# paninski-lab/lightning-pose

Measured on AMD Instinct MI355X. Metric: training frames/sec (whole node), ResNet-50 384x384 17-kp semi-sup, higher is better.
Workload: dtype bf16; 1 GPU; C2/C3: ResNet-50 SemiSupervisedHeatmapTracker 384x384, K=17, 64 labeled + 128 unlabeled frames per GPU, heatmap_mse + temporal + pca_singleview + unimodal_mse, Adam (backbone lr=0 as at step 0), bf16-mixed; global_batch=192, parallelism=dp1, sync_batchnorm=False, decode_prune=plain kernels (chosen from the maps)

## Files before the change

include/lp_hip.h:

```cpp
#ifndef LP_HIP_H
#define LP_HIP_H

#include <stddef.h>
#include <stdint.h>

#ifdef __cplusplus
extern "C" {
#endif

typedef void* lp_stream_t;

int lp_config_reload_env(void);

enum {
    LP_OK = 0,
    LP_ERR_ARGUMENT = -1,
    LP_ERR_UNSUPPORTED = -2,
};

enum { LP_TF_NONE = 0, LP_TF_SINGLE = 1, LP_TF_PER_FRAME = 2, LP_TF_PER_VIEW = 3 };

#define LP_HIP_ABI_VERSION 148
int lp_version(void);
const char* lp_strerror(int code);


typedef struct lp_decode_tables {
    const int* row_base;
    const float* row_taps;
    const int* col_start;
    const float* col_taps;
    const int* colT_start;
    const float* colT_taps;
    int ty, tx, tc;
} lp_decode_tables;

typedef struct lp_frame_map {
    const float* transforms;
    int tf_mode;
    const float* bbox;
    int bbox_stride;
    int kp_per_view;
    float model_h, model_w;
} lp_frame_map;

int lp_decode_window(int downsample_factor, int n);


int lp_decode_fwd(const float* heat, int B, int K, int h, int w, int downsample_factor, float temperature,
                  const lp_decode_tables* tables, const lp_frame_map* frame_map, float* kp_aug, float* kp_frame, float* conf,
                  float* stats, int prune, lp_stream_t stream);

int lp_decode_bwd(const float* heat, int B, int K, int h, int w, int downsample_factor, float temperature,
                  const lp_decode_tables* tables, const lp_frame_map* frame_map, const float* stats, const float* g_kp_aug,
                  const float* g_kp_frame, float* g_heat, int accumulate, int prune, lp_stream_t stream);

int lp_frame_map_apply(const float* kp_in, int B, int K, const lp_frame_map* frame_map, int backward, float* kp_out,
                       lp_stream_t stream);


int lp_heatmap_gen(const float* keypoints, const int* visibility, int B, int K, int img_h, int img_w, int h, int w, float sigma,
                   float* out, lp_stream_t stream);
int lp_heatmap_gen_bwd(const float* keypoints, const int* visibility, int B, int K, int img_h, int img_w, int h, int w, float sigma,
                       const float* grad_out, float* grad_keypoints, lp_stream_t stream);

size_t lp_temporal_heatmap_workspace_bytes(int S, int K);
int lp_temporal_heatmap_fwd(int kind, const float* pred, const float* conf, int S, int K, int h, int w, const float* epsilon,
                            float prob_threshold, float* loss, void* workspace, lp_stream_t stream);
int lp_temporal_heatmap_bwd(int kind, const float* pred, int S, int K, int h, int w, const void* workspace, const float* gout,
                            float* gpred, int accumulate, lp_stream_t stream);

int lp_heatmap_confidence(const float* heat, const float* locs, int B, int K, int h, int w, int radius, float* out, lp_stream_t stream);

size_t lp_heatmap_mse_workspace_bytes(int B, int K);
int lp_heatmap_mse_fwd(const float* targ, const float* pred, int B, int K, int h, int w, float* loss, void* workspace,
                       lp_stream_t stream);
int lp_heatmap_mse_bwd(const float* targ, const float* pred, int B, int K, int h, int w, const void* workspace, const float* gout,
                       float* gpred, int accumulate, lp_stream_t stream);
enum { LP_HM_MSE = 0, LP_HM_KL = 1, LP_HM_JS = 2 };
int lp_heatmap_loss_fwd(int kind, const float* targ, const float* pred, int B, int K, int h, int w, float* loss, void* workspace,
                        lp_stream_t stream);
int lp_heatmap_loss_bwd(int kind, const float* targ, const float* pred, int B, int K, int h, int w, const void* workspace,
                        const float* gout, float* gpred, int accumulate, lp_stream_t stream);

int lp_unimodal_mse_fwd(const float* kp_aug, const float* pred, const float* conf, int S, int K, int img_h, int img_w, int h, int w,
                        float sigma, float prob_threshold, float* loss, void* workspace, lp_stream_t stream);
int lp_unimodal_mse_bwd(const float* kp_aug, const float* pred, int S, int K, int img_h, int img_w, int h, int w, float sigma,
                        const void* workspace, const float* gout, float* gpred, int accumulate, lp_stream_t stream);

int lp_softmax2d_fwd(const float* in, long stride_b, long stride_i, long stride_k, int B, int K, int n, float* out,
                     lp_stream_t stream);
int lp_softmax2d_bwd(const float* prob, const float* gprob, int B, int K, int n, void* gin_bf16, long stride_b, long stride_i,
                     long stride_k, lp_stream_t stream);


int lp_temporal_fwd_bwd(const float* kp, const float* conf, int S, int K, const float* eps_per_kp, float prob_threshold,
                        float* loss, float* grad_unit, lp_stream_t stream);

int lp_pca_fwd_bwd(const float* kp, int S, int K, const int* index, int rows, int points, const float* mean,
                   const float* kept_eigenvectors, int ncomp, float epsilon, float* loss, float* grad_unit, lp_stream_t stream);

int lp_rmse_fwd(const float* kp_targ, const float* kp_pred, int n_points, float* loss, lp_stream_t stream);
int lp_loss_combine(const float* const* x, const float* w, const float* a, int n, float* weighted, float* total, lp_stream_t stream);
int lp_loss_combine_bwd(const float* w, const float* a, int n, const float* g_weighted, const float* g_total, float* gx, lp_stream_t stream);

typedef struct lp_conv_geom {
    int B, Hi, Wi, Ci;
    int Ho, Wo, Co;
    int R, S, stride, pad;
} lp_conv_geom;

#define LP_CONV_KERNEL_IGEMM 0
#define LP_CONV_KERNEL_PIPE 1
#define LP_CONV_KERNEL_WGRAD 2
#define LP_CONV_KERNEL_WGRAD_PIPE 3
#define LP_CONV_KERNEL_PIPE_HALO 4
#define LP_CONV_KERNEL_STEM_WGRAD_NB 8
#define LP_CONV_KERNEL_WGRAD_NB 9
#define LP_CONV_KERNEL_RES2D 5
int lp_conv_last_kernel(void);

int lp_conv_fwd(const void* x, const void* w, const lp_conv_geom* geom, const float* bias, void* out_bf16, float* out_f32, int ldo,
                int n_store, lp_stream_t stream);
int lp_conv_dgrad(const void* dy, const void* wd, const lp_conv_geom* geom, const float* bias, const void* addend,
                  const void* relu_mask, void* dx_bf16, float* dx_f32, int ldo, int n_store, int skip_empty_classes,
                  lp_stream_t stream);
typedef struct lp_gemm_batch {
    int nb, nh;
    long long a_b, a_h, b_b, b_h, c_b, c_h;
} lp_gemm_batch;
int lp_gemm_nt(const void* a, int lda, const void* b, int ldb, void* c_bf16, float* c_f32, int ldc, int M, int N, int K, int n_store,
               const float* bias, const lp_gemm_batch* batch, lp_stream_t stream);
int lp_gemm_tn(const void* x, int ldx, const void* y, int ldy, void* out_bf16, int ldo, int M, int J, int N, const lp_gemm_batch* batch,
               lp_stream_t stream);
int lp_attn_fwd(const void* qkv_bf16, int ld_qkv, int k_off, int v_off, int B, int nh, int T, float scale, void* p_bf16, int ldp,
                void* out_bf16, int ldo, lp_stream_t stream);
int lp_attn_bwd_kv(const void* qkv_bf16, int ld_qkv, int v_off, const void* d_out_bf16, int ld_do, const void* p_bf16, int ldp, const float* d_rows,
                   int B, int nh, int T, float scale, void* ds_bf16, void* dqkv_bf16, int ld_dqkv, int dk_off, int dv_off, lp_stream_t stream);
int lp_attn_rowdot(const void* a_bf16, const void* b_bf16, int rows, int nh, int ld, float* out, lp_stream_t stream);
int lp_attn_dscores(const void* d_out, int ld_do, const void* v, int ldv, const void* p_bf16, const float* d_rows, int d_row_stride,
                    long long d_b, long long d_h, float scale, void* ds_bf16, int ldc, int M, int N, int K, const lp_gemm_batch* batch,
                    lp_stream_t stream);
typedef struct lp_fxsum {
    long long hi, lo;
} lp_fxsum;
int lp_gemm_nt_gelu_bwd(const void* a, const void* b, const void* u_bf16, void* c_bf16, int M, int N, int K, lp_fxsum* colsum,
                        lp_stream_t stream);
int lp_gemm_nt_gelu_fwd(const void* a, const void* b, const float* bias, void* c_bf16, void* act_bf16, int M, int N, int K,
                        lp_stream_t stream);
typedef struct lp_bn_fuse {
    const void* z;
    const float* mean;
    const float* invstd;
    const float* gamma;
    const float* beta;
    int mask_from_z;
    const void* relu_bits;
    lp_fxsum* sums;
    int seg_images;
    int addend_half;
} lp_bn_fuse;
int lp_conv_dgrad_bits(const void* dy, const void* wd, const lp_conv_geom* geom, const void* addend, const void* relu_bits, void* dx_bf16,
                       int skip_empty_classes, lp_stream_t stream);
int lp_bn_fold(const float* w, const float* gamma, const float* beta, const float* running_mean, const float* running_var, float eps,
               int Co, int per_co, void* w_bf16, float* bias, lp_stream_t stream);
int lp_conv_fwd_act(const void* x, const void* w, const lp_conv_geom* geom, const float* bias, const void* residual_bf16, int relu,
                    void* out_bf16, lp_stream_t stream);
int lp_conv_fwd_bn(const void* x, const void* w, const lp_conv_geom* geom, void* out_bf16, const lp_bn_fuse* bn, lp_stream_t stream);
int lp_stem_fwd_bn(const void* x4, const void* w, const lp_conv_geom* geom, void* out_bf16, const lp_bn_fuse* bn, lp_stream_t stream);
int lp_conv_dgrad_bn(const void* dy, const void* wd, const lp_conv_geom* geom, const void* addend, const void* relu_mask,
                     void* dx_bf16, const lp_bn_fuse* bn, lp_stream_t stream);
size_t lp_conv_wgrad_workspace_bytes(const lp_conv_geom* geom, int split_hint);
int lp_conv_wgrad(const void* x, const void* dy, const lp_conv_geom* geom, float* dw, int split_hint, void* workspace,
                  size_t workspace_bytes, lp_stream_t stream);
int lp_conv_wgrad_bias(const void* x, const void* dy, const lp_conv_geom* geom, float* dw, float* dbias, int split_hint, void* workspace,
                       size_t workspace_bytes, lp_stream_t stream);
int lp_stem_fwd(const void* x4, const void* w, const lp_conv_geom* geom, void* out_bf16, lp_stream_t stream);
int lp_stem_wgrad(const void* x4, const void* dy, const lp_conv_geom* geom, float* dw, int split_hint, void* workspace,
                  size_t workspace_bytes, lp_stream_t stream);

int lp_f32_conv_fwd(const float* x, const float* w, const lp_conv_geom* geom, int KH, int KW, int CiS, const float* bias,
                    const float* addend, float* out, lp_stream_t stream);
int lp_f32_conv_dgrad(const float* dy, const float* w, const lp_conv_geom* geom, int KH, int KW, int CiS, const float* bias,
                      const float* addend, float* dx, lp_stream_t stream);
int lp_f32_conv_wgrad(const float* x, const float* dy, const lp_conv_geom* geom, int KH, int KW, int CiS, float* dw, lp_stream_t stream);
int lp_f32_bn_stats(const float* x, int M, int C, float* sums, lp_stream_t stream);
size_t lp_f32_bn_stats_workspace_bytes(int M, int C);
int lp_f32_bn_stats_ordered(const float* x, int M, int C, float* sums, void* workspace, size_t workspace_bytes, lp_stream_t stream);
int lp_f32_bn_apply(const float* x, const float* mean, const float* invstd, const float* gamma, const float* beta, const float* residual,
                    int relu, int M, int C, float* y, lp_stream_t stream);
int lp_f32_bn_bwd_reduce(const float* dy, const float* y_out, const float* x, const float* mean, const float* invstd, int M, int C,
                         float* sums, float* dbeta_acc, float* dgamma_acc, lp_stream_t stream);
int lp_f32_bn_bwd_apply(const float* dy, const float* y_out, const float* x, const float* mean, const float* invstd, const float* gamma,
                        const float* sums, float count, int M, int C, float* dx, float* dres, lp_stream_t stream);
int lp_f32_maxpool_fwd(const float* x, int B, int Hi, int Wi, int C, float* y, void* argmax_u8, lp_stream_t stream);
int lp_f32_maxpool_bwd(const void* argmax_u8, const float* dy, int B, int Hi, int Wi, int C, float* dx, lp_stream_t stream);
int lp_f32_images_to_nhwc4(const float* images, int B, int H, int W, float* out, lp_stream_t stream);
int lp_f32_pixel_shuffle(const float* in, int B, int h, int w, int c_out, int ld, int inverse, float* out, lp_stream_t stream);
int lp_f32_softmax2d_bwd(const float* prob, const float* gprob, int B, int K, int n, float* gin, long stride_b, long stride_i, long stride_k,
                         lp_stream_t stream);
int lp_f32_vit_patchify(const float* images, int B, int H, int W, int patch, float* out, lp_stream_t stream);
int lp_f32_vit_tokens_fwd(const float* patch, const float* cls, const float* pos, int B, int Np, int D, float* x, lp_stream_t stream);
int lp_f32_vit_tokens_bwd(const float* dx, int B, int Np, int D, float* dpatch, float* dpos, lp_stream_t stream);
int lp_f32_vit_mv_tokens_fwd(const float* patch, const float* pos, const float* view, int B, int V, int Np, int D, float* x, lp_stream_t stream);
int lp_f32_vit_mv_tokens_bwd(const float* dx, int B, int V, int Np, int D, float* dpatch, float* dpos, float* dview, void* workspace,
                             size_t workspace_bytes, lp_stream_t stream);
int lp_f32_layernorm_fwd(const float* x, const float* delta, float* x_out, const float* gamma, const float* beta, float eps, int M, int D,
                         int drop_T, float* y, float* mean, float* rstd, lp_stream_t stream);
int lp_f32_layernorm_bwd(const float* dy, const float* x, const float* mean, const float* rstd, const float* gamma, int M, int D, int drop_T,
                         float* dx_acc, float* dgamma_acc, float* dbeta_acc, lp_stream_t stream);
int lp_f32_layernorm_ls_fwd(const float* x, const float* delta, const float* ls, float* x_out, const float* gamma, const float* beta, float eps,
                            int M, int D, int drop_T, float* y, float* mean, float* rstd, lp_stream_t stream);
int lp_f32_layernorm_ls_bwd(const float* dy, const float* x, const float* mean, const float* rstd, const float* gamma, const float* ls,
                            const float* branch, int M, int D, int drop_T, float* dx_acc, float* dx_out, float* dgamma_acc, float* dbeta_acc,
                            float* colsum_acc, float* dls_acc, lp_stream_t stream);
int lp_f32_gelu_fwd(const float* x, size_t n, float* y, lp_stream_t stream);
int lp_f32_gelu_bwd(const float* x, const float* dy, size_t n, float* dx, lp_stream_t stream);
int lp_f32_attn_fwd(const float* qkv, int ld, int k_off, int v_off, int B, int nh, int T, float scale, float* p, float* o, int ldo,
                    lp_stream_t stream);
int lp_f32_attn_bwd(const float* qkv, int ld, int k_off, int v_off, const float* dout, int ldo, const float* p, int B, int nh, int T,
                    float scale, float* ds_workspace, float* dqkv, int ldd, lp_stream_t stream);

size_t lp_bn_reduce_workspace_bytes(int M, int C);
int lp_bn_stats(const void* x, int M, int C, lp_fxsum* sums, void* workspace, size_t workspace_bytes, lp_stream_t stream);
int lp_fxsum_accumulate(const lp_fxsum* sums, int n, float* dst, lp_stream_t stream);
int lp_bn_finalize(const lp_fxsum* sums, float count, int C, float eps, float momentum, float* mean, float* invstd,
                   float* running_mean, float* running_var, lp_stream_t stream);
int lp_bn_finalize_f32(const float* sums, float count, int C, float eps, float momentum, float* mean, float* invstd,
                       float* running_mean, float* running_var, lp_stream_t stream);
int lp_bn_finalize2(const lp_fxsum* sums, float count0, float count1, int C, float eps, float momentum, float* mean, float* invstd,
                    float* running_mean, float* running_var, lp_stream_t stream);
int lp_bn_apply(const void* x, const float* mean, const float* invstd, const float* gamma, const float* beta, const void* residual,
                int relu, int M, int C, void* y, void* relu_bits, lp_stream_t stream);
int lp_bn_apply_seg(const void* x, const float* mean, const float* invstd, const float* gamma, const float* beta, const void* residual,
                    int relu, int M, int C, int seg_rows, void* y, void* relu_bits, lp_stream_t stream);
int lp_bn_apply_seg_lo(const void* x, const float* mean, const float* invstd, const float* gamma, const float* beta, const void* residual,
                       const void* residual_lo, const void* zd, const float* mean_d, const float* invstd_d, const float* gamma_d,
                       const float* beta_d, int relu, int M, int C, int seg_rows, void* y, void* y_lo, void* relu_bits, lp_stream_t stream);
int lp_bn_apply_seg_rbn(const void* x, const float* mean, const float* invstd, const float* gamma, const float* beta, const void* zd,
                        const float* mean_d, const float* invstd_d, const float* gamma_d, const float* beta_d, int relu, int M, int C,
                        int seg_rows, void* y, void* relu_bits, lp_stream_t stream);
int lp_bn_bwd_reduce(const void* dy, const void* y_out, const void* x, const float* mean, const float* invstd, int M, int C,
                     lp_fxsum* sums, void* workspace, size_t workspace_bytes, lp_stream_t stream);
int lp_bn_bwd_apply(const void* dy, const void* y_out, const void* x, const float* mean, const float* invstd, const float* gamma,
                    const lp_fxsum* sums, float count, int M, int C, void* dx, void* dres, const lp_fxsum* sums_local, float* dbeta_acc,
                    float* dgamma_acc, float* terms_ws, lp_stream_t stream);
int lp_bn_bwd_apply_seg(const void* dy, const void* y_out, const void* x, const float* mean, const float* invstd, const float* gamma,
                        const lp_fxsum* sums, float count0, float count1, int M, int C, int seg_rows, void* dx, void* dres,
                        const lp_fxsum* sums_local, float* dbeta_acc, float* dgamma_acc, float* terms_ws, lp_stream_t stream);
size_t lp_bn_bwd_ds_workspace_bytes(int M, int C);
int lp_bn_bwd_apply_seg_ds(const void* dy, const void* y_out, const void* x, const float* mean, const float* invstd, const float* gamma,
                           const lp_fxsum* sums, float count0, float count1, int M, int C, int seg_rows, void* dx, void* dres,
                           const lp_fxsum* sums_local, float* dbeta_acc, float* dgamma_acc, float* terms_ws, const void* zd,
                           const float* mean_d, const float* invstd_d, lp_fxsum* sums_d, void* workspace, size_t workspace_bytes,
                           lp_stream_t stream);
int lp_maxpool_fwd(const void* x, int B, int Hi, int Wi, int C, void* y, void* argmax_u8, lp_stream_t stream);
int lp_maxpool_bwd(const void* argmax_u8, const void* dy, int B, int Hi, int Wi, int C, void* dx, lp_stream_t stream);
int lp_bn_relu_maxpool_fwd(const void* z, const float* mean, const float* invstd, const float* gamma, const float* beta, int B, int Hi, int Wi,
                           int C, void* y, void* argmax_u8, lp_stream_t stream);
int lp_bn_pool_bwd_reduce(const void* argmax_u8, const void* dy, const void* z, const float* mean, const float* invstd, const float* gamma,
                          const float* beta, int B, int Hi, int Wi, int C, lp_fxsum* sums, lp_stream_t stream);
int lp_bn_pool_bwd_apply(const void* argmax_u8, const void* dy, const void* z, const float* mean, const float* invstd, const float* gamma,
                         const float* beta, const lp_fxsum* sums, float count, int B, int Hi, int Wi, int C, void* dx,
                         const lp_fxsum* sums_local, float* dbeta_acc, float* dgamma_acc, lp_stream_t stream);
int lp_images_to_nhwc4(const float* images_nchw, int B, int H, int W, void* out_bf16, lp_stream_t stream);
int lp_pixel_shuffle(const void* in, int B, int h, int w, int c_out, int ld, int inverse, void* out, lp_stream_t stream);

int lp_vit_patchify(const float* images_nchw, int B, int H, int W, int patch, void* out_bf16, lp_stream_t stream);
int lp_vit_tokens_fwd(const void* patch_bf16, const float* cls, const float* pos, int B, int Np, int D, float* x, lp_stream_t stream);
int lp_vit_tokens_bwd(const float* dx, int B, int Np, int D, void* dpatch_bf16, float* dpos, lp_stream_t stream);
int lp_vit_mv_tokens_fwd(const void* patch_bf16, const float* pos, const float* view, int B, int V, int Np, int D, float* x,
                         lp_stream_t stream);
size_t lp_vit_mv_tokens_bwd_workspace_bytes(int B, int V, int Np, int D);
int lp_vit_mv_tokens_bwd(const float* dx, int B, int V, int Np, int D, void* dpatch_bf16, float* dpos, float* dview, void* workspace,
                         size_t workspace_bytes, lp_stream_t stream);
#define LP_CAM_MAX_VIEWS 32
size_t lp_cam_chain_workspace_bytes(int B, int V, int K);
int lp_cam_chain_fwd(const float* points, const float* intrinsics, const float* extrinsics, const float* dist12, const float* bbox, float model_h,
                     float model_w, int B, int V, int K, float* p3d, float* p2d, lp_stream_t stream);
int lp_cam_chain_bwd(const float* points, const float* intrinsics, const float* extrinsics, const float* dist12, const float* bbox, float model_h,
                     float model_w, int B, int V, int K, const float* p3d, const float* g3d, const float* g2d, void* workspace,
                     size_t workspace_bytes, float* gpoints, lp_stream_t stream);
int lp_cam_project_fwd(const float* points_3d, const float* intrinsics, const float* extrinsics, const float* dist12, const float* bbox,
                       float model_h, float model_w, int B, int V, int K, float* p2d, lp_stream_t stream);
int lp_cam_project_bwd(const float* points_3d, const float* intrinsics, const float* extrinsics, const float* dist12, const float* bbox,
                       float model_h, float model_w, int B, int V, int K, const float* g2d, float* g3d, lp_stream_t stream);
int lp_cam_pairwise_fwd_bwd(const float* targ_3d, const float* pred_3d, int B, int P, int K, float* loss, float* grad_unit, lp_stream_t stream);
int lp_small_matmul(const float* w, const float* x, int R, int Q, int D, int transpose_w, int accumulate, float* y, lp_stream_t stream);
int lp_layernorm_fwd(const float* x, const void* delta_bf16, float* x_out, const float* gamma, const float* beta, float eps, int M,
                     int D, int drop_T, void* y_bf16, float* mean, float* rstd, lp_stream_t stream);
int lp_layernorm_bwd(const void* dy_bf16, const float* x, const float* mean, const float* rstd, const float* gamma, int M, int D,
                     int drop_T, float* dx_acc, float* dgamma_acc, float* dbeta_acc, lp_stream_t stream);
int lp_layernorm_bwd_bf16(const void* dy_bf16, const float* x, const float* mean, const float* rstd, const float* gamma, int M, int D,
                          int drop_T, float* dx_acc, void* dx_bf16, float* dgamma_acc, float* dbeta_acc, lp_stream_t stream);
int lp_gelu_fwd(const void* x_bf16, size_t n, void* y_bf16, lp_stream_t stream);
int lp_gelu_bwd(const void* x_bf16, const void* dy_bf16, size_t n, void* dx_bf16, lp_stream_t stream);
int lp_gelu_bwd_colsum(const void* x_bf16, const void* dy_bf16, int rows, int cols, void* dx_bf16, float* colsum_acc, lp_stream_t stream);
int lp_layernorm_bwd_bf16_colsum(const void* dy_bf16, const float* x, const float* mean, const float* rstd, const float* gamma, int M, int D,
                                 int drop_T, float* dx_acc, void* dx_bf16, float* dgamma_acc, float* dbeta_acc, float* colsum_acc,
                                 lp_stream_t stream);
int lp_layernorm_ls_fwd(const float* x, const void* delta_bf16, const float* ls, float* x_out, const float* gamma, const float* beta, float eps,
                        int M, int D, int drop_T, void* y_bf16, float* mean, float* rstd, lp_stream_t stream);
int lp_layernorm_ls_bwd(const void* dy_bf16, const float* x, const float* mean, const float* rstd, const float* gamma, const float* ls,
                        const void* branch_bf16, int M, int D, int drop_T, float* dx_acc, void* dx_bf16, float* dgamma_acc, float* dbeta_acc,
                        float* colsum_acc, float* dls_acc, lp_stream_t stream);
int lp_softmax_rows_fwd(void* s_bf16, int rows, int n, int ld, float scale, lp_stream_t stream);
int lp_softmax_rows_bwd(const void* p_bf16, void* dp_bf16, int rows, int n, int ld, float scale, lp_stream_t stream);
int lp_transpose_batched(const void* in_bf16, int R, int Cc, int ldi, long long in_b, long long in_h, void* out_bf16, int ldo,
                         long long out_b, long long out_h, int nb, int nh, lp_stream_t stream);

enum { LP_BORDER_RENORM = 0,
       LP_BORDER_CLAMP = 1    };

typedef struct lp_frame_norm {
    float mean[3], std[3];
} lp_frame_norm;

typedef struct lp_frame_augment {
    int has_matrix;
    float matrix[6];
    float brightness, contrast, contrast_center;
    float shot_factor;
    unsigned long long seed;
} lp_frame_augment;

int lp_frames_resize(const void* src_u8, int S, int Hs, int Ws, long long frame_stride, int row_stride, int H, int W, int border,
                     const lp_frame_norm* finish_norm, float* dst, lp_stream_t stream);
int lp_frames_resize_cubic(const void* src_u8, int S, int Hs, int Ws, long long frame_stride, int row_stride, int H, int W, int round_u8,
                           const lp_frame_norm* finish_norm, float* dst, lp_stream_t stream);
int lp_frames_augment(const float* src_hwc, int S, int H, int W, const lp_frame_augment* aug, const lp_frame_norm* norm,
                      float* dst_nchw, lp_stream_t stream);
int lp_labeled_keypoints(const float* kp_src, const float* src_hw, const float* affine, const int* hflip, const int* swap,
                         const int* vis_in, int uniform_heatmaps, int B, int K, int H, int W, float* kp_out, int* vis_out,
                         lp_stream_t stream);

enum { LP_AUG_GEOM = 1, LP_AUG_BLUR = 2, LP_AUG_DROPOUT = 4, LP_AUG_DROP_PER_CHANNEL = 8, LP_AUG_SALT = 16, LP_AUG_PEPPER = 32,
       LP_AUG_ELASTIC = 64, LP_AUG_HISTEQ = 128, LP_AUG_CLAHE = 256, LP_AUG_EMBOSS = 512, LP_AUG_CROPPAD = 1024, LP_AUG_HFLIP = 2048 };
enum { LP_AUG_OP_DROPOUT = 0, LP_AUG_OP_SALT = 1, LP_AUG_OP_PEPPER = 2, LP_AUG_OP_ELASTIC = 3 };
enum { LP_AUG_LOCAL_BLUR_COARSE = 0, LP_AUG_LOCAL_EMBOSS = 1 };
#define LP_AUG_ELASTIC_MAX_RADIUS 20

typedef struct lp_labelaug_image {
    int flags;
    int image_id;
    float geom[6];
    float blur[25];
    float emboss[9];
    int coarse_gh[3], coarse_gw[3];
    unsigned coarse_thr[3];
    float elastic_alpha;
    int clahe_clip, clahe_tiles_y, clahe_tiles_x, clahe_slot;
    int pad[4];
} lp_labelaug_image;

int lp_labelaug_geom(const void* src_u8, int B, int H, int W, const lp_labelaug_image* params, void* dst_u8, lp_stream_t stream);
int lp_labelaug_local(const void* src_u8, int B, int H, int W, const lp_labelaug_image* params, int which, const void* salt_lut,
                      unsigned long long seed, void* dst_u8, lp_stream_t stream);
int lp_labelaug_elastic_field(int B, int H, int W, const lp_labelaug_image* params, float sigma, unsigned long long seed, float* tmp,
                              float* field, lp_stream_t stream);
int lp_labelaug_elastic_apply(const void* src_u8, int B, int H, int W, const lp_labelaug_image* params, const float* field, void* dst_u8,
                              lp_stream_t stream);
int lp_labelaug_histeq(const void* src_u8, int B, int H, int W, const lp_labelaug_image* params, unsigned* ws, void* lut_out, void* dst_u8,
                       lp_stream_t stream);
int lp_labelaug_clahe(const void* src_u8, int B, int H, int W, const lp_labelaug_image* params, const int* slot_image, int n_slots,
                      int max_ty, int max_tx, void* luts, void* dst_u8, lp_stream_t stream);
int lp_labelaug_finish(const void* src_u8, int B, int Hs, int Ws, const lp_labelaug_image* params, int H, int W, const lp_frame_norm* norm,
                       float* dst, lp_stream_t stream);
int lp_labelaug_keypoints(const float* kp, int B, int K, const float* affine, const lp_labelaug_image* params, const float* field, int H,
                          int W, float* kp_out, lp_stream_t stream);

int lp_patch_mask_f32(const float* images, int BV, int C, int H, int W, int patch, int count, unsigned long long key, const float* mask_in,
                      float* out, float* mask_out, lp_stream_t stream);

#define LP_MV3D_MAX_VIEWS 8
#define LP_MV3D_MAX_KEYPOINTS 128
int lp_mv3d_plan(const float* kp, const float* src_hw, const float* bbox, const float* intrinsics, const float* extrinsics,
                 const float* dist12, const float* draws, int augment, float shift_param, int H, int W, int B, int V, int K, float* kp3d,
                 float* kp2d, float* affine, int* status, lp_stream_t stream);
int lp_mv3d_fill(const void* src_u8, int B, int Hs, int Ws, const lp_frame_norm* norm, float* fill, lp_stream_t stream);
int lp_mv3d_finish(const void* src_u8, int B, int Hs, int Ws, const float* affine, const float* fill, const lp_frame_norm* norm, int V,
                   int v, int H, int W, float* dst, lp_stream_t stream);

int lp_adam_step(float* params, const float* grads, float* exp_avg, float* exp_avg_sq, size_t n, float lr, float beta1, float beta2,
                 float eps, float weight_decay, int decoupled, int step, float grad_scale, void* params_bf16, lp_stream_t stream);
int lp_cast_bf16(const float* src, size_t n, void* dst, lp_stream_t stream);
int lp_permute_cba(const void* src, int A, int B, int C, void* dst, lp_stream_t stream);

#ifdef __cplusplus
}
#endif
#endif
```

lightning-pose_amd/_lib.py:

```python

from __future__ import annotations

import ctypes as C
import os

_HERE = os.path.dirname(os.path.abspath(__file__))
LIB_PATH = os.environ.get("LP_HIP_LIB") or os.path.join(_HERE, "liblp_hip.so")


class LpHipUnavailable(RuntimeError):
    """liblp_hip.so could not be loaded, or an op was given a non-ROCm tensor.  There is no fallback path."""


class LpHipError(RuntimeError):
    pass


class DecodeTables(C.Structure):
    _fields_ = [("row_base", C.c_void_p), ("row_taps", C.c_void_p), ("col_start", C.c_void_p),
                ("col_taps", C.c_void_p), ("colT_start", C.c_void_p), ("colT_taps", C.c_void_p),
                ("ty", C.c_int), ("tx", C.c_int), ("tc", C.c_int)]


class FrameMap(C.Structure):
    _fields_ = [("transforms", C.c_void_p), ("tf_mode", C.c_int), ("bbox", C.c_void_p), ("bbox_stride", C.c_int),
                ("kp_per_view", C.c_int), ("model_h", C.c_float), ("model_w", C.c_float)]


class ConvGeom(C.Structure):
    _fields_ = [(n, C.c_int) for n in ("B", "Hi", "Wi", "Ci", "Ho", "Wo", "Co", "R", "S", "stride", "pad")]


class BnFuse(C.Structure):
    _fields_ = [("z", C.c_void_p), ("mean", C.c_void_p), ("invstd", C.c_void_p), ("gamma", C.c_void_p), ("beta", C.c_void_p),
                ("mask_from_z", C.c_int), ("relu_bits", C.c_void_p), ("sums", C.c_void_p), ("seg_images", C.c_int), ("addend_half", C.c_int)]


class FrameNorm(C.Structure):
    _fields_ = [("mean", C.c_float * 3), ("std", C.c_float * 3)]


class FrameAugment(C.Structure):
    _fields_ = [("has_matrix", C.c_int), ("matrix", C.c_float * 6), ("brightness", C.c_float), ("contrast", C.c_float),
                ("contrast_center", C.c_float), ("shot_factor", C.c_float), ("seed", C.c_ulonglong)]


class GemmBatch(C.Structure):
    _fields_ = [("nb", C.c_int), ("nh", C.c_int)] + [(n, C.c_longlong) for n in ("a_b", "a_h", "b_b", "b_h", "c_b", "c_h")]


HM_MSE, HM_KL, HM_JS = 0, 1, 2
(CONV_KERNEL_IGEMM, CONV_KERNEL_PIPE, CONV_KERNEL_WGRAD, CONV_KERNEL_WGRAD_PIPE, CONV_KERNEL_PIPE_HALO, CONV_KERNEL_RES2D, _CONV_KERNEL_6,
 _CONV_KERNEL_7, CONV_KERNEL_STEM_WGRAD_NB, CONV_KERNEL_WGRAD_NB) = range(10)
CONV_KERNEL_LABEL = {
    CONV_KERNEL_PIPE: (("conv_igemm_kernel", "conv_pipe_kernel"),),
    CONV_KERNEL_PIPE_HALO: (("conv_igemm_kernel", "conv_pipe_kernel"), (">", ",halo>")),
    CONV_KERNEL_RES2D: (("conv_igemm_kernel<64,", "conv_res2d_kernel<"), ("conv_igemm_kernel<64>", "conv_res2d_kernel<fwd>")),
    CONV_KERNEL_WGRAD_PIPE: (("conv_wgrad_kernel", "conv_wgrad_pipe_kernel"),),
    CONV_KERNEL_WGRAD_NB: (("conv_wgrad_kernel", "conv_wgrad_nb_kernel"),),
}
BORDER_RENORM, BORDER_CLAMP = 0, 1
AUG_GEOM, AUG_BLUR, AUG_DROPOUT, AUG_DROP_PER_CHANNEL, AUG_SALT, AUG_PEPPER = 1, 2, 4, 8, 16, 32
AUG_ELASTIC, AUG_HISTEQ, AUG_CLAHE, AUG_EMBOSS, AUG_CROPPAD, AUG_HFLIP = 64, 128, 256, 512, 1024, 2048
AUG_OP_DROPOUT, AUG_OP_SALT, AUG_OP_PEPPER, AUG_OP_ELASTIC = 0, 1, 2, 3
AUG_LOCAL_BLUR_COARSE, AUG_LOCAL_EMBOSS = 0, 1
AUG_ELASTIC_MAX_RADIUS = 20
TF_NONE, TF_SINGLE, TF_PER_FRAME, TF_PER_VIEW = 0, 1, 2, 3

ABI_VERSION = 148

_P, _I, _F, _L, _Z = C.c_void_p, C.c_int, C.c_float, C.c_long, C.c_size_t

PROTOTYPES = {
    "lp_version": (_I, []),
    "lp_strerror": (C.c_char_p, [_I]),
    "lp_config_reload_env": (_I, []),
    "lp_decode_window": (_I, [_I, _I]),
    "lp_decode_fwd": (_I, [_P, _I, _I, _I, _I, _I, _F, C.POINTER(DecodeTables), C.POINTER(FrameMap), _P, _P, _P, _P, _I, _P]),
    "lp_decode_bwd": (_I, [_P, _I, _I, _I, _I, _I, _F, C.POINTER(DecodeTables), C.POINTER(FrameMap), _P, _P, _P, _P, _I, _I, _P]),
    "lp_frame_map_apply": (_I, [_P, _I, _I, C.POINTER(FrameMap), _I, _P, _P]),
    "lp_heatmap_gen": (_I, [_P, _P, _I, _I, _I, _I, _I, _I, _F, _P, _P]),
    "lp_heatmap_gen_bwd": (_I, [_P, _P, _I, _I, _I, _I, _I, _I, _F, _P, _P, _P]),
    "lp_temporal_heatmap_workspace_bytes": (_Z, [_I, _I]),
    "lp_temporal_heatmap_fwd": (_I, [_I, _P, _P, _I, _I, _I, _I, _P, _F, _P, _P, _P]),
    "lp_temporal_heatmap_bwd": (_I, [_I, _P, _I, _I, _I, _I, _P, _P, _P, _I, _P]),
    "lp_heatmap_confidence": (_I, [_P, _P, _I, _I, _I, _I, _I, _P, _P]),
    "lp_heatmap_mse_workspace_bytes": (_Z, [_I, _I]),
    "lp_heatmap_mse_fwd": (_I, [_P, _P, _I, _I, _I, _I, _P, _P, _P]),
    "lp_heatmap_mse_bwd": (_I, [_P, _P, _I, _I, _I, _I, _P, _P, _P, _I, _P]),
    "lp_heatmap_loss_fwd": (_I, [_I, _P, _P, _I, _I, _I, _I, _P, _P, _P]),
    "lp_heatmap_loss_bwd": (_I, [_I, _P, _P, _I, _I, _I, _I, _P, _P, _P, _I, _P]),
    "lp_unimodal_mse_fwd": (_I, [_P, _P, _P, _I, _I, _I, _I, _I, _I, _F, _F, _P, _P, _P]),
    "lp_unimodal_mse_bwd": (_I, [_P, _P, _I, _I, _I, _I, _I, _I, _F, _P, _P, _P, _I, _P]),
    "lp_softmax2d_fwd": (_I, [_P, _L, _L, _L, _I, _I, _I, _P, _P]),
    "lp_softmax2d_bwd": (_I, [_P, _P, _I, _I, _I, _P, _L, _L, _L, _P]),
    "lp_temporal_fwd_bwd": (_I, [_P, _P, _I, _I, _P, _F, _P, _P, _P]),
    "lp_pca_fwd_bwd": (_I, [_P, _I, _I, _P, _I, _I, _P, _P, _I, _F, _P, _P, _P]),
    "lp_rmse_fwd": (_I, [_P, _P, _I, _P, _P]),
    "lp_loss_combine": (_I, [_P, _P, _P, _I, _P, _P, _P]),
    "lp_loss_combine_bwd": (_I, [_P, _P, _I, _P, _P, _P, _P]),
    "lp_conv_fwd": (_I, [_P, _P, C.POINTER(ConvGeom), _P, _P, _P, _I, _I, _P]),
    "lp_conv_dgrad": (_I, [_P, _P, C.POINTER(ConvGeom), _P, _P, _P, _P, _P, _I, _I, _I, _P]),
    "lp_conv_dgrad_bits": (_I, [_P, _P, C.POINTER(ConvGeom), _P, _P, _P, _I, _P]),
    "lp_gemm_nt": (_I, [_P, _I, _P, _I, _P, _P, _I, _I, _I, _I, _I, _P, C.POINTER(GemmBatch), _P]),
    "lp_gemm_nt_gelu_bwd": (_I, [_P, _P, _P, _P, _I, _I, _I, _P, _P]),
    "lp_gemm_nt_gelu_fwd": (_I, [_P, _P, _P, _P, _P, _I, _I, _I, _P]),
    "lp_gemm_tn": (_I, [_P, _I, _P, _I, _P, _I, _I, _I, _I, C.POINTER(GemmBatch), _P]),
    "lp_attn_fwd": (_I, [_P, _I, _I, _I, _I, _I, _I, C.c_float, _P, _I, _P, _I, _P]),
    "lp_attn_bwd_kv": (_I, [_P, _I, _I, _P, _I, _P, _I, _P, _I, _I, _I, C.c_float, _P, _P, _I, _I, _I, _P]),
    "lp_attn_rowdot": (_I, [_P, _P, _I, _I, _I, _P, _P]),
    "lp_attn_dscores": (_I, [_P, _I, _P, _I, _P, _P, _I, C.c_longlong, C.c_longlong, C.c_float, _P, _I, _I, _I, _I, C.POINTER(GemmBatch), _P]),
    "lp_conv_fwd_bn": (_I, [_P, _P, C.POINTER(ConvGeom), _P, C.POINTER(BnFuse), _P]),
    "lp_conv_last_kernel": (_I, []),
    "lp_stem_fwd_bn": (_I, [_P, _P, C.POINTER(ConvGeom), _P, C.POINTER(BnFuse), _P]),
    "lp_conv_dgrad_bn": (_I, [_P, _P, C.POINTER(ConvGeom), _P, _P, _P, C.POINTER(BnFuse), _P]),
    "lp_bn_fold": (_I, [_P, _P, _P, _P, _P, _F, _I, _I, _P, _P, _P]),
    "lp_conv_fwd_act": (_I, [_P, _P, C.POINTER(ConvGeom), _P, _P, _I, _P, _P]),
    "lp_conv_wgrad_workspace_bytes": (_Z, [C.POINTER(ConvGeom), _I]),
    "lp_conv_wgrad": (_I, [_P, _P, C.POINTER(ConvGeom), _P, _I, _P, _Z, _P]),
    "lp_conv_wgrad_bias": (_I, [_P, _P, C.POINTER(ConvGeom), _P, _P, _I, _P, C.c_size_t, _P]),
    "lp_stem_fwd": (_I, [_P, _P, C.POINTER(ConvGeom), _P, _P]),
    "lp_stem_wgrad": (_I, [_P, _P, C.POINTER(ConvGeom), _P, _I, _P, _Z, _P]),
    "lp_bn_reduce_workspace_bytes": (_Z, [_I, _I]),
    "lp_bn_stats": (_I, [_P, _I, _I, _P, _P, _Z, _P]),
    "lp_bn_finalize": (_I, [_P, _F, _I, _F, _F, _P, _P, _P, _P, _P]),
    "lp_fxsum_accumulate": (_I, [_P, _I, _P, _P]),
    "lp_bn_finalize_f32": (_I, [_P, _F, _I, _F, _F, _P, _P, _P, _P, _P]),
    "lp_bn_finalize2": (_I, [_P, _F, _F, _I, _F, _F, _P, _P, _P, _P, _P]),
    "lp_bn_apply": (_I, [_P, _P, _P, _P, _P, _P, _I, _I, _I, _P, _P, _P]),
    "lp_bn_apply_seg": (_I, [_P, _P, _P, _P, _P, _P, _I, _I, _I, _I, _P, _P, _P]),
    "lp_bn_apply_seg_lo": (_I, [_P, _P, _P, _P, _P, _P, _P, _P, _P, _P, _P, _P, _I, _I, _I, _I, _P, _P, _P, _P]),
    "lp_bn_apply_seg_rbn": (_I, [_P, _P, _P, _P, _P, _P, _P, _P, _P, _P, _I, _I, _I, _I, _P, _P, _P]),
    "lp_bn_bwd_apply_seg": (_I, [_P, _P, _P, _P, _P, _P, _P, _F, _F, _I, _I, _I, _P, _P, _P, _P, _P, _P, _P]),
    "lp_bn_bwd_ds_workspace_bytes": (_Z, [_I, _I]),
    "lp_bn_bwd_apply_seg_ds": (_I, [_P, _P, _P, _P, _P, _P, _P, _F, _F, _I, _I, _I, _P, _P, _P, _P, _P, _P, _P, _P, _P, _P, _P, _Z, _P]),
    "lp_bn_bwd_reduce": (_I, [_P, _P, _P, _P, _P, _I, _I, _P, _P, _Z, _P]),
    "lp_bn_bwd_apply": (_I, [_P, _P, _P, _P, _P, _P, _P, _F, _I, _I, _P, _P, _P, _P, _P, _P, _P]),
    "lp_maxpool_fwd": (_I, [_P, _I, _I, _I, _I, _P, _P, _P]),
    "lp_maxpool_bwd": (_I, [_P, _P, _I, _I, _I, _I, _P, _P]),
    "lp_bn_relu_maxpool_fwd": (_I, [_P, _P, _P, _P, _P, _I, _I, _I, _I, _P, _P, _P]),
    "lp_bn_pool_bwd_reduce": (_I, [_P, _P, _P, _P, _P, _P, _P, _I, _I, _I, _I, _P, _P]),
    "lp_bn_pool_bwd_apply": (_I, [_P, _P, _P, _P, _P, _P, _P, _P, C.c_float, _I, _I, _I, _I, _P, _P, _P, _P, _P]),
    "lp_images_to_nhwc4": (_I, [_P, _I, _I, _I, _P, _P]),
    "lp_pixel_shuffle": (_I, [_P, _I, _I, _I, _I, _I, _I, _P, _P]),
    "lp_vit_patchify": (_I, [_P, _I, _I, _I, _I, _P, _P]),
    "lp_vit_tokens_fwd": (_I, [_P, _P, _P, _I, _I, _I, _P, _P]),
    "lp_vit_tokens_bwd": (_I, [_P, _I, _I, _I, _P, _P, _P]),
    "lp_vit_mv_tokens_fwd": (_I, [_P, _P, _P, _I, _I, _I, _I, _P, _P]),
    "lp_vit_mv_tokens_bwd_workspace_bytes": (_Z, [_I, _I, _I, _I]),
    "lp_vit_mv_tokens_bwd": (_I, [_P, _I, _I, _I, _I, _P, _P, _P, _P, _Z, _P]),
    "lp_cam_chain_workspace_bytes": (_Z, [_I, _I, _I]),
    "lp_cam_chain_fwd": (_I, [_P, _P, _P, _P, _P, _F, _F, _I, _I, _I, _P, _P, _P]),
    "lp_cam_chain_bwd": (_I, [_P, _P, _P, _P, _P, _F, _F, _I, _I, _I, _P, _P, _P, _P, _Z, _P, _P]),
    "lp_cam_project_fwd": (_I, [_P, _P, _P, _P, _P, _F, _F, _I, _I, _I, _P, _P]),
    "lp_cam_project_bwd": (_I, [_P, _P, _P, _P, _P, _F, _F, _I, _I, _I, _P, _P, _P]),
    "lp_cam_pairwise_fwd_bwd": (_I, [_P, _P, _I, _I, _I, _P, _P, _P]),
    "lp_small_matmul": (_I, [_P, _P, _I, _I, _I, _I, _I, _P, _P]),
    "lp_layernorm_fwd": (_I, [_P, _P, _P, _P, _P, _F, _I, _I, _I, _P, _P, _P, _P]),
    "lp_layernorm_bwd": (_I, [_P, _P, _P, _P, _P, _I, _I, _I, _P, _P, _P, _P]),
    "lp_layernorm_bwd_bf16": (_I, [_P, _P, _P, _P, _P, _I, _I, _I, _P, _P, _P, _P, _P]),
    "lp_gelu_fwd": (_I, [_P, _Z, _P, _P]),
    "lp_gelu_bwd": (_I, [_P, _P, _Z, _P, _P]),
    "lp_gelu_bwd_colsum": (_I, [_P, _P, _I, _I, _P, _P, _P]),
    "lp_layernorm_bwd_bf16_colsum": (_I, [_P, _P, _P, _P, _P, _I, _I, _I, _P, _P, _P, _P, _P, _P]),
    "lp_layernorm_ls_fwd": (_I, [_P, _P, _P, _P, _P, _P, _F, _I, _I, _I, _P, _P, _P, _P]),
    "lp_layernorm_ls_bwd": (_I, [_P, _P, _P, _P, _P, _P, _P, _I, _I, _I, _P, _P, _P, _P, _P, _P, _P]),
    "lp_softmax_rows_fwd": (_I, [_P, _I, _I, _I, _F, _P]),
    "lp_softmax_rows_bwd": (_I, [_P, _P, _I, _I, _I, _F, _P]),
    "lp_transpose_batched": (_I, [_P, _I, _I, _I, C.c_longlong, C.c_longlong, _P, _I, C.c_longlong, C.c_longlong, _I, _I, _P]),
    "lp_frames_resize": (_I, [_P, _I, _I, _I, C.c_longlong, _I, _I, _I, _I, C.POINTER(FrameNorm), _P, _P]),
    "lp_frames_resize_cubic": (_I, [_P, _I, _I, _I, C.c_longlong, _I, _I, _I, _I, C.POINTER(FrameNorm), _P, _P]),
    "lp_frames_augment": (_I, [_P, _I, _I, _I, C.POINTER(FrameAugment), C.POINTER(FrameNorm), _P, _P]),
    "lp_labeled_keypoints": (_I, [_P, _P, _P, _P, _P, _P, _I, _I, _I, _I, _I, _P, _P, _P]),
    "lp_labelaug_geom": (_I, [_P, _I, _I, _I, _P, _P, _P]),
    "lp_labelaug_local": (_I, [_P, _I, _I, _I, _P, _I, _P, C.c_ulonglong, _P, _P]),
    "lp_labelaug_elastic_field": (_I, [_I, _I, _I, _P, _F, C.c_ulonglong, _P, _P, _P]),
    "lp_labelaug_elastic_apply": (_I, [_P, _I, _I, _I, _P, _P, _P, _P]),
    "lp_labelaug_histeq": (_I, [_P, _I, _I, _I, _P, _P, _P, _P, _P]),
    "lp_labelaug_clahe": (_I, [_P, _I, _I, _I, _P, _P, _I, _I, _I, _P, _P, _P]),
    "lp_labelaug_finish": (_I, [_P, _I, _I, _I, _P, _I, _I, C.POINTER(FrameNorm), _P, _P]),
    "lp_labelaug_keypoints": (_I, [_P, _I, _I, _P, _P, _P, _I, _I, _P, _P]),
    "lp_patch_mask_f32": (_I, [_P, _I, _I, _I, _I, _I, _I, C.c_ulonglong, _P, _P, _P, _P]),
    "lp_mv3d_plan": (_I, [_P, _P, _P, _P, _P, _P, _P, _I, _F, _I, _I, _I, _I, _I, _P, _P, _P, _P, _P]),
    "lp_mv3d_fill": (_I, [_P, _I, _I, _I, C.POINTER(FrameNorm), _P, _P]),
    "lp_mv3d_finish": (_I, [_P, _I, _I, _I, _P, _P, C.POINTER(FrameNorm), _I, _I, _I, _I, _P, _P]),
    "lp_f32_conv_fwd": (_I, [_P, _P, C.POINTER(ConvGeom), _I, _I, _I, _P, _P, _P, _P]),
    "lp_f32_conv_dgrad": (_I, [_P, _P, C.POINTER(ConvGeom), _I, _I, _I, _P, _P, _P, _P]),
    "lp_f32_conv_wgrad": (_I, [_P, _P, C.POINTER(ConvGeom), _I, _I, _I, _P, _P]),
    "lp_f32_bn_stats": (_I, [_P, _I, _I, _P, _P]),
    "lp_f32_bn_stats_workspace_bytes": (C.c_size_t, [_I, _I]),
    "lp_f32_bn_stats_ordered": (_I, [_P, _I, _I, _P, _P, C.c_size_t, _P]),
    "lp_f32_bn_apply": (_I, [_P, _P, _P, _P, _P, _P, _I, _I, _I, _P, _P]),
    "lp_f32_bn_bwd_reduce": (_I, [_P, _P, _P, _P, _P, _I, _I, _P, _P, _P, _P]),
    "lp_f32_bn_bwd_apply": (_I, [_P, _P, _P, _P, _P, _P, _P, _F, _I, _I, _P, _P, _P]),
    "lp_f32_maxpool_fwd": (_I, [_P, _I, _I, _I, _I, _P, _P, _P]),
    "lp_f32_maxpool_bwd": (_I, [_P, _P, _I, _I, _I, _I, _P, _P]),
    "lp_f32_images_to_nhwc4": (_I, [_P, _I, _I, _I, _P, _P]),
    "lp_f32_pixel_shuffle": (_I, [_P, _I, _I, _I, _I, _I, _I, _P, _P]),
    "lp_f32_softmax2d_bwd": (_I, [_P, _P, _I, _I, _I, _P, _L, _L, _L, _P]),
    "lp_f32_vit_patchify": (_I, [_P, _I, _I, _I, _I, _P, _P]),
    "lp_f32_vit_tokens_fwd": (_I, [_P, _P, _P, _I, _I, _I, _P, _P]),
    "lp_f32_vit_tokens_bwd": (_I, [_P, _I, _I, _I, _P, _P, _P]),
    "lp_f32_vit_mv_tokens_fwd": (_I, [_P, _P, _P, _I, _I, _I, _I, _P, _P]),
    "lp_f32_vit_mv_tokens_bwd": (_I, [_P, _I, _I, _I, _I, _P, _P, _P, _P, _Z, _P]),
    "lp_f32_layernorm_fwd": (_I, [_P, _P, _P, _P, _P, _F, _I, _I, _I, _P, _P, _P, _P]),
    "lp_f32_layernorm_bwd": (_I, [_P, _P, _P, _P, _P, _I, _I, _I, _P, _P, _P, _P]),
    "lp_f32_layernorm_ls_fwd": (_I, [_P, _P, _P, _P, _P, _P, _F, _I, _I, _I, _P, _P, _P, _P]),
    "lp_f32_layernorm_ls_bwd": (_I, [_P, _P, _P, _P, _P, _P, _P, _I, _I, _I, _P, _P, _P, _P, _P, _P, _P]),
    "lp_f32_gelu_fwd": (_I, [_P, _Z, _P, _P]),
    "lp_f32_gelu_bwd": (_I, [_P, _P, _Z, _P, _P]),
    "lp_f32_attn_fwd": (_I, [_P, _I, _I, _I, _I, _I, _I, _F, _P, _P, _I, _P]),
    "lp_f32_attn_bwd": (_I, [_P, _I, _I, _I, _P, _I, _P, _I, _I, _I, _F, _P, _P, _I, _P]),
    "lp_adam_step": (_I, [_P, _P, _P, _P, _Z, _F, _F, _F, _F, _F, _I, _I, _F, _P, _P]),
    "lp_cast_bf16": (_I, [_P, _Z, _P, _P]),
    "lp_permute_cba": (_I, [_P, _I, _I, _I, _P, _P]),
}


def declare(lib: C.CDLL) -> C.CDLL:
    for name, (res, args) in PROTOTYPES.items():
        fn = getattr(lib, name)
        fn.restype = res
        fn.argtypes = args
    have = int(lib.lp_version())
    if have != ABI_VERSION:
        raise LpHipUnavailable(f"{getattr(lib, '_name', 'liblp_hip.so')} was built for ABI {have}, this package binds ABI {ABI_VERSION} "
                               "(include/lp_hip.h: LP_HIP_ABI_VERSION) - rebuild it: python -c 'import __graft_entry__ as g; g.build()'")
    return lib


_lib = None


def lib() -> C.CDLL:
    global _lib
    if _lib is None:
        if not os.path.exists(LIB_PATH):
            raise LpHipUnavailable(
                f"{LIB_PATH} not found - build it with `python -c 'import __graft_entry__ as g; g.build()'` "
                "(lightning-pose_amd/csrc/build.sh).  lightning_pose_amd has no CPU fallback.")
        try:
            _lib = declare(C.CDLL(LIB_PATH))
        except OSError as e:
            raise LpHipUnavailable(f"cannot load {LIB_PATH}: {e}") from e
    return _lib


def check(code: int, what: str) -> None:
    if code == 0:
        return
    msg = lib().lp_strerror(code).decode()
    if code == -1:
        raise ValueError(f"{what}: {msg}")
    if code == -2:
        raise NotImplementedError(f"{what}: {msg}")
    raise LpHipError(f"{what}: HIP error {code}: {msg}")
```

lightning-pose_amd/csrc/api.hip:

```cpp
#include "lp_common.h"

#include <stdlib.h>

#include <atomic>

extern "C" int lp_version(void) { return LP_HIP_ABI_VERSION; }

namespace lp {
static int env_int(const char* name, int dflt) {
    const char* e = getenv(name);
    return (e == nullptr || *e == 0) ? dflt : atoi(e);
}
static LpSwitches read_switches() {
    LpSwitches s;
    s.conv_pipe = env_int("LP_CONV_PIPE", 1);
    s.conv_halo = env_int("LP_CONV_HALO", 1);
    s.conv_res2d = env_int("LP_CONV_RES2D", 1);
    s.infer_pipe = env_int("LP_INFER_PIPE", 1);
    s.gemm_pipe = env_int("LP_GEMM_PIPE", 1);
    s.wgrad_pipe = env_int("LP_WGRAD_PIPE", 1);
    s.wgrad_nb = env_int("LP_WGRAD_NB", 1);
    s.stem_2d = env_int("LP_STEM_2D", 1);
    s.stem_wgrad_nb = env_int("LP_STEM_WGRAD_NB", 1);
    s.pool_v2 = env_int("LP_POOL_V2", 1);
    s.bn_bwd_wgs_per_cu = env_int("LP_BN_BWD_WGS_PER_CU", 5);
    if (s.bn_bwd_wgs_per_cu < 1 || s.bn_bwd_wgs_per_cu > 5) s.bn_bwd_wgs_per_cu = 5;
    s.conv_max_wgs = env_int("LP_CONV_MAX_WGS", 0);
    return s;
}
static std::atomic<const LpSwitches*> g_switches{new LpSwitches(read_switches())};
const LpSwitches& lp_switches() { return *g_switches.load(std::memory_order_acquire); }
}

extern "C" int lp_config_reload_env(void) {
    lp::g_switches.store(new lp::LpSwitches(lp::read_switches()), std::memory_order_release);
    return LP_OK;
}

extern "C" const char* lp_strerror(int code) {
    if (code == LP_OK) return "ok";
    if (code == LP_ERR_ARGUMENT) return "invalid argument (null pointer or non-positive dimension)";
    if (code == LP_ERR_UNSUPPORTED) return "shape not covered by the instantiated kernels";
    if (code > 0) return hipGetErrorString((hipError_t)code);
    return "unknown lp_hip error";
}
```

lightning-pose_amd/csrc/bn.hip:

```cpp
#include <stdlib.h>

#include "lp_common.h"

namespace lp {

__device__ __forceinline__ void unpack8(const u16x8& v, float (&f)[8]) {
#pragma unroll
    for (int i = 0; i < 8; ++i) f[i] = bf16_to_f32(v[i]);
}

__device__ __forceinline__ u16x8 pack8(const float (&f)[8]) { return pack_bf16x8(f); }

__device__ __forceinline__ u16x8 load_stream8(const unsigned short* p) {
#if defined(__HIP_DEVICE_COMPILE__)
    return __builtin_nontemporal_load(reinterpret_cast<const u16x8*>(p));
#else
    return *reinterpret_cast<const u16x8*>(p);
#endif
}

template <int MODE>
__global__ __launch_bounds__(256) void colreduce_kernel(const unsigned short* __restrict__ A, const unsigned short* __restrict__ Yout,
                                                        const unsigned short* __restrict__ X, const float* __restrict__ mean,
                                                        const float* __restrict__ invstd, int M, int C,
// ... 839 lines not shown
}

__global__ __launch_bounds__(256) void bn_fold_kernel(const float* __restrict__ w, const float* __restrict__ gamma,
                                                      const float* __restrict__ beta, const float* __restrict__ rmean,
                                                      const float* __restrict__ rvar, float eps, int per_co,
                                                      unsigned short* __restrict__ w_out, float* __restrict__ bias_out) {
    const int co = blockIdx.x;
    const float a = gamma[co] / sqrtf(rvar[co] + eps);
    const float* src = w + (size_t)co * per_co;
    unsigned short* dst = w_out + (size_t)co * per_co;
    for (int j = threadIdx.x; j < per_co; j += 256) dst[j] = f32_to_bf16(src[j] * a);
    if (threadIdx.x == 0) bias_out[co] = beta[co] - rmean[co] * a;
}

}

extern "C" size_t lp_bn_reduce_workspace_bytes(int M, int C) {
    if (M <= 0 || C <= 0) return 0;
    return (size_t)lp::colreduce_blocks(M, C) * 2 * C * sizeof(float);
}

extern "C" int lp_bn_stats(const void* x, int M, int C, lp_fxsum* sums, void* workspace, size_t workspace_bytes, lp_stream_t stream) {
    using namespace lp;
    LP_REQUIRE(x && sums && workspace && M > 0 && C > 0);
    if (C % 8 != 0) return LP_ERR_UNSUPPORTED;
    dim3 grid(colreduce_blocks(M, C), 1);
    LP_REQUIRE(workspace_bytes >= (size_t)grid.x * 2 * C * sizeof(float));
    hipLaunchKernelGGL((colreduce_kernel<0>), grid, dim3(256), 0, (hipStream_t)stream, (const unsigned short*)x,
                       (const unsigned short*)nullptr, (const unsigned short*)nullptr, (const float*)nullptr, (const float*)nullptr, M,
                       C, (float*)workspace);
    hipLaunchKernelGGL(rows_reduce_kernel, dim3((C + 15) / 16), dim3(256), 0, (hipStream_t)stream, (const float*)workspace, (int)grid.x, C, sums);
    return launch_status();
}

__global__ void fx_accumulate_kernel(const lp_fxsum* __restrict__ sums, int n, float* __restrict__ dst) {
    const int i = blockIdx.x * blockDim.x + threadIdx.x;
    if (i < n) dst[i] += lp::fx_value(&sums[i]);
}

extern "C" int lp_fxsum_accumulate(const lp_fxsum* sums, int n, float* dst, lp_stream_t stream) {
    LP_REQUIRE(sums && dst && n > 0);
    hipLaunchKernelGGL(fx_accumulate_kernel, dim3((n + 255) / 256), dim3(256), 0, (hipStream_t)stream, sums, n, dst);
    return lp::launch_status();
}

extern "C" int lp_bn_fold(const float* w, const float* gamma, const float* beta, const float* running_mean, const float* running_var,
                          float eps, int Co, int per_co, void* w_bf16, float* bias, lp_stream_t stream) {
    using namespace lp;
    LP_REQUIRE(w && gamma && beta && running_mean && running_var && w_bf16 && bias && Co > 0 && per_co > 0 && eps > 0.f);
    hipLaunchKernelGGL(bn_fold_kernel, dim3(Co), dim3(256), 0, (hipStream_t)stream, w, gamma, beta, running_mean, running_var, eps, per_co,
                       (unsigned short*)w_bf16, bias);
    return launch_status();
}

extern "C" int lp_bn_finalize(const lp_fxsum* sums, float count, int C, float eps, float momentum, float* mean, float* invstd,
                              float* running_mean, float* running_var, lp_stream_t stream) {
    using namespace lp;
    LP_REQUIRE(sums && mean && invstd && C > 0 && count > 0.f);
    hipLaunchKernelGGL(bn_finalize_kernel<lp_fxsum>, dim3((C + 255) / 256), dim3(256), 0, (hipStream_t)stream, sums, count, count, 1, C, eps,
                       momentum, mean, invstd, running_mean, running_var);
    return launch_status();
}

extern "C" int lp_bn_finalize2(const lp_fxsum* sums, float count0, float count1, int C, float eps, float momentum, float* mean, float* invstd,
                               float* running_mean, float* running_var, lp_stream_t stream) {
    using namespace lp;
    LP_REQUIRE(sums && mean && invstd && C > 0 && count0 > 0.f && count1 > 0.f);
    hipLaunchKernelGGL(bn_finalize_kernel<lp_fxsum>, dim3((C + 255) / 256), dim3(256), 0, (hipStream_t)stream, sums, count0, count1, 2, C, eps,
                       momentum, mean, invstd, running_mean, running_var);
    return launch_status();
}

extern "C" int lp_bn_finalize_f32(const float* sums, float count, int C, float eps, float momentum, float* mean, float* invstd,
                                  float* running_mean, float* running_var, lp_stream_t stream) {
    using namespace lp;
    LP_REQUIRE(sums && mean && invstd && C > 0 && count > 0.f);
    hipLaunchKernelGGL(bn_finalize_kernel<float>, dim3((C + 255) / 256), dim3(256), 0, (hipStream_t)stream, sums, count, count, 1, C, eps,
                       momentum, mean, invstd, running_mean, running_var);
    return launch_status();
}


static int bn_apply_impl(const void* x, const float* mean, const float* invstd, const float* gamma, const float* beta, const void* residual,
                         int relu, int M, int C, int seg_rows, void* y, void* relu_bits, lp_stream_t stream) {
    using namespace lp;
    LP_REQUIRE(x && mean && invstd && gamma && beta && y && M > 0 && C > 0 && seg_rows >= 0 && seg_rows < M);
    if (C % 8 != 0) return LP_ERR_UNSUPPORTED;
    const size_t n_chunks = (size_t)M * (C / 8);
    hipLaunchKernelGGL(bn_apply_kernel<false>, dim3(bn_grid(n_chunks, C / 8)), dim3(256), 0, (hipStream_t)stream, (const unsigned short*)x, mean, invstd,
                       gamma, beta, (const unsigned short*)residual, relu, n_chunks, C, (unsigned short*)y, (unsigned char*)relu_bits,
                       (size_t)seg_rows * (C / 8), BnResidualBn{});
    return launch_status();
}

extern "C" int lp_bn_apply_seg_rbn(const void* x, const float* mean, const float* invstd, const float* gamma, const float* beta, const void* zd,
                                   const float* mean_d, const float* invstd_d, const float* gamma_d, const float* beta_d, int relu, int M, int C,
                                   int seg_rows, void* y, void* relu_bits, lp_stream_t stream) {
    using namespace lp;
    LP_REQUIRE(x && mean && invstd && gamma && beta && zd && mean_d && invstd_d && gamma_d && beta_d && y && M > 0 && C > 0 && seg_rows >= 0 &&
               seg_rows < M);
    if (C % 8 != 0) return LP_ERR_UNSUPPORTED;
    const size_t n_chunks = (size_t)M * (C / 8);
    hipLaunchKernelGGL(bn_apply_kernel<true>, dim3(bn_grid(n_chunks, C / 8)), dim3(256), 0, (hipStream_t)stream, (const unsigned short*)x, mean, invstd,
                       gamma, beta, (const unsigned short*)zd, relu, n_chunks, C, (unsigned short*)y, (unsigned char*)relu_bits,
                       (size_t)seg_rows * (C / 8), BnResidualBn{mean_d, invstd_d, gamma_d, beta_d});
    return launch_status();
}

extern "C" int lp_bn_apply_seg_lo(const void* x, const float* mean, const float* invstd, const float* gamma, const float* beta, const void* residual,
                                  const void* residual_lo, const void* zd, const float* mean_d, const float* invstd_d, const float* gamma_d,
                                  const float* beta_d, int relu, int M, int C, int seg_rows, void* y, void* y_lo, void* relu_bits,
                                  lp_stream_t stream) {
    using namespace lp;
    LP_REQUIRE(x && mean && invstd && gamma && beta && y && M > 0 && C > 0 && seg_rows >= 0 && seg_rows < M);
    LP_REQUIRE((zd == nullptr) || (mean_d && invstd_d && gamma_d && beta_d && residual == nullptr && residual_lo == nullptr));
    LP_REQUIRE(residual_lo == nullptr || residual != nullptr);
    if (C % 8 != 0) return LP_ERR_UNSUPPORTED;
    const size_t n_chunks = (size_t)M * (C / 8);
    const BnResidualLo rl{(const unsigned short*)residual_lo, (unsigned short*)y_lo};
    if (zd != nullptr)
        hipLaunchKernelGGL((bn_apply_kernel<true, true>), dim3(bn_grid(n_chunks, C / 8)), dim3(256), 0, (hipStream_t)stream, (const unsigned short*)x, mean,
                           invstd, gamma, beta, (const unsigned short*)zd, relu, n_chunks, C, (unsigned short*)y, (unsigned char*)relu_bits,
                           (size_t)seg_rows * (C / 8), BnResidualBn{mean_d, invstd_d, gamma_d, beta_d}, rl);
    else
        hipLaunchKernelGGL((bn_apply_kernel<false, true>), dim3(bn_grid(n_chunks, C / 8)), dim3(256), 0, (hipStream_t)stream, (const unsigned short*)x, mean,
                           invstd, gamma, beta, (const unsigned short*)residual, relu, n_chunks, C, (unsigned short*)y, (unsigned char*)relu_bits,
                           (size_t)seg_rows * (C / 8), BnResidualBn{}, rl);
    return launch_status();
}

extern "C" int lp_bn_apply(const void* x, const float* mean, const float* invstd, const float* gamma, const float* beta,
                           const void* residual, int relu, int M, int C, void* y, void* relu_bits, lp_stream_t stream) {
    return bn_apply_impl(x, mean, invstd, gamma, beta, residual, relu, M, C, 0, y, relu_bits, stream);
}

extern "C" int lp_bn_apply_seg(const void* x, const float* mean, const float* invstd, const float* gamma, const float* beta,
                               const void* residual, int relu, int M, int C, int seg_rows, void* y, void* relu_bits, lp_stream_t stream) {
    return bn_apply_impl(x, mean, invstd, gamma, beta, residual, relu, M, C, seg_rows, y, relu_bits, stream);
}

extern "C" int lp_bn_bwd_reduce(const void* dy, const void* y_out, const void* x, const float* mean, const float* invstd, int M, int C,
                                lp_fxsum* sums, void* workspace, size_t workspace_bytes, lp_stream_t stream) {
    using namespace lp;
    LP_REQUIRE(dy && x && mean && invstd && sums && workspace && M > 0 && C > 0);
    if (C % 8 != 0) return LP_ERR_UNSUPPORTED;
    dim3 grid(colreduce_blocks(M, C), 1);
    LP_REQUIRE(workspace_bytes >= (size_t)grid.x * 2 * C * sizeof(float));
    hipLaunchKernelGGL((colreduce_kernel<1>), grid, dim3(256), 0, (hipStream_t)stream, (const unsigned short*)dy,
                       (const unsigned short*)y_out, (const unsigned short*)x, mean, invstd, M, C, (float*)workspace);
    hipLaunchKernelGGL(rows_reduce_kernel, dim3((C + 15) / 16), dim3(256), 0, (hipStream_t)stream, (const float*)workspace, (int)grid.x, C, sums);
    return launch_status();
}

static int bn_bwd_apply_impl(const void* dy, const void* y_out, const void* x, const float* mean, const float* invstd, const float* gamma,
                             const lp_fxsum* sums, float count0, float count1, int M, int C, int seg_rows, void* dx, void* dres,
                             const lp_fxsum* sums_local, float* dbeta_acc, float* dgamma_acc, float* terms_ws, lp_stream_t stream) {
    using namespace lp;
    LP_REQUIRE(dy && x && mean && invstd && gamma && dx && M > 0 && C > 0 && count0 > 0.f && count1 > 0.f && seg_rows >= 0 && seg_rows < M);
    LP_REQUIRE(sums_local != nullptr || (dbeta_acc == nullptr && dgamma_acc == nullptr));
    if (C % 8 != 0 || (terms_ws == nullptr && C > kBnBwdMaxC)) return LP_ERR_UNSUPPORTED;
    const size_t n_chunks = (size_t)M * (C / 8);
    if (terms_ws != nullptr) {
        const int nseg = seg_rows > 0 ? 2 : 1;
        hipLaunchKernelGGL(bn_bwd_terms_kernel, dim3((nseg * 2 * C + 255) / 256), dim3(256), 0, (hipStream_t)stream, sums, 1.f / count0, 1.f / count1, C,
                           nseg, terms_ws, sums_local, dbeta_acc, dgamma_acc);
        hipLaunchKernelGGL(bn_bwd_apply_kernel<true>, dim3(bn_grid(n_chunks, C / 8, lp_switches().bn_bwd_wgs_per_cu)), dim3(256), 0, (hipStream_t)stream, (const unsigned short*)dy,
                           (const unsigned short*)y_out, (const unsigned short*)x, mean, invstd, gamma, sums, 1.f / count0, n_chunks, C,
                           (unsigned short*)dx, (unsigned short*)dres, (size_t)seg_rows * (C / 8), 1.f / count1, sums_local, dbeta_acc, dgamma_acc,
                           (const float*)terms_ws);
        return launch_status();
    }
    hipLaunchKernelGGL(bn_bwd_apply_kernel<false>, dim3(bn_grid(n_chunks, C / 8)), dim3(256), 0, (hipStream_t)stream, (const unsigned short*)dy,
                       (const unsigned short*)y_out, (const unsigned short*)x, mean, invstd, gamma, sums, 1.f / count0, n_chunks, C,
                       (unsigned short*)dx, (unsigned short*)dres, (size_t)seg_rows * (C / 8), 1.f / count1, sums_local, dbeta_acc, dgamma_acc,
                       (const float*)nullptr);
    return launch_status();
}

extern "C" int lp_bn_bwd_apply(const void* dy, const void* y_out, const void* x, const float* mean, const float* invstd,
                               const float* gamma, const lp_fxsum* sums, float count, int M, int C, void* dx, void* dres,
                               const lp_fxsum* sums_local, float* dbeta_acc, float* dgamma_acc, float* terms_ws, lp_stream_t stream) {
    return bn_bwd_apply_impl(dy, y_out, x, mean, invstd, gamma, sums, count, count, M, C, 0, dx, dres, sums_local, dbeta_acc, dgamma_acc, terms_ws,
                             stream);
}

extern "C" int lp_bn_bwd_apply_seg(const void* dy, const void* y_out, const void* x, const float* mean, const float* invstd,
                                   const float* gamma, const lp_fxsum* sums, float count0, float count1, int M, int C, int seg_rows, void* dx,
                                   void* dres, const lp_fxsum* sums_local, float* dbeta_acc, float* dgamma_acc, float* terms_ws,
                                   lp_stream_t stream) {
    return bn_bwd_apply_impl(dy, y_out, x, mean, invstd, gamma, sums, count0, count1, M, C, seg_rows, dx, dres, sums_local, dbeta_acc,
                             dgamma_acc, terms_ws, stream);
}

extern "C" size_t lp_bn_bwd_ds_workspace_bytes(int M, int C) {
    if (M <= 0 || C <= 0 || C % 8 != 0) return 0;
    return (size_t)2 * lp::bn_grid((size_t)M * (C / 8), C / 8, lp::lp_switches().bn_bwd_wgs_per_cu) * 2 * C * sizeof(float);
}

extern "C" int lp_bn_bwd_apply_seg_ds(const void* dy, const void* y_out, const void* x, const float* mean, const float* invstd,
                                      const float* gamma, const lp_fxsum* sums, float count0, float count1, int M, int C, int seg_rows,
                                      void* dx, void* dres, const lp_fxsum* sums_local, float* dbeta_acc, float* dgamma_acc, float* terms_ws,
                                      const void* zd, const float* mean_d, const float* invstd_d, lp_fxsum* sums_d, void* workspace,
                                      size_t workspace_bytes, lp_stream_t stream) {
    using namespace lp;
    LP_REQUIRE(dy && x && mean && invstd && gamma && dx && M > 0 && C > 0 && count0 > 0.f && count1 > 0.f && seg_rows >= 0 && seg_rows < M);
    LP_REQUIRE(sums_local != nullptr || (dbeta_acc == nullptr && dgamma_acc == nullptr));
    LP_REQUIRE(terms_ws && zd && mean_d && invstd_d && sums_d && workspace);
    if (C % 8 != 0 || 256 % (C / 8) != 0) return LP_ERR_UNSUPPORTED;
    const size_t n_chunks = (size_t)M * (C / 8);
    const int nseg = seg_rows > 0 ? 2 : 1;
    const int grid = bn_grid(n_chunks, C / 8, lp_switches().bn_bwd_wgs_per_cu);
    LP_REQUIRE(workspace_bytes >= (size_t)nseg * grid * 2 * C * sizeof(float));
    hipStream_t st = (hipStream_t)stream;
    hipLaunchKernelGGL(bn_bwd_terms_kernel, dim3((nseg * 2 * C + 255) / 256), dim3(256), 0, st, sums, 1.f / count0, 1.f / count1, C, nseg, terms_ws,
                       sums_local, dbeta_acc, dgamma_acc);
    hipLaunchKernelGGL((bn_bwd_apply_kernel<true, true>), dim3(grid), dim3(256), 0, st, (const unsigned short*)dy, (const unsigned short*)y_out,
                       (const unsigned short*)x, mean, invstd, gamma, sums, 1.f / count0, n_chunks, C, (unsigned short*)dx, (unsigned short*)dres,
                       (size_t)seg_rows * (C / 8), 1.f / count1, sums_local, dbeta_acc, dgamma_acc, (const float*)terms_ws,
                       BnBwdDs{(const unsigned short*)zd, mean_d, invstd_d, (float*)workspace});
    for (int sg = 0; sg < nseg; ++sg)
        hipLaunchKernelGGL(rows_reduce_kernel, dim3((C + 15) / 16), dim3(256), 0, st, (const float*)workspace + (size_t)sg * grid * 2 * C, grid, C,
                           sums_d + (size_t)sg * 2 * C);
    return launch_status();
}

extern "C" int lp_maxpool_fwd(const void* x, int B, int Hi, int Wi, int C, void* y, void* argmax_u8, lp_stream_t stream) {
    using namespace lp;
    LP_REQUIRE(x && y && argmax_u8 && B > 0 && Hi > 0 && Wi > 0 && C > 0);
    if (C % 8 != 0) return LP_ERR_UNSUPPORTED;
    const int Ho = (Hi - 1) / 2 + 1, Wo = (Wi - 1) / 2 + 1;
    hipLaunchKernelGGL(maxpool_fwd_kernel, dim3(grid_for((size_t)B * Ho * Wo * (C / 8))), dim3(256), 0, (hipStream_t)stream,
                       (const unsigned short*)x, B, Hi, Wi, C, Ho, Wo, (unsigned short*)y, (unsigned char*)argmax_u8);
    return launch_status();
}

extern "C" int lp_maxpool_bwd(const void* argmax_u8, const void* dy, int B, int Hi, int Wi, int C, void* dx, lp_stream_t stream) {
    using namespace lp;
    LP_REQUIRE(argmax_u8 && dy && dx && B > 0 && Hi > 0 && Wi > 0 && C > 0);
    if (C % 8 != 0) return LP_ERR_UNSUPPORTED;
    const int Ho = (Hi - 1) / 2 + 1, Wo = (Wi - 1) / 2 + 1;
    hipLaunchKernelGGL(maxpool_bwd_kernel, dim3(grid_for((size_t)B * Hi * Wi * (C / 8))), dim3(256), 0, (hipStream_t)stream,
                       (const unsigned char*)argmax_u8, (const unsigned short*)dy, B, Hi, Wi, C, Ho, Wo, (unsigned short*)dx);
    return launch_status();
}

extern "C" int lp_bn_relu_maxpool_fwd(const void* z, const float* mean, const float* invstd, const float* gamma, const float* beta, int B,
                                      int Hi, int Wi, int C, void* y, void* argmax_u8, lp_stream_t stream) {
    using namespace lp;
    LP_REQUIRE(z && mean && invstd && gamma && beta && y && argmax_u8 && B > 0 && Hi > 0 && Wi > 0 && C > 0);
    if (C % 8 != 0 || 256 % (C / 8) != 0 || (long long)B * Hi >= (1LL << 31)) return LP_ERR_UNSUPPORTED;
    const int Ho = (Hi - 1) / 2 + 1, Wo = (Wi - 1) / 2 + 1;
    hipLaunchKernelGGL(bn_relu_maxpool_fwd_kernel, dim3(pool_row_blocks(B * Ho)), dim3(256), 0, (hipStream_t)stream,
                       (const unsigned short*)z, mean, invstd, gamma, beta, B, Hi, Wi, C, Ho, Wo, (unsigned short*)y,
                       (unsigned char*)argmax_u8);
    return launch_status();
}

extern "C" int lp_bn_pool_bwd_reduce(const void* argmax_u8, const void* dy, const void* z, const float* mean, const float* invstd,
                                     const float* gamma, const float* beta, int B, int Hi, int Wi, int C, lp_fxsum* sums, lp_stream_t stream) {
    using namespace lp;
    LP_REQUIRE(argmax_u8 && dy && z && mean && invstd && gamma && beta && sums && B > 0 && Hi > 0 && Wi > 0 && C > 0);
    if (C % 8 != 0 || 256 % (C / 8) != 0) return LP_ERR_UNSUPPORTED;
    const int Ho = (Hi - 1) / 2 + 1, Wo = (Wi - 1) / 2 + 1;
    const long long pixels = (long long)B * Hi * Wi;
    if (pixels >= (1LL << 31)) return LP_ERR_UNSUPPORTED;
    if (pool_v2_ok(C, Hi, Wi, Ho, Wo)) {
        const int band = pool_v2_band(), wgs = B * ((Ho + band - 1) / band);
        hipLaunchKernelGGL(bn_pool_bwd_v2_kernel<false>, dim3(wgs), dim3(256), 0, (hipStream_t)stream,
                           (const unsigned char*)argmax_u8, (const unsigned short*)dy, (const unsigned short*)z, mean, invstd, gamma, beta, nullptr,
                           0.f, B, Hi, Wi, Ho, Wo, band, sums, nullptr, nullptr, nullptr, nullptr);
        return launch_status();
    }
    hipLaunchKernelGGL(bn_pool_bwd_reduce_kernel, dim3(pool_row_blocks(B * Hi, 4)), dim3(256), 0, (hipStream_t)stream,
                       (const unsigned char*)argmax_u8, (const unsigned short*)dy, (const unsigned short*)z, mean, invstd, gamma, beta, B, Hi,
                       Wi, C, Ho, Wo, sums);
    return launch_status();
}

extern "C" int lp_bn_pool_bwd_apply(const void* argmax_u8, const void* dy, const void* z, const float* mean, const float* invstd,
                                    const float* gamma, const float* beta, const lp_fxsum* sums, float count, int B, int Hi, int Wi, int C,
                                    void* dx, const lp_fxsum* sums_local, float* dbeta_acc, float* dgamma_acc, lp_stream_t stream) {
    using namespace lp;
    LP_REQUIRE(argmax_u8 && dy && z && mean && invstd && gamma && beta && dx && B > 0 && Hi > 0 && Wi > 0 && C > 0 && count > 0.f);
    LP_REQUIRE(sums_local != nullptr || (dbeta_acc == nullptr && dgamma_acc == nullptr));
    if (C % 8 != 0 || 256 % (C / 8) != 0 || (long long)B * Hi >= (1LL << 31)) return LP_ERR_UNSUPPORTED;
    const int Ho = (Hi - 1) / 2 + 1, Wo = (Wi - 1) / 2 + 1;
    if (pool_v2_ok(C, Hi, Wi, Ho, Wo)) {
        const int band = pool_v2_band(), wgs = B * ((Ho + band - 1) / band);
        hipLaunchKernelGGL(bn_pool_bwd_v2_kernel<true>, dim3(wgs), dim3(256), 0, (hipStream_t)stream,
                           (const unsigned char*)argmax_u8, (const unsigned short*)dy, (const unsigned short*)z, mean, invstd, gamma, beta, sums,
                           1.f / count, B, Hi, Wi, Ho, Wo, band, nullptr, (unsigned short*)dx, sums_local, dbeta_acc, dgamma_acc);
        return launch_status();
    }
    hipLaunchKernelGGL(bn_pool_bwd_apply_kernel, dim3(pool_row_blocks(B * Hi)), dim3(256), 0, (hipStream_t)stream,
                       (const unsigned char*)argmax_u8, (const unsigned short*)dy, (const unsigned short*)z, mean, invstd, gamma, beta, sums,
                       1.f / count, B, Hi, Wi, C, Ho, Wo, (unsigned short*)dx, sums_local, dbeta_acc, dgamma_acc);
    return launch_status();
}

extern "C" int lp_images_to_nhwc4(const float* images, int B, int H, int W, void* out, lp_stream_t stream) {
    using namespace lp;
    LP_REQUIRE(images && out && B > 0 && H > 0 && W > 0);
    hipLaunchKernelGGL(nchw3_to_nhwc4_kernel, dim3(grid_for((size_t)B * H * W)), dim3(256), 0, (hipStream_t)stream, images, B, H * W,
                       (unsigned short*)out);
    return launch_status();
}
// ... 15 lines not shown
```

lightning-pose_amd/csrc/conv.hip:

```cpp
#include <stdlib.h>

#include "lp_common.h"

namespace lp {

constexpr int kBM = 128;
constexpr int kBK = 64;
constexpr int kLD = kBK + 8;

struct ConvGeom {
    int B, Hi, Wi, Ci;
    int Ho, Wo, Co;
    int R, S, stride, pad;
};

struct ConvEpilogue {
    unsigned short* out_bf16;
    float* out_f32;
    int ldo;
    int n_store;
    const float* bias;
    const unsigned short* addend;
    const unsigned short* relu_mask;
    const unsigned char* relu_bits;
// ... 1008 lines not shown
    return (p.ek == kEkNone || p.ek == kEkInfer || p.ek == kEkZ) && halo_shape_ok(p.g, p.M, conv_ck(p), p.N > 64 ? 384 : 512);
}

static bool admits_res2d(const ConvProblem& p) {
    if (!res2d_shape_ok(p.g, conv_ck(p), p.N)) return false;
    if (p.mode == kModeInfer) return p.ep.addend == nullptr;
    return (p.ek == kEkNone || p.ek == kEkZ) && p.ep.bias == nullptr && admits_pipe(p);
}

static ConvRoute route_conv(const ConvProblem& p, const LpSwitches& sw) {
    const bool pipe = sw.conv_pipe != 0 && (p.gate == nullptr || sw.*p.gate != 0);
    if (p.mode == kModeStem) return ConvRoute{pipe && stem2d_shape_ok(p.g) ? LP_CONV_KERNEL_RES2D : LP_CONV_KERNEL_IGEMM, 64, p.mode, p.ek};
    if (pipe && sw.conv_res2d != 0 && admits_res2d(p)) return ConvRoute{LP_CONV_KERNEL_RES2D, 64, p.mode, p.ek};
    if (pipe && admits_pipe(p))
        return ConvRoute{sw.conv_halo != 0 && admits_halo(p) ? LP_CONV_KERNEL_PIPE_HALO : LP_CONV_KERNEL_PIPE, p.N > 64 ? 128 : 64, p.mode, p.ek};
    return ConvRoute{p.igemm_form ? LP_CONV_KERNEL_IGEMM : kNoKernel, p.igemm_cols > 64 ? 128 : 64, p.mode, p.ek};
}

static int conv_max_wgs(int per_cu) {
    if (lp_switches().conv_max_wgs > 0) return lp_switches().conv_max_wgs;
    static int cus = [] {
        int dev = 0, c = 0;
        if (hipGetDevice(&dev) != hipSuccess || hipDeviceGetAttribute(&c, hipDeviceAttributeMultiprocessorCount, dev) != hipSuccess || c <= 0) c = 256;
        return c;
    }();
    return per_cu * cus;
}

template <int BN, int MODE>
static void launch_igemm(const ConvProblem& p, hipStream_t st) {
    const ConvGeom& g = p.g;
    const int tm = (p.M + kBM - 1) / kBM, tn = (p.N + BN - 1) / BN, per_z = tm * tn, ntiles = per_z * p.nz;
    const int grid = ntiles < conv_max_wgs(2) ? ntiles : conv_max_wgs(2);
    const int ck = MODE == kModeDgrad ? g.Co : g.Ci;
    unsigned x_bytes = (unsigned)(2ull * (MODE == kModeDgrad ? (size_t)g.B * g.Ho * g.Wo * g.Co : (size_t)g.B * g.Hi * g.Wi * g.Ci));
    unsigned w_bytes = (unsigned)(2ull * (size_t)p.N * (MODE == kModeStem ? (size_t)p.K : (size_t)g.R * g.S * ck));
    GemmExt gx{ck, MODE == kModeStem ? p.K : g.R * g.S * ck, 1, per_z, 0u, 0u, 0u, 0u, 0u, 0u};
    if (p.gemm) {
        gx = p.gx;
        gx.tiles_per_z = per_z;
        x_bytes = p.x_bytes;
        w_bytes = p.w_bytes;
    }
    hipLaunchKernelGGL((conv_igemm_kernel<BN, MODE>), dim3(grid), dim3(256), 0, st, (const unsigned short*)p.x, (const unsigned short*)p.w,
                       x_bytes, w_bytes, g, p.lat, gx, make_fastdiv(p.lat.nh * p.lat.nw), make_fastdiv(p.lat.nw), p.M, p.N, p.K, tn, ntiles, p.ep);
}

template <int MODE, bool INFER = false>
static void launch_res2d(const ConvProblem& p, hipStream_t st) {
    const ConvGeom& g = p.g;
    const int ntiles = g.B * (g.Hi / 16) * (g.Wi / 16);
    const int grid = ntiles < conv_max_wgs(1) ? ntiles : conv_max_wgs(1);
    const unsigned x_bytes = (unsigned)(2ull * g.B * g.Hi * g.Wi * 64), w_bytes = (unsigned)(2ull * 64 * 9 * 64);
    hipLaunchKernelGGL((conv_res2d_kernel<MODE, INFER>), dim3(grid), dim3(512), 0, st, (const unsigned short*)p.x, (const unsigned short*)p.w, x_bytes,
                       w_bytes, g.B, g.Hi, g.Wi, ntiles, p.ep);
}

static void launch_stem2d(const ConvProblem& p, hipStream_t st) {
    const ConvGeom& g = p.g;
    const int ntiles = g.B * (g.Ho / 16) * (g.Wo / 16);
    const int grid = ntiles < 2 * conv_max_wgs(1) ? ntiles : 2 * conv_max_wgs(1);
    hipLaunchKernelGGL(conv_stem2d_kernel, dim3(grid), dim3(512), 0, st, (const unsigned short*)p.x, (const unsigned short*)p.w,
                       (unsigned)(2ull * g.B * g.Hi * g.Wi * 4), g.B, g.Ho, g.Wo, ntiles, p.ep);
}

template <int BN, int MODE, int EK, bool HALO = false>
static void launch_pipe(const ConvProblem& p, hipStream_t st) {
    const ConvGeom& g = p.g;
    const int tm = (p.M + kPM - 1) / kPM, tn = p.N / BN, ntiles = tm * tn;
    const int grid = ntiles < conv_max_wgs(1) ? ntiles : conv_max_wgs(1);
    const int ck = MODE == kModeDgrad ? g.Co : g.Ci;
    const unsigned x_bytes = (unsigned)(2ull * (MODE == kModeDgrad ? (size_t)g.B * g.Ho * g.Wo * g.Co : (size_t)g.B * g.Hi * g.Wi * g.Ci));
    const unsigned w_bytes = (unsigned)(2ull * (size_t)p.N * g.R * g.S * ck);
    const HaloDivs hd{make_fastdiv(g.Hi), make_fastdiv(g.Wi + 2), make_fastdiv(g.Hi + 2)};
    hipLaunchKernelGGL((conv_pipe_kernel<BN, MODE, EK, HALO>), dim3(grid), dim3(512), 0, st, (const unsigned short*)p.x, (const unsigned short*)p.w,
                       x_bytes, w_bytes, g, p.lat, make_fastdiv(p.lat.nh * p.lat.nw), make_fastdiv(p.lat.nw), p.M, p.N, p.K, tn, ntiles, p.ep, hd);
}

template <int BN>
static void launch_conv_bn(const ConvRoute& r, const ConvProblem& p, hipStream_t st) {
    if (r.kernel == LP_CONV_KERNEL_IGEMM) {
        switch (r.mode) {
            case kModeFwd: return launch_igemm<BN, kModeFwd>(p, st);
            case kModeDgrad: return launch_igemm<BN, kModeDgrad>(p, st);
            case kModeInfer: return launch_igemm<BN, kModeInfer>(p, st);
            default: return launch_igemm<BN, kModeAttn>(p, st);
        }
    }
    const bool halo = r.kernel == LP_CONV_KERNEL_PIPE_HALO;
    switch (r.ek) {
        case kEkNone: return halo ? launch_pipe<BN, kModeFwd, kEkNone, true>(p, st) : launch_pipe<BN, kModeFwd, kEkNone>(p, st);
        case kEkInfer: return halo ? launch_pipe<BN, kModeFwd, kEkInfer, true>(p, st) : launch_pipe<BN, kModeFwd, kEkInfer>(p, st);
        case kEkZ: return halo ? launch_pipe<BN, kModeDgrad, kEkZ, true>(p, st) : launch_pipe<BN, kModeDgrad, kEkZ>(p, st);
        case kEkAZB: return launch_pipe<BN, kModeDgrad, kEkAZB>(p, st);
        case kEkPB: return launch_pipe<BN, kModeDgrad, kEkPB>(p, st);
        default: return launch_pipe<BN, kModeDgrad, kEkPlain>(p, st);
    }
}

static void launch_conv(const ConvRoute& r, const ConvProblem& p, hipStream_t st) {
    g_last_conv_kernel = r.kernel;
    if (r.kernel == LP_CONV_KERNEL_RES2D) {
        switch (r.mode) {
            case kModeStem: return launch_stem2d(p, st);
            case kModeInfer: return launch_res2d<kModeFwd, true>(p, st);
            case kModeDgrad: return launch_res2d<kModeDgrad>(p, st);
            default: return launch_res2d<kModeFwd>(p, st);
        }
    }
    if (r.mode == kModeStem) return launch_igemm<64, kModeStem>(p, st);
    if (r.ek == kEkGeluFwd) return launch_pipe<128, kModeFwd, kEkGeluFwd>(p, st);
    if (r.ek == kEkGeluBwd) return launch_pipe<128, kModeFwd, kEkGeluBwd>(p, st);
    if (r.bn == 128) launch_conv_bn<128>(r, p, st);
    else launch_conv_bn<64>(r, p, st);
}

static int run_conv(const ConvProblem& p, lp_stream_t stream) {
    const ConvRoute r = route_conv(p, lp_switches());
    if (r.kernel == kNoKernel) return LP_ERR_UNSUPPORTED;
    launch_conv(r, p, (hipStream_t)stream);
    return launch_status();
}

static ConvProblem conv_problem(int mode, const void* x, const void* w, const ConvGeom& g, int rows_h, int rows_w, int N, int K) {
    ConvProblem p{};
    p.mode = mode, p.ek = -1, p.x = x, p.w = w, p.g = g;
    p.lat = Lattice{0, 1, rows_h, 0, 1, rows_w, 0, 1, g.R, 0, 1, g.S};
    p.M = g.B * rows_h * rows_w, p.N = N, p.K = K, p.seg_rows = p.M;
    p.dense = true, p.igemm_form = true, p.igemm_cols = N, p.nz = 1;
    return p;
}

static int gemm_problem(ConvProblem& p, int mode, const void* a, int lda, const void* b, int ldb, int ldc, int c_align, int M, int N, int K,
                        const lp_gemm_batch* batch) {
    if (K % kBK != 0 || lda % 8 != 0 || ldb % 8 != 0 || ldc % c_align != 0) return LP_ERR_UNSUPPORTED;
    const lp_gemm_batch z = batch ? *batch : lp_gemm_batch{1, 1, 0, 0, 0, 0, 0, 0};
    LP_REQUIRE(z.nb > 0 && z.nh > 0 && z.a_b >= 0 && z.a_h >= 0 && z.b_b >= 0 && z.b_h >= 0 && z.c_b >= 0 && z.c_h >= 0);
    const long long a_elems = (z.nb - 1) * z.a_b + (z.nh - 1) * z.a_h + (long long)(M - 1) * lda + K;
    const long long b_elems = (z.nb - 1) * z.b_b + (z.nh - 1) * z.b_h + (long long)(N - 1) * ldb + K;
    const long long c_elems = (z.nb - 1) * z.c_b + (z.nh - 1) * z.c_h + (long long)M * ldc;
    if (a_elems >= (1LL << 31) || b_elems >= (1LL << 31) || c_elems >= (1LL << 32)) return LP_ERR_UNSUPPORTED;
    if ((z.a_b | z.a_h | z.b_b | z.b_h) % 8 != 0 || (z.c_b | z.c_h) % c_align != 0) return LP_ERR_UNSUPPORTED;
    p = conv_problem(mode, a, b, ConvGeom{1, 1, M, K, 1, M, N, 1, 1, 1, 0}, 1, M, N, K);
    p.dense = z.nb * z.nh == 1 && lda == K && ldb == K && ldc == N;
    p.gemm = true, p.nz = z.nb * z.nh, p.x_bytes = (unsigned)(2 * a_elems), p.w_bytes = (unsigned)(2 * b_elems);
    p.gx = GemmExt{lda, ldb, z.nh, 0, (unsigned)(2 * z.a_b), (unsigned)(2 * z.a_h), (unsigned)(2 * z.b_b), (unsigned)(2 * z.b_h), (unsigned)z.c_b,
                   (unsigned)z.c_h};
    return LP_OK;
}

}
#include "conv_stem_wgrad.h"
#include "conv_wgrad_nb.h"
namespace lp {

constexpr int kWgradWgs = 512;

struct WgradRoute {
    bool ok;
    int kernel;
    int split, per;
    size_t ws_floats;
    int bn, tiles_a, tiles_b;
    bool swap, tuned;
    int Ka, Cb;
    int kh, PT, lead;
};

static void slice_pixels(WgradRoute& p, int units, int ksteps, int split, int cap) {
    if (split > cap) split = cap;
    if (split < 1) split = 1;
    p.per = ((ksteps + split - 1) / split) * kBK;
    p.split = (units + p.per - 1) / p.per;
}

static WgradRoute plan_wgrad(int M, int Kw, int Co, int split_hint) {
    WgradRoute p{};
    p.kernel = LP_CONV_KERNEL_WGRAD;
    p.bn = Co > 64 ? 128 : 64;
    p.tiles_a = (Kw + kBM - 1) / kBM;
    p.tiles_b = p.bn == 128 ? (Co + 127) / 128 : 1;
    const int tiles = p.tiles_a * p.tiles_b, ksteps = (M + kBK - 1) / kBK;
    slice_pixels(p, M, ksteps, split_hint > 0 ? split_hint : kWgradWgs / tiles, ksteps < 65535 ? ksteps : 65535);
    p.ws_floats = (size_t)p.split * tiles * 4 * 2 * (p.bn / 64) * 16 * 64;
    p.ok = true;
    return p;
}

static WgradRoute plan_stem_wgrad_nb(const ConvGeom& g, int split_hint) {
    WgradRoute p{};
    if (g.Wo % 64 != 0 || g.Hi != 2 * g.Ho || g.Wi != 2 * g.Wo || 128ull * g.B * g.Ho * g.Wo >= (1ull << 31) ||
        8ull * g.B * g.Hi * g.Wi >= (1ull << 31))
        return p;
    p.kernel = LP_CONV_KERNEL_STEM_WGRAD_NB;
    p.bn = 64, p.tiles_a = 2, p.tiles_b = 1;
    const int M = g.B * g.Ho * g.Wo, ksteps = M / kBK;
    slice_pixels(p, M, ksteps, split_hint > 0 ? split_hint : 768, ksteps);
    p.ws_floats = (size_t)p.split * 2 * 4 * 2 * 16 * 64;
    p.ok = true;
    return p;
}

static WgradRoute plan_wgrad_pipe(const ConvGeom& g, int split_hint) {
    WgradRoute p{};
    const int M = g.B * g.Ho * g.Wo, Kw = g.R * g.S * g.Ci;
    const bool one = g.R == 1 && g.S == 1 && g.stride == 1 && g.pad == 0 && g.Hi == g.Ho && g.Wi == g.Wo;
    if (g.Ci % 8 != 0 || g.Co % 64 != 0 || M < 4 * kBK) return p;
    p.kernel = LP_CONV_KERNEL_WGRAD_PIPE;
    p.swap = one && Kw % 256 != 0 && g.Co % 256 == 0 && Kw % 64 == 0;
    p.Ka = p.swap ? g.Co : Kw;
    p.Cb = p.swap ? Kw : g.Co;
    p.bn = p.Cb % 128 == 0 ? 128 : 64;
    if (p.Cb % p.bn != 0) return p;
    p.tiles_a = (p.Ka + 255) / 256;
    p.tiles_b = p.Cb / p.bn;
    p.tuned = (long long)p.tiles_a * 256 * 8 <= (long long)p.Ka * 9 && (long long)p.Ka * p.Cb >= 120LL * (p.Ka + p.Cb);
    const int tiles = p.tiles_a * p.tiles_b;
    const int cus = conv_max_wgs(1);
    const int ksteps = (M + kBK - 1) / kBK;
    int split = split_hint;
    if (split <= 0) {
        double best = 1e30;
        for (int s = 1; s <= 2 * cus && s <= ksteps / 2; ++s) {
            if (s != 1 && (tiles * s) % cus > 0 && (tiles * (s + 1) + cus - 1) / cus == (tiles * s + cus - 1) / cus) continue;
            const double rounds = (double)((tiles * s + cus - 1) / cus), per = (double)((ksteps + s - 1) / s);
            const double cost = rounds * per + 0.04 * (p.bn / 128.0) * s * tiles + 2.0 * rounds;
            if (cost < best) best = cost, split = s;
        }
    }
    slice_pixels(p, M, ksteps, split, ksteps / 2);
    p.ws_floats = (size_t)p.split * tiles * 256 * p.bn;
    p.ok = true;
    return p;
}

static WgradRoute plan_wgrad_nb(const ConvGeom& g, int split_hint) {
    WgradRoute p{};
    if (g.R != 3 || g.S != 3 || g.stride != 1 || g.pad != 1 || g.Hi != g.Ho || g.Wi != g.Wo || g.Ci % 64 != 0 || g.Co % 64 != 0) return p;
    if (g.Wi > 126) return p;
    const long long pt = (long long)g.B * (g.Hi + 1) * (g.Wi + 1);
    if (pt + 64 * 8 >= (1LL << 31)) return p;
    p.kernel = LP_CONV_KERNEL_WGRAD_NB;
    p.PT = (int)pt;
    p.lead = 1 + (g.Wi + 1) / 64;
    p.bn = g.Co % 128 == 0 ? 128 : 64;
    p.kh = p.bn == 64 ? 2 : 1;
    p.tiles_a = g.Ci / 64;
    p.tiles_b = g.Co / p.bn;
    const int tiles = p.tiles_a * p.tiles_b;
    const int ksteps = (p.PT + kBK - 1) / kBK;
    int split = split_hint;
    if (split <= 0) {
        const int cus = conv_max_wgs(1);
        const double step_us = 0.96 * p.bn / 128.0;
        double best = 1e30;
        for (int s = 1; s <= ksteps && s * tiles <= 2 * cus; ++s) {
            const double rounds = (double)((tiles * s + cus - 1) / cus), per = (double)((ksteps + s - 1) / s);
            const double cost = rounds * (per * step_us + 15.0) + 0.06 * s * tiles;
            if (cost < best) best = cost, split = s;
        }
    }
    slice_pixels(p, p.PT, ksteps, split, ksteps < 65535 ? ksteps : 65535);
    p.ws_floats = (size_t)p.split * p.kh * tiles * 9 * 64 * p.bn;
    p.ok = true;
    return p;
}

static bool is_stem(const ConvGeom& g) { return g.R == 7 && g.S == 7 && g.stride == 2 && g.pad == 3 && g.Ci == 4 && g.Co == 64; }

struct WgradCandidates {
    int n;
    WgradRoute r[3];
};

static WgradCandidates wgrad_candidates(const ConvGeom& g, bool stem, int split_hint) {
    WgradCandidates c{};
    const int M = g.B * g.Ho * g.Wo;
    auto add = [&c](const WgradRoute& p) {
        if (p.ok) c.r[c.n++] = p;
    };
    if (stem) {
        if (lp_switches().stem_wgrad_nb != 0) add(plan_stem_wgrad_nb(g, split_hint));
        add(plan_wgrad(M, 256, 64, split_hint));
    } else {
        add(plan_wgrad_nb(g, split_hint));
        add(plan_wgrad_pipe(g, split_hint));
        add(plan_wgrad(M, g.R * g.S * g.Ci, g.Co, split_hint));
    }
    return c;
}

static const WgradRoute& route_wgrad(const WgradCandidates& c, const LpSwitches& sw, bool dbias) {
    const bool pipe = !dbias && sw.conv_pipe != 0;
    for (int i = 0; i < c.n - 1; ++i) {
        const WgradRoute& r = c.r[i];
        if (r.kernel == LP_CONV_KERNEL_WGRAD_NB && !(pipe && sw.wgrad_pipe == 1 && sw.wgrad_nb != 0)) continue;
        if (r.kernel == LP_CONV_KERNEL_WGRAD_PIPE && !(pipe && sw.wgrad_pipe != 0 && (sw.wgrad_pipe == 2 || r.tuned))) continue;
        return r;
    }
    return c.r[c.n - 1];
}

template <int BN>
static void launch_wgrad(const WgradRoute& p, const void* x, const void* dy, const ConvGeom& g, float* dw, float* dbias, float* ws, hipStream_t st) {
    const int M = g.B * g.Ho * g.Wo, Kw = g.R * g.S * g.Ci, tiles = p.tiles_a * p.tiles_b;
    const unsigned x_bytes = (unsigned)(2ull * g.B * g.Hi * g.Wi * g.Ci), dy_bytes = (unsigned)(2ull * M * g.Co);
    TnExt ext{};
    ext.col_sums = dbias;
    const auto kernel = dbias ? conv_wgrad_kernel<BN, false, true> : conv_wgrad_kernel<BN, false, false>;
    hipLaunchKernelGGL(kernel, dim3(tiles * p.split), dim3(256), 0, st, (const unsigned short*)x, (const unsigned short*)dy, x_bytes, dy_bytes, g,
                       M, Kw, tiles, p.tiles_b, p.per, make_fastdiv(g.Ho * g.Wo), make_fastdiv(g.Wo), ws, ext);
    launch_wgrad_reduce<BN>(ws, p.split, tiles, p.tiles_b, Kw, g.Co, dw, st);
}

template <int BN>
static void launch_wgrad_pipe(const WgradRoute& p, const void* x, const void* dy, const ConvGeom& g, float* dw, float* ws, hipStream_t st) {
    const int M = g.B * g.Ho * g.Wo, Kw = g.R * g.S * g.Ci;
    const unsigned x_bytes = (unsigned)(2ull * g.B * g.Hi * g.Wi * g.Ci), dy_bytes = (unsigned)(2ull * M * g.Co);
    WgradPipeGeom wg{};
    const void *pa = x, *qb = dy;
    unsigned pa_bytes = x_bytes, qb_bytes = dy_bytes;
    if (p.swap) {
        wg = WgradPipeGeom{g.B, g.Ho, g.Wo, g.Ho, g.Wo, g.Co, 1, 1, 1, 0, p.Ka, p.Cb, 1};
        pa = dy, qb = x, pa_bytes = dy_bytes, qb_bytes = x_bytes;
    } else {
        const int plain = g.R == 1 && g.S == 1 && g.stride == 1 && g.pad == 0 && g.Hi == g.Ho && g.Wi == g.Wo;
        wg = WgradPipeGeom{g.B, g.Hi, g.Wi, g.Ho, g.Wo, g.Ci, g.R, g.S, g.stride, g.pad, p.Ka, p.Cb, plain};
    }
    const int tiles = p.tiles_a * p.tiles_b;
    const int sa = p.swap ? Kw : 1, sb = p.swap ? 1 : Kw;
    hipLaunchKernelGGL((conv_wgrad_pipe_kernel<BN>), dim3(tiles * p.split), dim3(512), 0, st, (const unsigned short*)pa, (const unsigned short*)qb,
                       pa_bytes, qb_bytes, wg, M, tiles, p.tiles_b, p.per, make_fastdiv(g.Ho * g.Wo), make_fastdiv(g.Wo), ws);
    hipLaunchKernelGGL((wgrad_pipe_reduce_kernel<BN>), dim3(tiles * 256 * BN / 64), dim3(256), 0, st, ws, p.split, tiles, p.tiles_b, p.Ka, p.Cb,
                       sa, sb, dw);
}

template <int BN>
static void launch_wgrad_nb(const WgradRoute& p, const void* x, const void* dy, const ConvGeom& g, float* dw, float* ws, hipStream_t st) {
    const unsigned x_bytes = (unsigned)(2ull * g.B * g.Hi * g.Wi * g.Ci), dy_bytes = (unsigned)(2ull * g.B * g.Ho * g.Wo * g.Co);
    const WgradNbGeom ng{g.B, g.Hi, g.Wi, g.Ci, g.Co, p.PT, p.lead};
    const int tiles = p.tiles_a * p.tiles_b;
    hipLaunchKernelGGL((conv_wgrad_nb_kernel<BN>), dim3(tiles * p.split), dim3(512), 0, st, (const unsigned short*)x, (const unsigned short*)dy,
                       x_bytes, dy_bytes, ng, tiles, p.tiles_b, p.per, make_fastdiv(g.Wi + 1), make_fastdiv(g.Hi + 1), ws);
    hipLaunchKernelGGL((wgrad_nb_reduce_kernel<BN>), dim3(tiles * 9 * BN), dim3(256), 0, st, ws, p.split * p.kh, tiles, p.tiles_b, g.Ci, dw);
}

static bool geom_ok(const lp_conv_geom* c) {
    return c && c->B > 0 && c->Hi > 0 && c->Wi > 0 && c->Ci > 0 && c->Ho > 0 && c->Wo > 0 && c->Co > 0 && c->R > 0 && c->S > 0 &&
           c->stride > 0 && c->pad >= 0;
}

static ConvGeom to_geom(const lp_conv_geom* c) {
    ConvGeom g{c->B, c->Hi, c->Wi, c->Ci, c->Ho, c->Wo, c->Co, c->R, c->S, c->stride, c->pad};
    return g;
}

}

static int conv_fwd_impl(const void* x, const void* w, const lp_conv_geom* geom, const float* bias, void* out_bf16, float* out_f32, int ldo,
                         int n_store, const lp_bn_fuse* bn, lp_stream_t stream) {
    using namespace lp;
    LP_REQUIRE(x && w && geom_ok(geom) && (out_bf16 || out_f32) && ldo > 0);
    ConvGeom g = to_geom(geom);
    if (g.Ci % kBK != 0 || g.R * g.S > 32 || (long long)g.B * g.Hi * g.Wi * g.Ci >= (1LL << 31) ||
        (long long)g.B * g.Ho * g.Wo * ldo >= (1LL << 32))
        return LP_ERR_UNSUPPORTED;
    ConvProblem p = conv_problem(kModeFwd, x, w, g, g.Ho, g.Wo, g.Co, g.R * g.S * g.Ci);
    p.ek = kEkNone;
    p.ep = ConvEpilogue{(unsigned short*)out_bf16, out_f32, ldo, n_store > 0 ? n_store : p.N, bias};
    if (bn) {
        LP_REQUIRE(bn->sums && bn->seg_images >= 0);
        if (p.N % 8 != 0) return LP_ERR_UNSUPPORTED;
        p.seg_rows = seg_split_rows(bn->seg_images, g.B, (long long)g.Ho * g.Wo, p.M);
        if (p.seg_rows < 0) return LP_ERR_UNSUPPORTED;
        bn_fuse_begin(p.ep, bn);
    }
    return run_conv(p, stream);
}

extern "C" int lp_conv_last_kernel(void) { return lp::g_last_conv_kernel; }

extern "C" int lp_conv_fwd(const void* x, const void* w, const lp_conv_geom* geom, const float* bias, void* out_bf16, float* out_f32,
                           int ldo, int n_store, lp_stream_t stream) {
    return conv_fwd_impl(x, w, geom, bias, out_bf16, out_f32, ldo, n_store, nullptr, stream);
}

extern "C" int lp_conv_fwd_act(const void* x, const void* w, const lp_conv_geom* geom, const float* bias, const void* residual_bf16, int relu,
                               void* out_bf16, lp_stream_t stream) {
    using namespace lp;
    LP_REQUIRE(x && w && geom_ok(geom) && out_bf16);
    ConvGeom g = to_geom(geom);
    if (g.Ci % kBK != 0 || g.Co % 8 != 0 || g.R * g.S > 32 || (long long)g.B * g.Hi * g.Wi * g.Ci >= (1LL << 31) ||
        (long long)g.B * g.Ho * g.Wo * g.Co >= (1LL << 32))
        return LP_ERR_UNSUPPORTED;
    ConvProblem p = conv_problem(kModeInfer, x, w, g, g.Ho, g.Wo, g.Co, g.R * g.S * g.Ci);
    p.ek = kEkInfer, p.gate = &LpSwitches::infer_pipe;
    p.ep.out_bf16 = (unsigned short*)out_bf16, p.ep.ldo = p.N, p.ep.n_store = p.N, p.ep.bias = bias;
    p.ep.addend = (const unsigned short*)residual_bf16, p.ep.relu_fwd = relu != 0;
    return run_conv(p, stream);
}

extern "C" int lp_conv_fwd_bn(const void* x, const void* w, const lp_conv_geom* geom, void* out_bf16, const lp_bn_fuse* bn,
                              lp_stream_t stream) {
    LP_REQUIRE(bn && geom && out_bf16);
    return conv_fwd_impl(x, w, geom, nullptr, out_bf16, nullptr, geom->Co, 0, bn, stream);
}

extern "C" int lp_gemm_nt(const void* a, int lda, const void* b, int ldb, void* c_bf16, float* c_f32, int ldc, int M, int N, int K,
                          int n_store, const float* bias, const lp_gemm_batch* batch, lp_stream_t stream) {
    using namespace lp;
    LP_REQUIRE(a && b && (c_bf16 || c_f32) && M > 0 && N > 0 && K > 0 && lda >= K && ldb >= K && ldc > 0);
    ConvProblem p;
    if (const int rc = gemm_problem(p, kModeFwd, a, lda, b, ldb, ldc, 1, M, N, K, batch)) return rc;
    p.ek = kEkNone, p.gate = &LpSwitches::gemm_pipe;
    p.ep = ConvEpilogue{(unsigned short*)c_bf16, c_f32, ldc, n_store > 0 ? n_store : N, bias};
    p.igemm_cols = p.ep.n_store;
    return run_conv(p, stream);
}

extern "C" int lp_gemm_nt_gelu_fwd(const void* a, const void* b, const float* bias, void* c_bf16, void* act_bf16, int M, int N, int K,
                                   lp_stream_t stream) {
    using namespace lp;
    LP_REQUIRE(a && b && c_bf16 && act_bf16 && M > 0 && N > 0 && K > 0);
    ConvProblem p;
    if (const int rc = gemm_problem(p, kModeFwd, a, K, b, K, N, 1, M, N, K, nullptr)) return rc;
    p.ek = kEkGeluFwd, p.igemm_form = false;
    p.ep = ConvEpilogue{(unsigned short*)c_bf16, nullptr, N, N, bias};
    p.ep.out2_bf16 = (unsigned short*)act_bf16;
    return run_conv(p, stream);
}

extern "C" int lp_gemm_nt_gelu_bwd(const void* a, const void* b, const void* u_bf16, void* c_bf16, int M, int N, int K, lp_fxsum* colsum,
                                   lp_stream_t stream) {
    using namespace lp;
    LP_REQUIRE(a && b && u_bf16 && c_bf16 && M > 0 && N > 0 && K > 0);
    ConvProblem p;
    if (const int rc = gemm_problem(p, kModeFwd, a, K, b, K, N, 1, M, N, K, nullptr)) return rc;
    p.ek = kEkGeluBwd, p.igemm_form = false;
    p.ep = ConvEpilogue{(unsigned short*)c_bf16, nullptr, N, N, nullptr};
    p.ep.addend = (const unsigned short*)u_bf16;
    p.ep.stats_sums = colsum;
    return run_conv(p, stream);
}

extern "C" int lp_attn_dscores(const void* d_out, int ld_do, const void* v, int ldv, const void* p_bf16, const float* d_rows, int d_row_stride,
                               long long d_b, long long d_h, float scale, void* ds_bf16, int ldc, int M, int N, int K,
                               const lp_gemm_batch* batch, lp_stream_t stream) {
    using namespace lp;
    LP_REQUIRE(d_out && v && p_bf16 && d_rows && ds_bf16 && batch && M > 0 && N > 0 && K > 0 && ld_do >= K && ldv >= K && ldc >= N &&
               d_row_stride > 0 && d_b >= 0 && d_h >= 0);
    ConvProblem p;
    if (const int rc = gemm_problem(p, kModeAttn, d_out, ld_do, v, ldv, ldc, 8, M, N, K, batch)) return rc;
    const long long d_elems = (batch->nb - 1) * d_b + (batch->nh - 1) * d_h + (long long)(M - 1) * d_row_stride + 1;
// ... 65 lines not shown
            for (int pw = 0; pw < 2; ++pw) {
                const int h0 = ((ph - g.pad) % 2 + 2) % 2, w0 = ((pw - g.pad) % 2 + 2) % 2;
                const int nh = h0 < g.Hi ? (g.Hi - h0 + 1) / 2 : 0, nw = w0 < g.Wi ? (g.Wi - w0 + 1) / 2 : 0;
                const int nr = ph < g.R ? (g.R - ph + 1) / 2 : 0, ns = pw < g.S ? (g.S - pw + 1) / 2 : 0;
                if (skip_empty_classes && nr * ns == 0) continue;
                add(Lattice{h0, 2, nh, w0, 2, nw, ph, 2, nr, pw, 2, ns});
            }
    }
    auto problem_of = [&p](const DgradLaunch& e) {
        p.lat = e.lat, p.M = e.M, p.K = e.K, p.seg_rows = e.seg_rows;
    };
    for (int i = 0; i < n; ++i) {
        if (plan[i].seg_rows < 0) return LP_ERR_UNSUPPORTED;
        problem_of(plan[i]);
        plan[i].route = route_conv(p, lp_switches());
    }
    for (int i = 0; i < n; ++i) {
        problem_of(plan[i]);
        launch_conv(plan[i].route, p, (hipStream_t)stream);
    }
    return launch_status();
}

extern "C" int lp_conv_dgrad(const void* dy, const void* wd, const lp_conv_geom* geom, const float* bias, const void* addend,
                             const void* relu_mask, void* dx_bf16, float* dx_f32, int ldo, int n_store, int skip_empty_classes,
                             lp_stream_t stream) {
    return conv_dgrad_impl(dy, wd, geom, bias, addend, relu_mask, dx_bf16, dx_f32, ldo, n_store, skip_empty_classes, nullptr, stream);
}

extern "C" int lp_conv_dgrad_bits(const void* dy, const void* wd, const lp_conv_geom* geom, const void* addend, const void* relu_bits,
                                  void* dx_bf16, int skip_empty_classes, lp_stream_t stream) {
    LP_REQUIRE(relu_bits && geom);
    return conv_dgrad_impl(dy, wd, geom, nullptr, addend, nullptr, dx_bf16, nullptr, geom->Ci, 0, skip_empty_classes, nullptr, stream, relu_bits);
}

extern "C" int lp_conv_dgrad_bn(const void* dy, const void* wd, const lp_conv_geom* geom, const void* addend, const void* relu_mask,
                                void* dx_bf16, const lp_bn_fuse* bn, lp_stream_t stream) {
    LP_REQUIRE(bn && geom);
    return conv_dgrad_impl(dy, wd, geom, nullptr, addend, relu_mask, dx_bf16, nullptr, geom->Ci, 0, 0, bn, stream);
}

extern "C" size_t lp_conv_wgrad_workspace_bytes(const lp_conv_geom* geom, int split_hint) {
    using namespace lp;
    if (!geom_ok(geom)) return 0;
    const ConvGeom g = to_geom(geom);
    const WgradCandidates c = wgrad_candidates(g, is_stem(g), split_hint);
    size_t fl = 0;
    for (int i = 0; i < c.n; ++i)
        if (c.r[i].ws_floats > fl) fl = c.r[i].ws_floats;
    return fl * sizeof(float);
}

static int conv_wgrad_impl(const void* x, const void* dy, const lp_conv_geom* geom, float* dw, float* dbias, int split_hint, void* workspace,
                           size_t workspace_bytes, lp_stream_t stream) {
    using namespace lp;
    LP_REQUIRE(x && dy && geom_ok(geom) && dw && workspace);
    ConvGeom g = to_geom(geom);
    if (g.Ci % 8 != 0 || g.Co % 8 != 0 || (long long)g.B * g.Hi * g.Wi * g.Ci >= (1LL << 31) ||
        (long long)g.B * g.Ho * g.Wo * g.Co >= (1LL << 31))
        return LP_ERR_UNSUPPORTED;
    const WgradCandidates c = wgrad_candidates(g, false, split_hint);
    const WgradRoute& p = route_wgrad(c, lp_switches(), dbias != nullptr);
    LP_REQUIRE(workspace_bytes >= p.ws_floats * sizeof(float));
    hipStream_t st = (hipStream_t)stream;
    float* ws = (float*)workspace;
    g_last_conv_kernel = p.kernel;
    if (p.kernel == LP_CONV_KERNEL_WGRAD_NB) {
        if (p.bn == 128) launch_wgrad_nb<128>(p, x, dy, g, dw, ws, st);
        else launch_wgrad_nb<64>(p, x, dy, g, dw, ws, st);
    } else if (p.kernel == LP_CONV_KERNEL_WGRAD_PIPE) {
        if (p.bn == 128) launch_wgrad_pipe<128>(p, x, dy, g, dw, ws, st);
        else launch_wgrad_pipe<64>(p, x, dy, g, dw, ws, st);
    } else {
        if (p.bn == 128) launch_wgrad<128>(p, x, dy, g, dw, dbias, ws, st);
        else launch_wgrad<64>(p, x, dy, g, dw, dbias, ws, st);
    }
    return launch_status();
}

extern "C" int lp_conv_wgrad(const void* x, const void* dy, const lp_conv_geom* geom, float* dw, int split_hint, void* workspace,
                             size_t workspace_bytes, lp_stream_t stream) {
    return conv_wgrad_impl(x, dy, geom, dw, nullptr, split_hint, workspace, workspace_bytes, stream);
}

extern "C" int lp_conv_wgrad_bias(const void* x, const void* dy, const lp_conv_geom* geom, float* dw, float* dbias, int split_hint,
                                  void* workspace, size_t workspace_bytes, lp_stream_t stream) {
    LP_REQUIRE(dbias);
    return conv_wgrad_impl(x, dy, geom, dw, dbias, split_hint, workspace, workspace_bytes, stream);
}

extern "C" int lp_gemm_tn(const void* x, int ldx, const void* y, int ldy, void* out_bf16, int ldo, int M, int J, int N,
                          const lp_gemm_batch* batch, lp_stream_t stream) {
    using namespace lp;
    LP_REQUIRE(x && y && out_bf16 && M > 0 && J > 0 && N > 0 && ldx >= J && ldy >= N && ldo >= N);
    if (ldx % 8 != 0 || ldy % 8 != 0 || N % 8 != 0) return LP_ERR_UNSUPPORTED;
    const int nb = batch ? batch->nb : 1, nh = batch ? batch->nh : 1;
    LP_REQUIRE(nb > 0 && nh > 0);
    const long long a_b = batch ? batch->a_b : 0, a_h = batch ? batch->a_h : 0, b_b = batch ? batch->b_b : 0, b_h = batch ? batch->b_h : 0;
    const long long c_b = batch ? batch->c_b : 0, c_h = batch ? batch->c_h : 0;
    LP_REQUIRE(a_b >= 0 && a_h >= 0 && b_b >= 0 && b_h >= 0 && c_b >= 0 && c_h >= 0);
    if ((a_b | a_h | b_b | b_h) % 8 != 0) return LP_ERR_UNSUPPORTED;
    const int Jr = (J + 7) / 8 * 8;
    LP_REQUIRE(Jr <= ldx);
    const long long x_elems = (nb - 1) * a_b + (nh - 1) * a_h + (long long)(M - 1) * ldx + Jr;
    const long long y_elems = (nb - 1) * b_b + (nh - 1) * b_h + (long long)(M - 1) * ldy + N;
    const long long o_elems = (nb - 1) * c_b + (nh - 1) * c_h + (long long)J * ldo;
    if (x_elems >= (1LL << 31) || y_elems >= (1LL << 31) || o_elems >= (1LL << 32)) return LP_ERR_UNSUPPORTED;
    ConvGeom g{1, 1, M, Jr, 1, M, N, 1, 1, 1, 0};
    const int tj = (Jr + kBM - 1) / kBM;
    TnExt tn{(unsigned short*)out_bf16, ldx, ldy, ldo, nh, (unsigned)(2 * a_b), (unsigned)(2 * a_h), (unsigned)(2 * b_b), (unsigned)(2 * b_h),
             (unsigned)c_b, (unsigned)c_h};
    hipStream_t st = (hipStream_t)stream;
    const int nz = nb * nh;
    if (N > 64) {
        const int tn_ = (N + 127) / 128;
        hipLaunchKernelGGL((conv_wgrad_kernel<128, false>), dim3(tj * tn_ * nz), dim3(256), 0, st, (const unsigned short*)x,
                           (const unsigned short*)y, (unsigned)(2 * x_elems), (unsigned)(2 * y_elems), g, M, J, tj * tn_, tn_, M,
                           make_fastdiv(M), make_fastdiv(M), (float*)nullptr, tn);
    } else {
        hipLaunchKernelGGL((conv_wgrad_kernel<64, false>), dim3(tj * nz), dim3(256), 0, st, (const unsigned short*)x,
                           (const unsigned short*)y, (unsigned)(2 * x_elems), (unsigned)(2 * y_elems), g, M, J, tj, 1, M, make_fastdiv(M),
                           make_fastdiv(M), (float*)nullptr, tn);
    }
    return launch_status();
}

static int stem_fwd_impl(const void* x4, const void* w, const lp_conv_geom* geom, void* out_bf16, const lp_bn_fuse* bn,
                         lp_stream_t stream) {
    using namespace lp;
    LP_REQUIRE(x4 && w && geom_ok(geom) && out_bf16);
    ConvGeom g = to_geom(geom);
    if (!is_stem(g)) return LP_ERR_UNSUPPORTED;
    ConvProblem p = conv_problem(kModeStem, x4, w, g, g.Ho, g.Wo, 64, 256);
    p.gate = &LpSwitches::stem_2d;
    p.ep = ConvEpilogue{(unsigned short*)out_bf16, nullptr, 64, 64};
    if (bn) {
        LP_REQUIRE(bn->sums && bn->seg_images >= 0);
        if (seg_split_rows(bn->seg_images, g.B, (long long)g.Ho * g.Wo, p.M) < 0) return LP_ERR_UNSUPPORTED;
        bn_fuse_begin(p.ep, bn);
    }
    return run_conv(p, stream);
}

extern "C" int lp_stem_fwd(const void* x4, const void* w, const lp_conv_geom* geom, void* out_bf16, lp_stream_t stream) {
    return stem_fwd_impl(x4, w, geom, out_bf16, nullptr, stream);
}

extern "C" int lp_stem_fwd_bn(const void* x4, const void* w, const lp_conv_geom* geom, void* out_bf16, const lp_bn_fuse* bn,
                              lp_stream_t stream) {
    LP_REQUIRE(bn);
    return stem_fwd_impl(x4, w, geom, out_bf16, bn, stream);
}

extern "C" int lp_stem_wgrad(const void* x4, const void* dy, const lp_conv_geom* geom, float* dw, int split_hint, void* workspace,
                             size_t workspace_bytes, lp_stream_t stream) {
    using namespace lp;
    LP_REQUIRE(x4 && dy && geom_ok(geom) && dw && workspace);
    ConvGeom g = to_geom(geom);
    if (!is_stem(g)) return LP_ERR_UNSUPPORTED;
    const WgradCandidates c = wgrad_candidates(g, true, split_hint);
    const WgradRoute& p = route_wgrad(c, lp_switches(), false);
    LP_REQUIRE(workspace_bytes >= p.ws_floats * sizeof(float));
    const int M = g.B * g.Ho * g.Wo, Kw = 256;
    const unsigned short *xs = (const unsigned short*)x4, *dys = (const unsigned short*)dy;
    const FastDiv dhw = make_fastdiv(g.Ho * g.Wo), dwo = make_fastdiv(g.Wo);
    hipStream_t st = (hipStream_t)stream;
    float* ws = (float*)workspace;
    g_last_conv_kernel = p.kernel;
    if (p.kernel == LP_CONV_KERNEL_STEM_WGRAD_NB)
        hipLaunchKernelGGL(stem_wgrad_nb_kernel, dim3(p.split), dim3(256), 0, st, xs, dys, (unsigned)(8ull * g.B * g.Hi * g.Wi),
                           (unsigned)(128ull * M), g, M, p.per, dhw, dwo, ws);
    else
        hipLaunchKernelGGL((conv_wgrad_kernel<64, true>), dim3(p.tiles_a * p.split), dim3(256), 0, st, xs, dys, 0u, 0u, g, M, Kw, p.tiles_a, 1,
                           p.per, dhw, dwo, ws, TnExt{});
    launch_wgrad_reduce<64>(ws, p.split, p.tiles_a, 1, Kw, 64, dw, st);
    return launch_status();
}
```

lightning-pose_amd/csrc/lp_common.h:

```cpp
#pragma once

#include <hip/hip_runtime.h>
#include <stdint.h>

#include "../../include/lp_hip.h"

namespace lp {

constexpr int kWave = 64;

typedef __attribute__((ext_vector_type(8))) __bf16 bf16x8;
typedef __attribute__((ext_vector_type(8))) unsigned short u16x8;
typedef __attribute__((ext_vector_type(4))) unsigned short u16x4;
typedef __attribute__((ext_vector_type(4))) float f32x4;
typedef __attribute__((ext_vector_type(16))) float f32x16;

__device__ __forceinline__ float bf16_to_f32(unsigned short b) { return __uint_as_float(((unsigned)b) << 16); }

#if defined(__HIP_DEVICE_COMPILE__)
typedef __attribute__((ext_vector_type(2))) __bf16 bf16x2_t;
typedef __attribute__((ext_vector_type(2))) float f32x2_t;
__device__ __forceinline__ unsigned short f32_to_bf16(float f) { return __builtin_bit_cast(unsigned short, (__bf16)f); }
__device__ __forceinline__ unsigned pack_bf16x2(float lo, float hi) {
    const f32x2_t v = {lo, hi};
// ... 94 lines not shown
__device__ __forceinline__ u16x8 buf_load16_nt(buf_rsrc r, unsigned voff, unsigned soff) {
    typedef __attribute__((ext_vector_type(4))) unsigned u32x4_t;
    const u32x4_t v = __builtin_amdgcn_raw_buffer_load_b128(r, voff, soff, 2);
    return __builtin_bit_cast(u16x8, v);
}
__device__ __forceinline__ void buf_load16_lds(buf_rsrc r, void* lds_wave_base, unsigned voff, unsigned soff) {
    __builtin_amdgcn_raw_ptr_buffer_load_lds(r, (__attribute__((address_space(3))) void*)lds_wave_base, 16, voff, soff, 0, 0);
}
#else
struct buf_rsrc {
    const char* p;
    unsigned bytes;
};
__device__ __forceinline__ buf_rsrc make_buf_rsrc(const void* p, unsigned bytes) { return buf_rsrc{(const char*)p, bytes}; }
__device__ __forceinline__ u16x8 buf_load16(buf_rsrc r, unsigned voff, unsigned soff) {
    u16x8 v = {0, 0, 0, 0, 0, 0, 0, 0};
    if (voff < r.bytes && (unsigned long long)voff + 16 <= r.bytes) v = *reinterpret_cast<const u16x8*>(r.p + voff + soff);
    return v;
}
__device__ __forceinline__ u16x8 buf_load16_nt(buf_rsrc r, unsigned voff, unsigned soff) { return buf_load16(r, voff, soff); }
#if !defined(__HIP__)
__device__ __forceinline__ void buf_load16_lds(buf_rsrc r, void* lds_wave_base, unsigned voff, unsigned soff) {
    *reinterpret_cast<u16x8*>(static_cast<char*>(lds_wave_base) + (threadIdx.x & 63) * 16) = buf_load16(r, voff, soff);
}
#else
__device__ __forceinline__ void buf_load16_lds(buf_rsrc, void*, unsigned, unsigned) {}
#endif
#endif

typedef __attribute__((ext_vector_type(4))) short s16x4_t;
#if defined(__HIP_DEVICE_COMPILE__)
__device__ __forceinline__ s16x4_t lds_read_tr16(const unsigned short* p) {
    return __builtin_amdgcn_ds_read_tr16_b64_v4i16((__attribute__((address_space(3))) s16x4_t*)p);
}
__device__ __forceinline__ s16x4_t lds_read_tr16_async(const unsigned short* p) {
    s16x4_t v;
    const unsigned a = (unsigned)(size_t)(__attribute__((address_space(3))) const unsigned short*)p;
    asm volatile("ds_read_b64_tr_b16 %0, %1" : "=v"(v) : "v"(a) : "memory");
    return v;
}
template <int OFF>
__device__ __forceinline__ s16x4_t lds_read_tr16_async_off(const unsigned char* p) {
    static_assert(OFF >= 0 && OFF < 65536, "16-bit offset field");
    s16x4_t v;
    const unsigned a = (unsigned)(size_t)(__attribute__((address_space(3))) const unsigned char*)p;
    asm volatile("ds_read_b64_tr_b16 %0, %1 offset:%2" : "=v"(v) : "v"(a), "n"(OFF) : "memory");
    return v;
}
#elif defined(__HIP__)
__device__ __forceinline__ s16x4_t lds_read_tr16(const unsigned short*) { return s16x4_t{0, 0, 0, 0}; }
__device__ __forceinline__ s16x4_t lds_read_tr16_async(const unsigned short*) { return s16x4_t{0, 0, 0, 0}; }
template <int OFF>
__device__ __forceinline__ s16x4_t lds_read_tr16_async_off(const unsigned char*) { return s16x4_t{0, 0, 0, 0}; }
#else
__device__ __forceinline__ s16x4_t lds_read_tr16(const unsigned short* p) {
    const int lane = threadIdx.x & 63, base = lane & ~15, c = lane & 15;
    s16x4_t r;
    for (int e = 0; e < 4; ++e) {
        const unsigned short* q = __shfl(p, base + 4 * e + (c >> 2), 64);
        r[e] = (short)q[c & 3];
    }
    return r;
}
__device__ __forceinline__ s16x4_t lds_read_tr16_async(const unsigned short* p) { return lds_read_tr16(p); }
template <int OFF>
__device__ __forceinline__ s16x4_t lds_read_tr16_async_off(const unsigned char* p) { return lds_read_tr16(reinterpret_cast<const unsigned short*>(p + OFF)); }
#endif

#if defined(__HIP_DEVICE_COMPILE__)
#define LP_OPAQUE(x) asm volatile("" : "+v"(x))
#else
#define LP_OPAQUE(x) asm volatile("" : "+r"(x))
#endif

#ifndef LP_UNIFORM_LOADS
#define LP_UNIFORM_LOADS 1
#endif
#if defined(__HIP_DEVICE_COMPILE__) && LP_UNIFORM_LOADS
template <typename T>
using uniform_ptr = const __attribute__((address_space(4))) T*;
template <typename T>
__device__ __forceinline__ uniform_ptr<T> as_uniform(const T* p) {
    return (uniform_ptr<T>)(unsigned long long)p;
}
#else
template <typename T>
using uniform_ptr = const T*;
template <typename T>
__host__ __device__ inline uniform_ptr<T> as_uniform(const T* p) {
    return p;
}
#endif

__device__ __forceinline__ float wave_sum(float v) {
#pragma unroll
    for (int m = 32; m >= 1; m >>= 1) v += __shfl_xor(v, m, 64);
    return v;
}

__device__ __forceinline__ float wave_max(float v) {
#pragma unroll
    for (int m = 32; m >= 1; m >>= 1) v = fmaxf(v, __shfl_xor(v, m, 64));
    return v;
}

template <int NW>
__device__ __forceinline__ float block_sum(float v, float* scratch) {
    v = wave_sum(v);
    const int lane = threadIdx.x & 63, wave = threadIdx.x >> 6;
    if (lane == 0) scratch[wave] = v;
    __syncthreads();
    float t = 0.f;
#pragma unroll
    for (int i = 0; i < NW; ++i) t += scratch[i];
    __syncthreads();
    return t;
}

template <int NW>
__device__ __forceinline__ float block_max(float v, float* scratch) {
    v = wave_max(v);
    const int lane = threadIdx.x & 63, wave = threadIdx.x >> 6;
    if (lane == 0) scratch[wave] = v;
    __syncthreads();
    float t = scratch[0];
#pragma unroll
    for (int i = 1; i < NW; ++i) t = fmaxf(t, scratch[i]);
    __syncthreads();
    return t;
}

constexpr long long kFxPoison = 5LL << 60;
constexpr long long kFxPoisonSeen = 1LL << 59;
__device__ __forceinline__ void fx_add(lp_fxsum* p, float t) {
    double td = (double)t;
    if (!(fabs(td) <= 0x1p127 * 2.0)) {
        atomicMax(&p->lo, kFxPoison);
        return;
    }
    td = fmin(fmax(td, -0x1p49), 0x1p49);
    const double h = rint(td * 0x1p12);
    const long long hi = (long long)h;
    const long long lo = (long long)rint((td - h * 0x1p-12) * 0x1p60);
    atomicAdd(reinterpret_cast<unsigned long long*>(&p->hi), (unsigned long long)hi);
    atomicAdd(reinterpret_cast<unsigned long long*>(&p->lo), (unsigned long long)lo);
}
__device__ __forceinline__ float fx_value(const lp_fxsum* p) {
    const long long lo = p->lo;
    if (lo >= kFxPoisonSeen || lo <= -kFxPoisonSeen) return __int_as_float(0x7fc00000);
    return (float)((double)p->hi * 0x1p-12 + (double)lo * 0x1p-60);
}

struct LpSwitches {
    int conv_pipe, conv_halo, conv_res2d, infer_pipe, gemm_pipe, wgrad_pipe, wgrad_nb, stem_2d, stem_wgrad_nb, pool_v2, conv_max_wgs, bn_bwd_wgs_per_cu;
};
const LpSwitches& lp_switches();

inline int launch_status() {
    hipError_t e = hipGetLastError();
    return e == hipSuccess ? LP_OK : (int)e;
}

}

#define LP_REQUIRE(cond)                    \
    do {                                    \
        if (!(cond)) return LP_ERR_ARGUMENT; \
    } while (0)
```

lightning-pose_amd/engine.py:

```python

from __future__ import annotations

import ctypes as C
import math
import os
from dataclasses import dataclass, field

import torch
import torch.distributed as dist

from . import _lib
from ._lib import check
from . import ops
from .ops import _p

BN_EPS = 1e-5
BN_MOMENTUM = 0.1
CPAD = 64


@dataclass
class ConvP:
    name: str
    kind: str
# ... 33 lines not shown
    bn3: BNP
    down: ConvP | None = None
    dbn: BNP | None = None


@dataclass
class Plan:
    stem: ConvP
    stem_bn: BNP
    blocks: list[Block]
    head: list[ConvP]
    n_backbone: int = 0
    n_total: int = 0
    n_wd: int = 0
    n_running: int = 0
    convs: list[ConvP] = field(default_factory=list)
    bns: list[BNP] = field(default_factory=list)

    def group_ranges(self) -> dict[str, tuple[int, int]]:
        return {"backbone": (0, self.n_backbone), "head": (self.n_backbone, self.n_total)}


def build_head(feat_channels: int, stride: int, num_keypoints: int, downsample_factor: int, int_channels: int | None = None) -> list[ConvP]:
    n_layers = int(math.log2(stride)) - downsample_factor - 1
    if n_layers < 1:
        raise NotImplementedError(f"downsample_factor={downsample_factor} leaves no upsampling layer for a stride-{stride} backbone")
    head: list[ConvP] = []
    cin = feat_channels // 4
    for i in range(n_layers):
        cout = num_keypoints if i == n_layers - 1 else (int_channels or num_keypoints)
        co_store, ci_store = -(-cin // 64) * 64, -(-cout // 64) * 64
        head.append(ConvP(f"head.upsampling_layers.{i + 1}", "convT", cin, cout, 3, 2, 1, co_store, ci_store))
        cin = cout
    return head


def build_plan(num_keypoints: int, downsample_factor: int) -> Plan:
    if num_keypoints > CPAD:
        raise NotImplementedError(f"at most {CPAD} heat-map channels (keypoints x views) are supported, got {num_keypoints}")
    stem = ConvP("backbone.0", "stem", 3, 64, 7, 2, 3, 64, 4)
    stem_bn = BNP("backbone.1", 64)
    blocks: list[Block] = []
    inplanes = 64
    for li, (planes, nblk, stride) in enumerate(((64, 3, 1), (128, 4, 2), (256, 6, 2), (512, 3, 2))):
        for bi in range(nblk):
            pre = f"backbone.{4 + li}.{bi}"
            st = stride if bi == 0 else 1
            blk = Block(
                ConvP(f"{pre}.conv1", "conv", inplanes, planes, 1, 1, 0, planes, inplanes), BNP(f"{pre}.bn1", planes),
                ConvP(f"{pre}.conv2", "conv", planes, planes, 3, st, 1, planes, planes), BNP(f"{pre}.bn2", planes),
                ConvP(f"{pre}.conv3", "conv", planes, planes * 4, 1, 1, 0, planes * 4, planes), BNP(f"{pre}.bn3", planes * 4))
            if bi == 0 and (st != 1 or inplanes != planes * 4):
                blk.down = ConvP(f"{pre}.downsample.0", "conv", inplanes, planes * 4, 1, st, 0, planes * 4, inplanes)
                blk.dbn = BNP(f"{pre}.downsample.1", planes * 4)
            blocks.append(blk)
            inplanes = planes * 4
    head = build_head(2048, 32, num_keypoints, downsample_factor)

    plan = Plan(stem, stem_bn, blocks, head)
    off = 0
    wd = 0
    run = 0

    def add_conv(c: ConvP):
        nonlocal off, wd
        c.w_off = off
        off += c.numel
        if c.kind != "stem":
            c.wd_off = wd
            wd += c.numel
        if c.kind == "convT":
            c.bias_off = off
            off += c.Ci
        plan.convs.append(c)

    def add_bn(b: BNP):
        nonlocal off, run
        b.g_off = off
        b.b_off = off + b.C
        off += 2 * b.C
        b.r_off = run
        run += 2 * b.C
        plan.bns.append(b)

    add_conv(stem)
    add_bn(stem_bn)
    for blk in blocks:
        add_conv(blk.conv1); add_bn(blk.bn1)
        add_conv(blk.conv2); add_bn(blk.bn2)
        add_conv(blk.conv3); add_bn(blk.bn3)
        if blk.down is not None:
            add_conv(blk.down); add_bn(blk.dbn)
    plan.n_backbone = off
    for c in head:
        add_conv(c)
    plan.n_total = off
    plan.n_wd = wd
    plan.n_running = run
    return plan


class Tape:

    def __init__(self):
        self.t: dict[str, torch.Tensor] = {}
        self.meta: dict[str, object] = {}


class Engine:
    wgrad_side_stream = True
    dgrad_mask_bits = True
    bn_bwd_ds = True
    bn_apply_rbn = True
    residual_fp32 = False
    dgrad_half_addend = True

    final_softmax = True

    def __init__(self, num_keypoints: int, downsample_factor: int = 2, device: torch.device | str = "cuda:0", plan: Plan | None = None):
        self.device = torch.device(device)
        ops.require_device_type(self.device)
        _lib.lib()
        self.K = num_keypoints
        self.ds = downsample_factor
        self.plan = build_plan(num_keypoints, downsample_factor) if plan is None else plan
        n = self.plan.n_total
        dev = self.device
        self.P = torch.zeros(n, device=dev, dtype=torch.float32)
        self.G = torch.zeros(n, device=dev, dtype=torch.float32)
        self.Wb = torch.zeros(n, device=dev, dtype=torch.bfloat16)
        self.Wd = torch.zeros(self.plan.n_wd, device=dev, dtype=torch.bfloat16)
        self.R = torch.zeros(self.plan.n_running, device=dev, dtype=torch.float32)
        for b in self.plan.bns:
            self.P[b.g_off:b.g_off + b.C] = 1.0
            self.R[b.r_off + b.C:b.r_off + 2 * b.C] = 1.0
        self.nbt = torch.zeros((), dtype=torch.long)
        self.sync_bn = False
        self.grad_progress = None
        self.single_backward = False
        self._bwd_training = True
        self.sync_bn_messages = 0
        self.process_group = None
        self.sync_bn_gather = os.environ.get("LP_SYNCBN_GATHER", "0") == "1"
        self.bn_bwd_terms = os.environ.get("LP_BN_BWD_TERMS", "1") != "0"
        self.dgrad_half_addend = os.environ.get("LP_DGRAD_HALF_ADDEND", "1") != "0"
        self.bn_apply_rbn = os.environ.get("LP_BN_APPLY_RBN", "1") != "0"
        self.bn_bwd_ds = os.environ.get("LP_BN_BWD_DS", "1") != "0"
        self.residual_fp32 = os.environ.get("LP_RESIDUAL_FP32", "0") == "1"
        self.dgrad_mask_bits = os.environ.get("LP_DGRAD_MASK_BITS", "1") != "0"
        self._gather_buf: torch.Tensor | None = None
        self._lib = _lib.lib()
        self.profile: list | None = None
        self._wgrad_ws: torch.Tensor | None = None
        self._red_ws: torch.Tensor | None = None
        self._side = None
        self._side_busy = False
        self._side_keep: list = []
        self._fold: tuple[torch.Tensor, torch.Tensor] | None = None

    def _zeros_f32(self, n: int) -> torch.Tensor:
        ar = getattr(self, "_zero_arena", None)
        if ar is not None and self._zero_off + n <= ar.numel():
            t = ar[self._zero_off:self._zero_off + n]
            self._zero_off += (n + 3) // 4 * 4
            return t
        return torch.zeros(n, device=self.device, dtype=torch.float32)

    def _zeros_fx(self, n: int) -> torch.Tensor:
        return self._zeros_f32(4 * n).view(torch.int64)

    def _timed(self, tag: str, flops: float, fn, nbytes: float = 0.0, layer: str = ""):
        if self.profile is None:
            return fn()
        e0, e1 = torch.cuda.Event(enable_timing=True), torch.cuda.Event(enable_timing=True)
        e0.record()
        out = fn()
        e1.record()
        if tag.startswith("conv_") and hasattr(self._lib, "lp_conv_last_kernel"):
            for old, new in _lib.CONV_KERNEL_LABEL.get(self._lib.lp_conv_last_kernel(), ()):
                tag = tag.replace(old, new)
        self.profile.append((tag, flops, e0, e1, nbytes, layer))
        return out

    def _wgrad(self, x, dy, g, dw: torch.Tensor, stem: bool = False, dbias: torch.Tensor | None = None) -> None:
        need = self._lib.lp_conv_wgrad_workspace_bytes(C.byref(g), 0)
        if self._wgrad_ws is None or self._wgrad_ws.numel() < need:
            self._join_side_stream()
            self._wgrad_ws = torch.empty(max(need, 96 << 20), device=self.device, dtype=torch.uint8)
        fn = self._lib.lp_stem_wgrad if stem else self._lib.lp_conv_wgrad
        what = "lp_stem_wgrad" if stem else "lp_conv_wgrad"
        if dbias is not None:
            what = "lp_conv_wgrad_bias"
            fn = lambda x_, dy_, g_, dw_, split, ws, nws, st: self._lib.lp_conv_wgrad_bias(x_, dy_, g_, dw_, _p(dbias), split, ws, nws, st)
        if (self.device.type != "cuda" or not self.wgrad_side_stream or self.profile is not None
                or os.environ.get("LP_WGRAD_SIDE_STREAM", "1") == "0"):
            check(fn(_p(x), _p(dy), C.byref(g), _p(dw), 0, _p(self._wgrad_ws), self._wgrad_ws.numel(), ops._stream()), what)
            return
        if self._side is None:
            self._side = torch.cuda.Stream(device=self.device)
        main = torch.cuda.current_stream(self.device)
        self._side.wait_stream(main)
        self._side_keep.append((x, dy))
        with torch.cuda.stream(self._side):
            check(fn(_p(x), _p(dy), C.byref(g), _p(dw), 0, _p(self._wgrad_ws), self._wgrad_ws.numel(), ops._stream()), what)
        self._side_busy = True

    def _join_side_stream(self) -> None:
        if getattr(self, "_side_busy", False):
            torch.cuda.current_stream(self.device).wait_stream(self._side)
            self._side_busy = False
            self._side_keep.clear()

    @staticmethod
    def _bytes(c: "ConvP", g, wgrad: bool = False) -> float:
        kk = 8 * 8 if c.kind == "stem" else c.k * c.k
        acts = 2.0 * g.B * (g.Hi * g.Wi * g.Ci + g.Ho * g.Wo * g.Co)
        return acts + (4.0 if wgrad else 2.0) * c.Co * kk * c.Ci

    @staticmethod
    def _flops(c: "ConvP", g) -> float:
        kk = c.k * c.k
        if c.kind == "convT":
            return 2.0 * g.B * g.Ho * g.Wo * c.cin * kk * c.cout
        return 2.0 * g.B * g.Ho * g.Wo * c.cout * kk * c.cin

    def param_view(self, c: ConvP | BNP, which: str = "weight", buf: torch.Tensor | None = None) -> torch.Tensor:
        buf = self.P if buf is None else buf
        if isinstance(c, BNP):
            off = c.g_off if which == "weight" else c.b_off
            return buf[off:off + c.C]
        if which == "bias":
            return buf[c.bias_off:c.bias_off + c.cout]
        flat = buf[c.w_off:c.w_off + c.numel]
        if c.kind == "stem":
            return flat.view(64, 8, 8, 4)[:, :7, :7, :3].permute(0, 3, 1, 2)
        if c.kind == "convT":
            return flat.view(c.Co, 3, 3, c.Ci)[:c.cin, :, :, :c.cout].permute(0, 3, 1, 2)
        return flat.view(c.Co, c.k, c.k, c.Ci).permute(0, 3, 1, 2)

    def running_view(self, b: BNP, which: str) -> torch.Tensor:
        off = b.r_off if which == "running_mean" else b.r_off + b.C
        return self.R[off:off + b.C]

    def state_dict(self) -> dict[str, torch.Tensor]:
        sd: dict[str, torch.Tensor] = {}
        plan = self.plan

        def put_bn(b: BNP):
            sd[f"{b.name}.weight"] = self.param_view(b, "weight")
            sd[f"{b.name}.bias"] = self.param_view(b, "bias")
            sd[f"{b.name}.running_mean"] = self.running_view(b, "running_mean")
            sd[f"{b.name}.running_var"] = self.running_view(b, "running_var")
            sd[f"{b.name}.num_batches_tracked"] = self.nbt

        sd[f"{plan.stem.name}.weight"] = self.param_view(plan.stem)
        put_bn(plan.stem_bn)
        for blk in plan.blocks:
            for c, b in ((blk.conv1, blk.bn1), (blk.conv2, blk.bn2), (blk.conv3, blk.bn3)):
                sd[f"{c.name}.weight"] = self.param_view(c)
                put_bn(b)
            if blk.down is not None:
                sd[f"{blk.down.name}.weight"] = self.param_view(blk.down)
                put_bn(blk.dbn)
        for c in plan.head:
            sd[f"{c.name}.weight"] = self.param_view(c)
            sd[f"{c.name}.bias"] = self.param_view(c, "bias")
        return sd

    @torch.no_grad()
    def load_state_dict(self, sd: dict[str, torch.Tensor], strict: bool = True) -> None:
        own = self.state_dict()
        missing = [k for k in own if k not in sd]
        unexpected = [k for k in sd if k not in own]
        if strict and (missing or unexpected):
            raise KeyError(f"state_dict mismatch: missing {missing[:5]}..., unexpected {unexpected[:5]}...")
        for k, dst in own.items():
            if k not in sd:
                continue
            if k.endswith("num_batches_tracked"):
                self.nbt.fill_(int(sd[k]))
                continue
            dst.copy_(sd[k].to(device=self.device, dtype=torch.float32))
        self.refresh_weight_copies()

    def invalidate_inference_copies(self) -> None:
        self._fold = None

    def refresh_weight_copies(self, lo: int = 0, hi: int | None = None) -> None:
        self._fold = None
        hi = self.plan.n_total if hi is None else hi
        check(self._lib.lp_cast_bf16(_p(self.P[lo:hi]), hi - lo, _p(self.Wb[lo:hi]), ops._stream()), "lp_cast_bf16")
        self.refresh_dgrad_copies(lo, hi)

    def refresh_dgrad_copies(self, lo: int = 0, hi: int | None = None) -> None:
        hi = self.plan.n_total if hi is None else hi
        for c in self.plan.convs:
            if c.kind == "stem" or not (lo <= c.w_off < hi):
                continue
            check(self._lib.lp_permute_cba(_p(self.Wb[c.w_off:]), c.Co, c.k * c.k, c.Ci, _p(self.Wd[c.wd_off:]), ops._stream()),
                  "lp_permute_cba")

    def zero_grad(self) -> None:
        self.G.zero_()

    def _geom(self, c: ConvP, B: int, Hi: int, Wi: int) -> _lib.ConvGeom:
        if c.kind == "convT":
# ... 202 lines not shown
        if H % 32 or W % 32:
            raise ValueError(f"image size must be a multiple of 32, got {H}x{W}")
        if len(parts) > 2 or any(p_.shape[1:] != parts[0].shape[1:] for p_ in parts):
            raise ValueError("a joint pass takes at most two batches of equally sized images")
        B = sum(p_.shape[0] for p_ in parts)
        seg = parts[0].shape[0] if (len(parts) == 2 and training) else 0
        if seg and not self.can_segment(seg, H, W):
            raise NotImplementedError(f"{seg} images of {H}x{W} do not end on a tile boundary in every layer: run the two batches separately")
        tp = Tape()
        T = tp.t
        plan = self.plan
        nseg = 2 if seg else 1
        n_bn = sum(2 * b.C for b in plan.bns) * nseg
        sums_all = torch.zeros(2 * n_bn, device=self.device, dtype=torch.int64)
        so = [0]

        def next_sums(b: BNP) -> torch.Tensor:
            s = sums_all[so[0]:so[0] + 4 * b.C * nseg]
            so[0] += 4 * b.C * nseg
            return s

        x4 = torch.empty(B, H, W, 4, device=self.device, dtype=torch.bfloat16)
        i0 = 0
        for p_ in parts:
            check(self._lib.lp_images_to_nhwc4(_p(p_), p_.shape[0], H, W, _p(x4[i0:]), ops._stream()), "lp_images_to_nhwc4")
            i0 += p_.shape[0]
        T["x4"] = x4
        def conv_bn(c: ConvP, b: BNP, xin, hh, ww, residual, relu, bits_key=None, residual_bn=None, apply=True, pair=None):
            sums = next_sums(b)
            zz, gg = self._conv_fwd(c, xin, B, hh, ww, sums if training else None, seg=seg)
            if not apply:
                mm, vv = self._bn_moments(b, zz, B * gg.Ho * gg.Wo, training, sums, training, seg)
                return zz, None, mm, vv, gg
            res = self._bn_fwd(b, zz, B * gg.Ho * gg.Wo, residual, relu, training, sums, have_sums=training,
                               want_bits=bits_key is not None and training, seg=seg, residual_bn=residual_bn, pair=pair)
            if len(res) == 4:
                T[bits_key] = res[3]
            aa, mm, vv = res[:3]
            return zz, aa, mm, vv, gg

        sb = plan.stem_bn
        s_sums = next_sums(sb)
        z, g = self._conv_fwd(plan.stem, x4, B, H, W, s_sums if training else None, seg=seg)
        h, w = g.Ho, g.Wo
        mu, iv = self._bn_moments(sb, z, B * h * w, training, s_sums, have_sums=training, seg=seg)
        T["stem.z"], T["stem.mu"], T["stem.iv"] = z, mu, iv
        ph, pw = (h - 1) // 2 + 1, (w - 1) // 2 + 1
        x = torch.empty(B, ph, pw, 64, device=self.device, dtype=torch.bfloat16)
        T["pool.arg"] = torch.empty(B, ph, pw, 64, device=self.device, dtype=torch.uint8)
        for si, (i0, n) in enumerate(self._segments(B, seg)):
            check(self._lib.lp_bn_relu_maxpool_fwd(_p(z[i0:i0 + n]), _p(mu[si * 64:]), _p(iv[si * 64:]), _p(self.param_view(sb, "weight")),
                                                   _p(self.param_view(sb, "bias")), n, h, w, 64, _p(x[i0:i0 + n]), _p(T["pool.arg"][i0:i0 + n]),
                                                   ops._stream()), "lp_bn_relu_maxpool_fwd")
        h, w = ph, pw
        tp.meta["stem_hw"] = (g.Ho, g.Wo)

        x_lo = None
        for i, blk in enumerate(plan.blocks):
            key = f"b{i}"
            T[f"{key}.x"] = x
            tp.meta[f"{key}.hw"] = (h, w)
            z1, a1, m1, v1, _ = conv_bn(blk.conv1, blk.bn1, x, h, w, None, True)
            z2, a2, m2, v2, g2 = conv_bn(blk.conv2, blk.bn2, a1, h, w, None, True)
            ho, wo = g2.Ho, g2.Wo
            rbn = None
            if blk.down is not None:
                zd, idt, md, vd, _ = conv_bn(blk.down, blk.dbn, x, h, w, None, False, apply=not self.bn_apply_rbn)
                T[f"{key}.zd"], T[f"{key}.md"], T[f"{key}.vd"] = zd, md, vd
                if self.bn_apply_rbn:
                    idt, rbn = zd, (blk.dbn, md, vd)
            else:
                idt = x
            pair = None
            if self.residual_fp32 and (rbn is not None or blk.down is None):
                nxt_identity = i + 1 < len(plan.blocks) and plan.blocks[i + 1].down is None
                y_lo = torch.empty(B, ho, wo, blk.bn3.C, device=self.device, dtype=torch.bfloat16) if nxt_identity else None
                pair = (x_lo if blk.down is None else None, y_lo)
            z3, out, m3, v3, _ = conv_bn(blk.conv3, blk.bn3, a2, ho, wo, idt, True, bits_key=f"{key}.out_bits", residual_bn=rbn, pair=pair)
            x_lo = pair[1] if pair is not None else None
            if x_lo is not None:
                T[f"{key}.out_lo"] = x_lo
            for nm, val in (("z1", z1), ("a1", a1), ("m1", m1), ("v1", v1), ("z2", z2), ("a2", a2), ("m2", m2), ("v2", v2),
                            ("z3", z3), ("m3", m3), ("v3", v3), ("out", out)):
                if val is not None:
                    T[f"{key}.{nm}"] = val
            x, h, w = out, ho, wo

        heat = self._head_forward(x, B, h, w, T)
        T["heat"] = heat
        tp.meta.update(B=B, H=H, W=W, training=training, seg=seg)
        if training:
            self.nbt += nseg
            self._fold = None
        return heat, tp

    def _folded(self) -> tuple[torch.Tensor, torch.Tensor]:
        if self._fold is None:
            plan = self.plan
            wf = torch.empty_like(self.Wb)
            bf = torch.zeros(plan.n_total, device=self.device, dtype=torch.float32)
            pairs = []
            for blk in plan.blocks:
                pairs += [(blk.conv1, blk.bn1), (blk.conv2, blk.bn2), (blk.conv3, blk.bn3)]
                if blk.down is not None:
                    pairs.append((blk.down, blk.dbn))
            for c, b in pairs:
                check(self._lib.lp_bn_fold(_p(self.P[c.w_off:]), _p(self.param_view(b, "weight")), _p(self.param_view(b, "bias")),
                                           _p(self.running_view(b, "running_mean")), _p(self.running_view(b, "running_var")), BN_EPS,
                                           c.Co, c.k * c.k * c.Ci, _p(wf[c.w_off:]), _p(bf[b.b_off:]), ops._stream()), "lp_bn_fold")
            self._fold = (wf, bf)
        return self._fold

    def forward_infer(self, images: torch.Tensor) -> torch.Tensor:
        ops.require_device(images)
        images = images.to(torch.float32).contiguous()
        if images.dim() != 4 or images.shape[1] != 3:
            raise ValueError(f"images must be (B, 3, H, W), got {tuple(images.shape)}")
        B, _, H, W = images.shape
        if H % 32 or W % 32:
            raise ValueError(f"image size must be a multiple of 32, got {H}x{W}")
        plan = self.plan
        wf, bf = self._folded()
        st = ops._stream()
        x4 = torch.empty(B, H, W, 4, device=self.device, dtype=torch.bfloat16)
        check(self._lib.lp_images_to_nhwc4(_p(images), B, H, W, _p(x4), st), "lp_images_to_nhwc4")
        sb = plan.stem_bn
        z, g = self._conv_fwd(plan.stem, x4, B, H, W, None)
        h, w = g.Ho, g.Wo
        mu, iv = self._bn_moments(sb, z, B * h * w, False, None)
        ph, pw = (h - 1) // 2 + 1, (w - 1) // 2 + 1
        x = torch.empty(B, ph, pw, 64, device=self.device, dtype=torch.bfloat16)
        arg = torch.empty(B, ph, pw, 64, device=self.device, dtype=torch.uint8)
        check(self._lib.lp_bn_relu_maxpool_fwd(_p(z), _p(mu), _p(iv), _p(self.param_view(sb, "weight")), _p(self.param_view(sb, "bias")), B, h, w,
                                               64, _p(x), _p(arg), st), "lp_bn_relu_maxpool_fwd")
        del z, arg
        h, w = ph, pw

        def layer(c: ConvP, b: BNP, xin, hh, ww, residual, relu):
            g_ = self._geom(c, B, hh, ww)
            out = torch.empty(B, g_.Ho, g_.Wo, c.Co, device=self.device, dtype=torch.bfloat16)
            run = lambda: check(self._lib.lp_conv_fwd_act(_p(xin), _p(wf[c.w_off:]), C.byref(g_), _p(bf[b.b_off:]), _p(residual), int(relu),
                                                          _p(out), st), "lp_conv_fwd_act")
            self._timed(f"conv_igemm_kernel<{128 if c.Co > 64 else 64},infer>", self._flops(c, g_), run, self._bytes(c, g_), layer=c.name)
            return out, g_

        for blk in plan.blocks:
            a1, _ = layer(blk.conv1, blk.bn1, x, h, w, None, True)
            a2, g2 = layer(blk.conv2, blk.bn2, a1, h, w, None, True)
            idt = x if blk.down is None else layer(blk.down, blk.dbn, x, h, w, None, False)[0]
            x, _ = layer(blk.conv3, blk.bn3, a2, g2.Ho, g2.Wo, idt, True)
            h, w = g2.Ho, g2.Wo
        return self._head_forward(x, B, h, w, {})

    def _bn_bwd(self, b: BNP, dy, y_out, z, mean, invstd, M: int, want_dres: bool, sums: torch.Tensor | None = None, seg: int = 0, ds=None):
        B = z.shape[0]
        rpi = M // B
        segs = self._segments(B, seg)
        Cn = b.C
        if sums is None:
            sums = self._zeros_fx(len(segs) * 2 * Cn)
            rws = self._reduce_ws(M, Cn)
            for si, (i0, n) in enumerate(segs):
                check(self._lib.lp_bn_bwd_reduce(_p(dy[i0:i0 + n]), _p(y_out[i0:i0 + n]) if y_out is not None else None, _p(z[i0:i0 + n]),
                                                 _p(mean[si * Cn:]), _p(invstd[si * Cn:]), n * rpi, Cn, _p(sums[si * 4 * Cn:]), _p(rws), rws.numel(),
                                                 ops._stream()), "lp_bn_bwd_reduce")
        world = 1
        local, total = sums, sums
        if not self._bwd_training:
            total = None
        elif self.sync_bn:
            local = sums.clone()
            self._sync_stats(sums)
            self.sync_bn_messages += 1
            world = dist.get_world_size(self.process_group)
        dz = torch.empty_like(z)
        dres = torch.empty_like(z) if want_dres else None
        gam = _p(self.param_view(b, "weight"))
        counts = [float(n * rpi * world) for _, n in segs]
        terms = torch.empty(len(segs) * 2 * Cn, device=z.device, dtype=torch.float32) if self.bn_bwd_terms else None
        if ds is not None:
            dsums = None
            if self.bn_bwd_ds and terms is not None and 256 % (Cn // 8) == 0:
                zd, md, vd = ds
                dsums = self._zeros_fx(len(segs) * 2 * Cn)
                need = int(self._lib.lp_bn_bwd_ds_workspace_bytes(M, Cn))
                if getattr(self, "_ds_ws", None) is None or self._ds_ws.numel() < need:
                    self._ds_ws = torch.empty(need, device=self.device, dtype=torch.uint8)
                check(self._lib.lp_bn_bwd_apply_seg_ds(_p(dy), _p(y_out), _p(z), _p(mean), _p(invstd), gam, _p(total), counts[0], counts[-1], M, Cn,
                                                       seg * rpi, _p(dz), _p(dres), _p(local), _p(self.G[b.b_off:]), _p(self.G[b.g_off:]),
                                                       _p(terms), _p(zd), _p(md), _p(vd), _p(dsums), _p(self._ds_ws), self._ds_ws.numel(),
                                                       ops._stream()), "lp_bn_bwd_apply_seg_ds")
                return dz, dres, dsums
        check(self._lib.lp_bn_bwd_apply_seg(_p(dy), _p(y_out), _p(z), _p(mean), _p(invstd), gam, _p(total), counts[0], counts[-1], M, Cn,
                                            seg * rpi, _p(dz), _p(dres), _p(local), _p(self.G[b.b_off:]), _p(self.G[b.g_off:]), _p(terms),
                                            ops._stream()), "lp_bn_bwd_apply_seg")
        return (dz, dres, None) if ds is not None else (dz, dres)

    def _conv_bwd(self, c: ConvP, x, dz, B, Hi, Wi, need_dx: bool, addend=None, relu_mask=None, accumulate_into=None, bn=None,
                  relu_bits=None, seg: int = 0, mask_bits=None, addend_half: bool = False):
        g = self._geom(c, B, Hi, Wi)
        self._timed(f"conv_wgrad_kernel<{128 if c.Co > 64 else 64}>", self._flops(c, g),
                    lambda: self._wgrad(x, dz, g, self.G[c.w_off:]), self._bytes(c, g, wgrad=True), layer=c.name)
        if not need_dx:
            return None
        st = ops._stream()
        if accumulate_into is not None:
            dx, addend, skip = accumulate_into, accumulate_into, 1
        else:
            dx, skip = torch.empty(B, Hi, Wi, c.Ci, device=self.device, dtype=torch.bfloat16), 0
        if bn is not None:
            assert accumulate_into is None
            b, z, mean, invstd, sums = bn
            if relu_bits is not None:
                relu_mask = None
            f = self._bn_fuse(sums, b, z, mean, invstd, mask_from_z=relu_mask is None and relu_bits is None, relu_bits=relu_bits, seg=seg,
                              addend_half=addend_half)
            run = lambda: check(self._lib.lp_conv_dgrad_bn(_p(dz), _p(self.Wd[c.wd_off:]), C.byref(g), _p(addend), _p(relu_mask), _p(dx),
                                                           C.byref(f), st), "lp_conv_dgrad_bn")
        elif mask_bits is not None and self.dgrad_mask_bits:
            relu_mask = None
            run = lambda: check(self._lib.lp_conv_dgrad_bits(_p(dz), _p(self.Wd[c.wd_off:]), C.byref(g), _p(addend), _p(mask_bits), _p(dx),
                                                             skip, st), "lp_conv_dgrad_bits")
        else:
            run = lambda: check(self._lib.lp_conv_dgrad(_p(dz), _p(self.Wd[c.wd_off:]), C.byref(g), None, _p(addend), _p(relu_mask),
                                                        _p(dx), None, c.Ci, 0, skip, st), "lp_conv_dgrad")
        dx_bytes = 2.0 * B * Hi * Wi * c.Ci
        extra = ((dx_bytes / 4 if addend_half else dx_bytes) if addend is not None else 0.0) + (dx_bytes if bn is not None else 0.0) + \
                (dx_bytes if relu_mask is not None else 0.0) + (dx_bytes / 16 if (bn is not None and relu_bits is not None) else 0.0) + \
                (dx_bytes / 16 if (bn is None and relu_mask is None and mask_bits is not None and self.dgrad_mask_bits) else 0.0)
        self._timed(f"conv_igemm_kernel<{128 if c.Ci > 64 else 64},dgrad>", self._flops(c, g), run, self._bytes(c, g) + extra, layer=c.name)
        return dx

    def backward(self, tp: Tape, g_heat: torch.Tensor, trace: dict | None = None) -> None:
        T, plan = tp.t, self.plan
        B, H, W = tp.meta["B"], tp.meta["H"], tp.meta["W"]
        self._bwd_training = bool(tp.meta.get("training", True))
        seg = tp.meta.get("seg", 0)
        nseg = 2 if seg else 1
        self._zero_arena = torch.zeros(4 * ((sum(2 * b.C for b in plan.bns) + 2 * plan.stem_bn.C) * nseg + sum(2 * c.Ci for c in plan.head)) + 64,
                                       device=self.device, dtype=torch.float32)
        self._zero_off = 0
        try:
            self._backward(tp, g_heat, trace, seg, nseg)
        finally:
            self._zero_arena = None

    def _backward(self, tp: Tape, g_heat: torch.Tensor, trace: dict | None, seg: int, nseg: int) -> None:
        T, plan = tp.t, self.plan
        B, H, W = tp.meta["B"], tp.meta["H"], tp.meta["W"]
        d = self._head_backward(T, B, g_heat)
        progress = self.grad_progress if (self.grad_progress is not None and self.single_backward) else None
        if progress is not None:
            progress(plan.n_backbone)

        def new_sums(b: BNP) -> torch.Tensor:
            return self._zeros_fx(2 * b.C * nseg)

        d_sums = None
        for i in range(len(plan.blocks) - 1, -1, -1):
            blk, key = plan.blocks[i], f"b{i}"
            if trace is not None:
                trace[f"{key}.dout"] = d
            hi, wi = tp.meta[f"{key}.hw"]
            st = blk.conv2.stride
            ho, wo = (hi - 1) // st + 1, (wi - 1) // st + 1
            Mo, Mi = B * ho * wo, B * hi * wi
            x = T[f"{key}.x"]
            last = i == len(plan.blocks) - 1
            dbn_sums = None
            if last:
                dz3, dres = self._bn_bwd(blk.bn3, d, T[f"{key}.out"], T[f"{key}.z3"], T[f"{key}.m3"], T[f"{key}.v3"], Mo, True, seg=seg)
            elif blk.down is not None:
                dz3, _, dbn_sums = self._bn_bwd(blk.bn3, d, None, T[f"{key}.z3"], T[f"{key}.m3"], T[f"{key}.v3"], Mo, False, sums=d_sums, seg=seg,
                                                ds=(T[f"{key}.zd"], T[f"{key}.md"], T[f"{key}.vd"]))
                dres = d
            else:
                dz3, _ = self._bn_bwd(blk.bn3, d, None, T[f"{key}.z3"], T[f"{key}.m3"], T[f"{key}.v3"], Mo, False, sums=d_sums, seg=seg)
                dres = d
            s2 = new_sums(blk.bn2)
            da2 = self._conv_bwd(blk.conv3, T[f"{key}.a2"], dz3, B, ho, wo, True,
                                 bn=(blk.bn2, T[f"{key}.z2"], T[f"{key}.m2"], T[f"{key}.v2"], s2), seg=seg)
            dz2, _ = self._bn_bwd(blk.bn2, da2, None, T[f"{key}.z2"], T[f"{key}.m2"], T[f"{key}.v2"], Mo, False, sums=s2, seg=seg)
            s1 = new_sums(blk.bn1)
            da1 = self._conv_bwd(blk.conv2, T[f"{key}.a1"], dz2, B, hi, wi, True,
                                 bn=(blk.bn1, T[f"{key}.z1"], T[f"{key}.m1"], T[f"{key}.v1"], s1), seg=seg)
            dz1, _ = self._bn_bwd(blk.bn1, da1, None, T[f"{key}.z1"], T[f"{key}.m1"], T[f"{key}.v1"], Mi, False, sums=s1, seg=seg)
            mask_x = x if i > 0 else None
            d_sums = None
            if blk.down is not None:
                dzd, _ = self._bn_bwd(blk.dbn, dres, None, T[f"{key}.zd"], T[f"{key}.md"], T[f"{key}.vd"], Mo, False, sums=dbn_sums, seg=seg)
                xbits = T.get(f"b{i - 1}.out_bits") if i > 0 else None
                if i > 0 and xbits is not None and self.dgrad_half_addend and blk.down.stride == 2 and blk.down.k == 1 and blk.conv1.stride == 1:
                    prev, pk = plan.blocks[i - 1], f"b{i - 1}"
                    gd = self._geom(blk.down, B, hi, wi)
                    self._timed(f"conv_wgrad_kernel<{128 if blk.down.Co > 64 else 64}>", self._flops(blk.down, gd),
                                lambda: self._wgrad(x, dzd, gd, self.G[blk.down.w_off:]), self._bytes(blk.down, gd, wgrad=True), layer=blk.down.name)
                    gh = _lib.ConvGeom(B, gd.Ho, gd.Wo, blk.down.Ci, gd.Ho, gd.Wo, blk.down.Co, 1, 1, 1, 0)
                    dd = torch.empty(B, gd.Ho, gd.Wo, blk.down.Ci, device=self.device, dtype=torch.bfloat16)
                    self._timed(f"conv_igemm_kernel<{128 if blk.down.Ci > 64 else 64},dgrad>", self._flops(blk.down, gd),
                                lambda: check(self._lib.lp_conv_dgrad(_p(dzd), _p(self.Wd[blk.down.wd_off:]), C.byref(gh), None, None, None, _p(dd), None,
                                                                      blk.down.Ci, 0, 0, ops._stream()), "lp_conv_dgrad"),
                                2.0 * B * gd.Ho * gd.Wo * (blk.down.Co + blk.down.Ci), layer=blk.down.name)
                    d_sums = new_sums(prev.bn3)
                    d = self._conv_bwd(blk.conv1, x, dz1, B, hi, wi, True, addend=dd, addend_half=True,
                                       bn=(prev.bn3, T[f"{pk}.z3"], T[f"{pk}.m3"], T[f"{pk}.v3"], d_sums), relu_bits=xbits, seg=seg)
                else:
                    d = self._conv_bwd(blk.conv1, x, dz1, B, hi, wi, True, relu_mask=mask_x, mask_bits=xbits)
                    self._conv_bwd(blk.down, x, dzd, B, hi, wi, True, relu_mask=mask_x, accumulate_into=d, mask_bits=xbits)
            elif i > 0:
                prev, pk = plan.blocks[i - 1], f"b{i - 1}"
                d_sums = new_sums(prev.bn3)
                d = self._conv_bwd(blk.conv1, x, dz1, B, hi, wi, True, addend=dres, relu_mask=mask_x,
                                   bn=(prev.bn3, T[f"{pk}.z3"], T[f"{pk}.m3"], T[f"{pk}.v3"], d_sums),
                                   relu_bits=T.get(f"{pk}.out_bits"), seg=seg)
            else:
                d = self._conv_bwd(blk.conv1, x, dz1, B, hi, wi, True, addend=dres, relu_mask=mask_x)
            if progress is not None:
                progress(blk.conv1.w_off)

        if trace is not None:
            trace["stem.dpool"] = d
        sh, sw = tp.meta["stem_hw"]
        sb = plan.stem_bn
        segs = self._segments(B, seg)
        ssum = self._zeros_fx(nseg * 2 * sb.C)
        gam, bet = self.param_view(sb, "weight"), self.param_view(sb, "bias")
        arg, sz, smu, siv = T["pool.arg"], T["stem.z"], T["stem.mu"], T["stem.iv"]
        for si, (i0, n) in enumerate(segs):
            check(self._lib.lp_bn_pool_bwd_reduce(_p(arg[i0:i0 + n]), _p(d[i0:i0 + n]), _p(sz[i0:i0 + n]), _p(smu[si * sb.C:]), _p(siv[si * sb.C:]),
                                                  _p(gam), _p(bet), n, sh, sw, 64, _p(ssum[si * 4 * sb.C:]), ops._stream()), "lp_bn_pool_bwd_reduce")
        world = 1
        slocal, stotal = ssum, ssum
        if not self._bwd_training:
            stotal = None
        elif self.sync_bn:
            slocal = ssum.clone()
            self._sync_stats(ssum)
            self.sync_bn_messages += 1
            world = dist.get_world_size(self.process_group)
        dz = torch.empty(B, sh, sw, 64, device=self.device, dtype=torch.bfloat16)
        for si, (i0, n) in enumerate(segs):
            check(self._lib.lp_bn_pool_bwd_apply(_p(arg[i0:i0 + n]), _p(d[i0:i0 + n]), _p(sz[i0:i0 + n]), _p(smu[si * sb.C:]), _p(siv[si * sb.C:]),
                                                 _p(gam), _p(bet), _p(stotal[si * 4 * sb.C:]) if stotal is not None else None,
                                                 float(n * sh * sw * world), n, sh, sw, 64, _p(dz[i0:i0 + n]), _p(slocal[si * 4 * sb.C:]),
                                                 _p(self.G[sb.b_off:]), _p(self.G[sb.g_off:]), ops._stream()), "lp_bn_pool_bwd_apply")
        g = self._geom(plan.stem, B, H, W)
        self._timed("conv_wgrad_kernel<64,stem>", self._flops(plan.stem, g),
                    lambda: self._wgrad(T["x4"], dz, g, self.G[plan.stem.w_off:], stem=True), self._bytes(plan.stem, g, wgrad=True), layer=plan.stem.name)
        self._join_side_stream()


class HeadEngine(Engine):

    def __init__(self, in_channels: int, stride: int, num_keypoints: int, downsample_factor: int = 2, deconv_out_channels: int | None = None,
                 final_softmax: bool = True, device: torch.device | str = "cuda:0"):
        if num_keypoints > CPAD:
            raise NotImplementedError(f"at most {CPAD} heat-map channels are supported, got {num_keypoints}")
        if in_channels % 4:
            raise ValueError(f"PixelShuffle(2) needs a multiple of 4 input channels, got {in_channels}")
        head = build_head(in_channels, stride, num_keypoints, downsample_factor, deconv_out_channels)
        plan = Plan(None, None, [], head)
        off = wd = 0
        for c in head:
            c.w_off, c.wd_off = off, wd
            off += c.numel
            wd += c.numel
            c.bias_off = off
            off += c.Ci
            plan.convs.append(c)
        plan.n_backbone, plan.n_total, plan.n_wd, plan.n_running = 0, off, wd, 0
        super().__init__(num_keypoints, downsample_factor, device, plan=plan)
        self.in_channels = in_channels
        self.final_softmax = bool(final_softmax)

    def state_dict(self) -> dict[str, torch.Tensor]:
        sd: dict[str, torch.Tensor] = {}
        for c in self.plan.head:
            sd[f"{c.name}.weight"] = self.param_view(c)
            sd[f"{c.name}.bias"] = self.param_view(c, "bias")
        return sd

    def forward(self, features: torch.Tensor, training: bool = True) -> tuple[torch.Tensor, Tape]:
        ops.require_device(features)
        if features.dim() != 4 or features.shape[1] != self.in_channels:
            raise ValueError(f"features must be (B, {self.in_channels}, h, w), got {tuple(features.shape)}")
        B, _, h, w = features.shape
        x = features.detach().permute(0, 2, 3, 1).to(torch.bfloat16).contiguous()
        tp = Tape()
        tp.meta.update(B=B, h=h, w=w)
        heat = self._head_forward(x, B, h, w, tp.t)
        return heat, tp

    def backward(self, tp: Tape, g_heat: torch.Tensor, trace: dict | None = None) -> torch.Tensor:
        d = self._head_backward(tp.t, tp.meta["B"], g_heat)
        self._join_side_stream()
        return d.permute(0, 3, 1, 2).to(torch.float32)
```

profiles/kernel_resources.py:

```python
import os
import re
import shutil
import subprocess
import sys
import tempfile

ROOT = os.path.dirname(os.path.dirname(os.path.abspath(__file__)))
LLVM = os.path.join(os.environ.get("ROCM_PATH", "/opt/rocm"), "lib", "llvm", "bin")
HOT = ("lp::conv_pipe_kernel", "lp::conv_spec_kernel", "lp::conv_wgrad_pipe_kernel", "lp::conv_res2d_kernel", "lp::conv_stem2d_kernel", "lp::conv_wgrad_kernel", "lp::stem_wgrad_nb_kernel", "lp::conv_wgrad_nb_kernel",
       "lp::conv_igemm_kernel", "lp::bn_apply_kernel", "lp::bn_bwd_apply_kernel", "lp::bn_relu_maxpool_fwd_kernel", "lp::bn_pool_bwd_v2_kernel",
       "lp::colreduce_kernel", "lp::rows_reduce_kernel", "lp::decode_fwd_kernel", "lp::decode_bwd_kernel", "lp::heatmap_gen_kernel",
       "lp::hm_rowsq_kernel", "lp::hm_grad_kernel", "lp::softmax2d", "lp::adam_kernel", "lp::pca_kernel", "lp::temporal_kernel",
       "lp::attn_fwd_kernel", "lp::attn_bwd_kv_kernel", "lp::pixel_shuffle",
       "lp::layernorm_ls_fwd_kernel", "lp::layernorm_ls_bwd_kernel")
ALLOWED_SCRATCH = (
    re.compile(r"lp::decode_bwd_kernel<\d+, \d+, 64, "),
    re.compile(r"lp::bn_bwd_apply_kernel<false, false>"),
    re.compile(r"lp::conv_igemm_kernel<128, 1>"),
)


def kernels(so_path: str) -> list[dict]:
    out = []
    with tempfile.TemporaryDirectory() as tmp:
        so = os.path.join(tmp, "lib.so")
        shutil.copy(so_path, so)
        subprocess.run([os.path.join(LLVM, "llvm-objdump"), "--offloading", so], check=True, capture_output=True, cwd=tmp)
        for f in sorted(os.listdir(tmp)):
            if "gfx950" not in f:
                continue
            notes = subprocess.run([os.path.join(LLVM, "llvm-readelf"), "--notes", os.path.join(tmp, f)], check=True, capture_output=True, text=True).stdout
            for blk in notes.split("  - .agpr_count:")[1:]:
                def num(key, blk=blk):
                    m = re.search(r"\." + key + r":\s+(\d+)", blk)
                    return int(m.group(1)) if m else 0
                name = re.search(r"\.name:\s+(\S+)", blk).group(1)
                out.append({"mangled": name, "agpr": int(re.match(r"\s*(\d+)", blk).group(1)), "vgpr": num("vgpr_count"), "vgpr_spill": num("vgpr_spill_count"),
                            "sgpr_spill": num("sgpr_spill_count"), "scratch": num("private_segment_fixed_size"), "lds": num("group_segment_fixed_size"),
                            "max_flat_wg": num("max_flat_workgroup_size")})
    names = subprocess.run(["c++filt"], input="\n".join(k["mangled"] for k in out), capture_output=True, text=True, check=True).stdout.splitlines()
    for k, n in zip(out, names):
        k["name"] = n.split("(")[0].replace("void ", "")
    return out


def hot_with_scratch(ks: list[dict]) -> list[dict]:
    return [k for k in ks if k["scratch"] > 0 and k["name"].startswith(HOT) and not any(p.search(k["name"]) for p in ALLOWED_SCRATCH)]


def main() -> int:
    args = [a for a in sys.argv[1:] if not a.startswith("--")]
    so = args[0] if args else os.path.join(ROOT, "lightning-pose_amd", "liblp_hip.so")
    ks = kernels(so)
    show = ks if "--all" in sys.argv else [k for k in ks if k["name"].startswith(HOT)]
    print(f"{len(ks)} gfx950 kernels in {so}; {'all' if '--all' in sys.argv else 'hot'} kernels:")
    print(f"{'vgpr':>5} {'agpr':>5} {'spill':>5} {'scratch':>7} {'lds':>7}  kernel")
    for k in sorted(show, key=lambda k: k["name"]):
        print(f"{k['vgpr']:5d} {k['agpr']:5d} {k['vgpr_spill']:5d} {k['scratch']:7d} {k['lds']:7d}  {k['name']}")
    bad = hot_with_scratch(ks)
    print(f"\n{sum(k['scratch'] > 0 for k in ks)} kernel(s) with scratch in the library, {len(bad)} of them hot")
    for k in bad:
        print(f"  SCRATCH {k['scratch']:5d} B ({k['vgpr_spill']} spilled VGPRs)  {k['name']}")
    return 1 if bad else 0


if __name__ == "__main__":
    raise SystemExit(main())
```

Before: 4692 frames/s.

## Fuse batchnorm backward apply into conv3 1x1 weight-gradient kernel

Adds a bn_wgrad kernel that computes the BN backward dz tile on the fly while loading it as the B operand of the 1x1 conv3 weight-gradient GEMM. The column-0 tiles also write dz out for the later dgrad. The goal is to drop the separate BN-apply pass and the re-read of dz by the wgrad kernel for bottleneck conv3 layers with Ci<=128. In exchange, the BN math is repeated across every output tile row, the load per step rises (d, z, a), and non-row-0 workgroups perform redundant elementwise work.

```diff
diff --git a/include/lp_hip.h b/include/lp_hip.h
--- a/include/lp_hip.h
+++ b/include/lp_hip.h
@@ -20,7 +20,7 @@
 
 enum { LP_TF_NONE = 0, LP_TF_SINGLE = 1, LP_TF_PER_FRAME = 2, LP_TF_PER_VIEW = 3 };
 
-#define LP_HIP_ABI_VERSION 148
+#define LP_HIP_ABI_VERSION 149
 int lp_version(void);
 const char* lp_strerror(int code);
 
@@ -117,6 +117,7 @@
 #define LP_CONV_KERNEL_PIPE_HALO 4
 #define LP_CONV_KERNEL_STEM_WGRAD_NB 8
 #define LP_CONV_KERNEL_WGRAD_NB 9
+#define LP_CONV_KERNEL_BN_WGRAD 10
 #define LP_CONV_KERNEL_RES2D 5
 int lp_conv_last_kernel(void);
 
@@ -248,6 +249,11 @@
 int lp_bn_bwd_apply_seg(const void* dy, const void* y_out, const void* x, const float* mean, const float* invstd, const float* gamma,
                         const lp_fxsum* sums, float count0, float count1, int M, int C, int seg_rows, void* dx, void* dres,
                         const lp_fxsum* sums_local, float* dbeta_acc, float* dgamma_acc, float* terms_ws, lp_stream_t stream);
+size_t lp_bn_bwd_apply_wgrad_workspace_bytes(const lp_conv_geom* geom);
+int lp_bn_bwd_apply_wgrad_seg(const void* dy, const void* y_out, const void* x, const float* mean, const float* invstd, const float* gamma,
+                              const lp_fxsum* sums, float count0, float count1, int M, int C, int seg_rows, void* dx, void* dres,
+                              const lp_fxsum* sums_local, float* dbeta_acc, float* dgamma_acc, float* terms_ws, const void* a,
+                              const lp_conv_geom* geom, float* dw, void* workspace, size_t workspace_bytes, lp_stream_t stream);
 size_t lp_bn_bwd_ds_workspace_bytes(int M, int C);
 int lp_bn_bwd_apply_seg_ds(const void* dy, const void* y_out, const void* x, const float* mean, const float* invstd, const float* gamma,
                            const lp_fxsum* sums, float count0, float count1, int M, int C, int seg_rows, void* dx, void* dres,
diff --git a/lightning-pose_amd/_lib.py b/lightning-pose_amd/_lib.py
--- a/lightning-pose_amd/_lib.py
+++ b/lightning-pose_amd/_lib.py
@@ -51,7 +51,7 @@
 
 HM_MSE, HM_KL, HM_JS = 0, 1, 2
 (CONV_KERNEL_IGEMM, CONV_KERNEL_PIPE, CONV_KERNEL_WGRAD, CONV_KERNEL_WGRAD_PIPE, CONV_KERNEL_PIPE_HALO, CONV_KERNEL_RES2D, _CONV_KERNEL_6,
- _CONV_KERNEL_7, CONV_KERNEL_STEM_WGRAD_NB, CONV_KERNEL_WGRAD_NB) = range(10)
+ _CONV_KERNEL_7, CONV_KERNEL_STEM_WGRAD_NB, CONV_KERNEL_WGRAD_NB, CONV_KERNEL_BN_WGRAD) = range(11)
 CONV_KERNEL_LABEL = {
     CONV_KERNEL_PIPE: (("conv_igemm_kernel", "conv_pipe_kernel"),),
     CONV_KERNEL_PIPE_HALO: (("conv_igemm_kernel", "conv_pipe_kernel"), (">", ",halo>")),
@@ -67,7 +67,7 @@
 AUG_ELASTIC_MAX_RADIUS = 20
 TF_NONE, TF_SINGLE, TF_PER_FRAME, TF_PER_VIEW = 0, 1, 2, 3
 
-ABI_VERSION = 148
+ABI_VERSION = 149
 
 _P, _I, _F, _L, _Z = C.c_void_p, C.c_int, C.c_float, C.c_long, C.c_size_t
 
@@ -132,6 +132,9 @@
     "lp_bn_apply_seg_lo": (_I, [_P, _P, _P, _P, _P, _P, _P, _P, _P, _P, _P, _P, _I, _I, _I, _I, _P, _P, _P, _P]),
     "lp_bn_apply_seg_rbn": (_I, [_P, _P, _P, _P, _P, _P, _P, _P, _P, _P, _I, _I, _I, _I, _P, _P, _P]),
     "lp_bn_bwd_apply_seg": (_I, [_P, _P, _P, _P, _P, _P, _P, _F, _F, _I, _I, _I, _P, _P, _P, _P, _P, _P, _P]),
+    "lp_bn_bwd_apply_wgrad_workspace_bytes": (_Z, [C.POINTER(ConvGeom)]),
+    "lp_bn_bwd_apply_wgrad_seg": (_I, [_P, _P, _P, _P, _P, _P, _P, _F, _F, _I, _I, _I, _P, _P, _P, _P, _P, _P, _P, C.POINTER(ConvGeom), _P, _P, _Z,
+                                       _P]),
     "lp_bn_bwd_ds_workspace_bytes": (_Z, [_I, _I]),
     "lp_bn_bwd_apply_seg_ds": (_I, [_P, _P, _P, _P, _P, _P, _P, _F, _F, _I, _I, _I, _P, _P, _P, _P, _P, _P, _P, _P, _P, _P, _P, _Z, _P]),
     "lp_bn_bwd_reduce": (_I, [_P, _P, _P, _P, _P, _I, _I, _P, _P, _Z, _P]),
@@ -246,6 +249,9 @@
     return _lib
 
 
+ERR_ARGUMENT, ERR_UNSUPPORTED = -1, -2
+
+
 def check(code: int, what: str) -> None:
     if code == 0:
         return
diff --git a/lightning-pose_amd/csrc/api.hip b/lightning-pose_amd/csrc/api.hip
--- a/lightning-pose_amd/csrc/api.hip
+++ b/lightning-pose_amd/csrc/api.hip
@@ -25,6 +25,7 @@
     s.pool_v2 = env_int("LP_POOL_V2", 1);
     s.bn_bwd_wgs_per_cu = env_int("LP_BN_BWD_WGS_PER_CU", 5);
     if (s.bn_bwd_wgs_per_cu < 1 || s.bn_bwd_wgs_per_cu > 5) s.bn_bwd_wgs_per_cu = 5;
+    s.bn_wgrad_fused = env_int("LP_BN_WGRAD_FUSED", 1);
     s.conv_max_wgs = env_int("LP_CONV_MAX_WGS", 0);
     return s;
 }
diff --git a/lightning-pose_amd/csrc/bn.hip b/lightning-pose_amd/csrc/bn.hip
--- a/lightning-pose_amd/csrc/bn.hip
+++ b/lightning-pose_amd/csrc/bn.hip
@@ -1015,6 +1015,12 @@
     return launch_status();
 }
 
+void lp::launch_bn_bwd_terms(const lp_fxsum* sums, float count0, float count1, int C, int nseg, float* terms, const lp_fxsum* sums_local,
+                         float* dbeta_acc, float* dgamma_acc, hipStream_t st) {
+    hipLaunchKernelGGL(lp::bn_bwd_terms_kernel, dim3((nseg * 2 * C + 255) / 256), dim3(256), 0, st, sums, 1.f / count0, 1.f / count1, C, nseg, terms,
+                       sums_local, dbeta_acc, dgamma_acc);
+}
+
 static int bn_bwd_apply_impl(const void* dy, const void* y_out, const void* x, const float* mean, const float* invstd, const float* gamma,
                              const lp_fxsum* sums, float count0, float count1, int M, int C, int seg_rows, void* dx, void* dres,
                              const lp_fxsum* sums_local, float* dbeta_acc, float* dgamma_acc, float* terms_ws, lp_stream_t stream) {
diff --git a/lightning-pose_amd/csrc/conv.hip b/lightning-pose_amd/csrc/conv.hip
--- a/lightning-pose_amd/csrc/conv.hip
+++ b/lightning-pose_amd/csrc/conv.hip
@@ -1184,6 +1184,7 @@
 }
 #include "conv_stem_wgrad.h"
 #include "conv_wgrad_nb.h"
+#include "conv_bn_wgrad.h"
 namespace lp {
 
 constexpr int kWgradWgs = 512;
@@ -1331,6 +1332,23 @@
         return r;
     }
     return c.r[c.n - 1];
+}
+
+constexpr int kBnWgradMaxC = 2048;
+constexpr int kBnWgradMaxCi = 128;
+static WgradRoute bn_wgrad_candidate(const ConvGeom& g, bool any_rows = false) {
+    WgradRoute p{};
+    const long long M = (long long)g.B * g.Ho * g.Wo;
+    if (g.R != 1 || g.S != 1 || g.stride != 1 || g.pad != 0 || g.Hi != g.Ho || g.Wi != g.Wo) return p;
+    if (g.Co % 128 != 0 || g.Co > kBnWgradMaxC || g.Ci % 8 != 0 || M * g.Co >= (1LL << 31) || M * g.Ci >= (1LL << 31)) return p;
+    if (!any_rows && g.Ci > kBnWgradMaxCi) return p;
+    p = plan_wgrad((int)M, g.Ci, g.Co, 0);
+    p.kernel = LP_CONV_KERNEL_BN_WGRAD;
+    return p;
+}
+static WgradRoute route_bn_wgrad(const ConvGeom& g, const LpSwitches& sw) {
+    if (sw.bn_wgrad_fused == 0) return WgradRoute{};
+    return bn_wgrad_candidate(g, sw.bn_wgrad_fused == 2);
 }
 
 template <int BN>
@@ -1702,6 +1720,39 @@
     return stem_fwd_impl(x4, w, geom, out_bf16, bn, stream);
 }
 
+extern "C" size_t lp_bn_bwd_apply_wgrad_workspace_bytes(const lp_conv_geom* geom) {
+    using namespace lp;
+    if (!geom_ok(geom)) return 0;
+    return route_bn_wgrad(to_geom(geom), lp_switches()).ws_floats * sizeof(float);
+}
+
+extern "C" int lp_bn_bwd_apply_wgrad_seg(const void* dy, const void* y_out, const void* x, const float* mean, const float* invstd,
+                                         const float* gamma, const lp_fxsum* sums, float count0, float count1, int M, int C, int seg_rows,
+                                         void* dx, void* dres, const lp_fxsum* sums_local, float* dbeta_acc, float* dgamma_acc, float* terms_ws,
+                                         const void* a, const lp_conv_geom* geom, float* dw, void* workspace, size_t workspace_bytes,
+                                         lp_stream_t stream) {
+    using namespace lp;
+    LP_REQUIRE(dy && x && mean && invstd && gamma && dx && M > 0 && C > 0 && count0 > 0.f && count1 > 0.f && seg_rows >= 0 && seg_rows < M);
+    LP_REQUIRE(sums_local != nullptr || (dbeta_acc == nullptr && dgamma_acc == nullptr));
+    LP_REQUIRE(terms_ws && a && geom_ok(geom) && dw && workspace);
+    const ConvGeom g = to_geom(geom);
+    LP_REQUIRE((long long)g.B * g.Ho * g.Wo == M && g.Co == C);
+    const WgradRoute p = route_bn_wgrad(g, lp_switches());
+    if (!p.ok || dres != nullptr || seg_rows % kBK != 0) return LP_ERR_UNSUPPORTED;
+    LP_REQUIRE(workspace_bytes >= p.ws_floats * sizeof(float));
+    hipStream_t st = (hipStream_t)stream;
+    launch_bn_bwd_terms(sums, count0, count1, C, seg_rows > 0 ? 2 : 1, terms_ws, sums_local, dbeta_acc, dgamma_acc, st);
+    const BnWgradArgs bn{(const unsigned short*)dy, (const unsigned short*)y_out, (const unsigned short*)x, mean, invstd, gamma, terms_ws,
+                         (unsigned short*)dx, seg_rows};
+    const int tiles = p.tiles_a * p.tiles_b;
+    const auto kernel = y_out != nullptr ? bn_wgrad_kernel<true> : bn_wgrad_kernel<false>;
+    g_last_conv_kernel = p.kernel;
+    hipLaunchKernelGGL(kernel, dim3(tiles * p.split), dim3(256), 0, st, (const unsigned short*)a, bn, (unsigned)(2ull * M * g.Ci),
+                       (unsigned)(2ull * M * C), M, g.Ci, C, tiles, p.tiles_b, p.per, (float*)workspace);
+    launch_wgrad_reduce<128>((const float*)workspace, p.split, tiles, p.tiles_b, g.Ci, C, dw, st);
+    return launch_status();
+}
+
 extern "C" int lp_stem_wgrad(const void* x4, const void* dy, const lp_conv_geom* geom, float* dw, int split_hint, void* workspace,
                              size_t workspace_bytes, lp_stream_t stream) {
     using namespace lp;
diff --git a/lightning-pose_amd/csrc/conv_bn_wgrad.h b/lightning-pose_amd/csrc/conv_bn_wgrad.h
--- /dev/null
+++ b/lightning-pose_amd/csrc/conv_bn_wgrad.h
@@ -0,0 +1,199 @@
+#pragma once
+
+#ifndef LP_BNW_DEEP
+#define LP_BNW_DEEP 1
+#endif
+
+namespace lp {
+
+struct BnWgradArgs {
+    const unsigned short* d;
+    const unsigned short* yout;
+    const unsigned short* z;
+    const float* mean;
+    const float* invstd;
+    const float* gamma;
+    const float* terms;
+    unsigned short* dz;
+    int seg_rows;
+};
+
+template <bool MASK>
+__global__ __launch_bounds__(256, 2) void bn_wgrad_kernel(const unsigned short* __restrict__ A, BnWgradArgs bn, unsigned a_bytes, unsigned d_bytes,
+                                                          int M, int Kw, int Co, int tiles, int tiles_n, int m_per_split,
+                                                          float* __restrict__ ws) {
+    constexpr int BN = 128, NT = BN / 64, RB = BN / 32;
+    constexpr int LDA = kBM + 32, LDB = BN + 32;
+    __shared__ __attribute__((aligned(16))) unsigned short sA[2][kBK * LDA];
+    __shared__ __attribute__((aligned(16))) unsigned short sB[2][kBK * LDB];
+
+    const int tid = threadIdx.x, lane = tid & 63;
+    const int wave = __builtin_amdgcn_readfirstlane(tid >> 6);
+    const int wm = wave >> 1, wn = wave & 1;
+    const int work = xcd_remap(blockIdx.x, gridDim.x);
+    const int slice = work / tiles, tile = work - slice * tiles;
+    const int j0 = (tile / tiles_n) * kBM, n0 = (tile % tiles_n) * BN;
+    const int m_begin = slice * m_per_split, m_end = min(M, m_begin + m_per_split);
+    const bool want_dz = j0 == 0;
+
+    const int jc = tid & 15, pg = tid >> 4;
+    const int j = j0 + jc * 8;
+    const unsigned jinv = j < Kw ? 0u : ~0u;
+    const int nB = n0 + jc * 8;
+
+    f32x16 acc[2][NT];
+#pragma unroll
+    for (int mt = 0; mt < 2; ++mt)
+#pragma unroll
+        for (int nt = 0; nt < NT; ++nt)
+#pragma unroll
+            for (int e = 0; e < 16; ++e) acc[mt][nt][e] = 0.f;
+
+    struct Step {
+        u16x8 a[4], d[RB], z[RB], y[MASK ? RB : 1];
+    };
+    Step s0, s1;
+
+    const buf_rsrc rsrc_a = make_buf_rsrc(A, a_bytes), rsrc_d = make_buf_rsrc(bn.d, d_bytes), rsrc_z = make_buf_rsrc(bn.z, d_bytes);
+    const buf_rsrc rsrc_y = make_buf_rsrc(MASK ? bn.yout : bn.d, d_bytes);
+    const unsigned ci2 = (unsigned)Kw * 2u, co2 = (unsigned)Co * 2u;
+    const int row0 = pg * 4;
+    const unsigned voffA = (unsigned)((m_begin + row0) * Kw + j) * 2u, voffB = (unsigned)((m_begin + row0) * Co + nB) * 2u;
+
+    auto load_step = [&](int mk, Step& s) {
+        const unsigned step = (unsigned)(mk - m_begin);
+        const unsigned soffA = step * ci2, soffB = step * co2;
+        const bool ragged = mk + kBK > m_end;
+#pragma unroll
+        for (int i = 0; i < 4; ++i) {
+            const unsigned rinv = (ragged && mk + row0 + i >= m_end) ? ~0u : 0u;
+            s.a[i] = buf_load16(rsrc_a, (voffA + i * ci2) | jinv | rinv, soffA);
+            s.d[i] = buf_load16(rsrc_d, (voffB + i * co2) | rinv, soffB);
+            s.z[i] = buf_load16(rsrc_z, (voffB + i * co2) | rinv, soffB);
+            if (MASK) s.y[MASK ? i : 0] = buf_load16(rsrc_y, (voffB + i * co2) | rinv, soffB);
+        }
+    };
+
+    float mu[8], ga[8], k0[8], k1[8];
+    int cur_sg = -1;
+    auto constants = [&](int sg) {
+#pragma unroll
+        for (int i = 0; i < 8; ++i) {
+            const float is = bn.invstd[sg * Co + nB + i];
+            mu[i] = bn.mean[sg * Co + nB + i];
+            ga[i] = bn.gamma[nB + i] * is;
+            k0[i] = bn.terms[sg * 2 * Co + nB + i];
+            k1[i] = bn.terms[sg * 2 * Co + Co + nB + i] * is;
+        }
+        cur_sg = sg;
+    };
+
+    auto store_step = [&](int buf, int mk, const Step& s) {
+        const int sg = (bn.seg_rows > 0 && mk >= bn.seg_rows) ? 1 : 0;
+        if (sg != cur_sg) constants(sg);
+        const bool ragged = mk + kBK > m_end;
+#pragma unroll
+        for (int i = 0; i < 4; ++i) *reinterpret_cast<u16x8*>(&sA[buf][(row0 + i) * LDA + jc * 8]) = s.a[i];
+#pragma unroll
+        for (int i = 0; i < RB; ++i) {
+            float dz[8], x[8], o[8];
+#pragma unroll
+            for (int q = 0; q < 8; ++q) {
+                dz[q] = bf16_to_f32(s.d[i][q]);
+                x[q] = bf16_to_f32(s.z[i][q]);
+            }
+            if (MASK) {
+#pragma unroll
+                for (int q = 0; q < 8; ++q)
+                    if (!bf16_positive(s.y[MASK ? i : 0][q])) dz[q] = 0.f;
+            }
+#pragma unroll
+            for (int q = 0; q < 8; ++q) {
+                o[q] = ga[q] * (dz[q] - k0[q] - (x[q] - mu[q]) * k1[q]);
+            }
+            u16x8 rb = pack_bf16x8(o);
+            const int m = mk + row0 + i;
+            const bool valid = !ragged || m < m_end;
+            if (!valid) rb = zero8();
+            *reinterpret_cast<u16x8*>(&sB[buf][(row0 + i) * LDB + jc * 8]) = rb;
+            if (want_dz && valid) *reinterpret_cast<u16x8*>(bn.dz + (size_t)m * Co + nB) = rb;
+        }
+    };
+
+    const int fq = lane >> 4, fi = lane & 15;
+    const int frow = (fq >> 1) * 8 + (fi >> 2), fcol = (fq & 1) * 16 + (fi & 3) * 4;
+    auto frag = [&](const unsigned short* tile_, int ld, int ch0, int kk) -> bf16x8 {
+        const unsigned short* p = tile_ + (kk * 16 + frow) * ld + ch0 + fcol;
+        const s16x4_t lo = lds_read_tr16(p), hi = lds_read_tr16(p + 4 * ld);
+        typedef __attribute__((ext_vector_type(8))) short s16x8_t;
+        const s16x8_t v = {lo[0], lo[1], lo[2], lo[3], hi[0], hi[1], hi[2], hi[3]};
+        return __builtin_bit_cast(bf16x8, v);
+    };
+    auto mma_step = [&](int buf) {
+#pragma unroll
+        for (int kk = 0; kk < kBK / 16; ++kk) {
+            bf16x8 a[2], b[NT];
+#pragma unroll
+            for (int mt = 0; mt < 2; ++mt) a[mt] = frag(sA[buf], LDA, wm * 64 + mt * 32, kk);
+#pragma unroll
+            for (int nt = 0; nt < NT; ++nt) b[nt] = frag(sB[buf], LDB, wn * (NT * 32) + nt * 32, kk);
+            __builtin_amdgcn_sched_barrier(0);
+#pragma unroll
+            for (int mt = 0; mt < 2; ++mt)
+#pragma unroll
+                for (int nt = 0; nt < NT; ++nt) acc[mt][nt] = __builtin_amdgcn_mfma_f32_32x32x16_bf16(a[mt], b[nt], acc[mt][nt], 0, 0, 0);
+            __builtin_amdgcn_sched_barrier(0);
+        }
+    };
+
+    const int KT = (m_end - m_begin + kBK - 1) / kBK;
+    if (LP_BNW_DEEP && !MASK && KT >= 2) {
+        load_step(m_begin, s0);
+        load_step(m_begin + kBK, s1);
+        store_step(0, m_begin, s0);
+        __syncthreads();
+        int kt = 0;
+        for (; kt + 3 < KT; kt += 2) {
+            load_step(m_begin + (kt + 2) * kBK, s0);
+            mma_step(0);
+            store_step(1, m_begin + (kt + 1) * kBK, s1);
+            __syncthreads();
+            load_step(m_begin + (kt + 3) * kBK, s1);
+            mma_step(1);
+            store_step(0, m_begin + (kt + 2) * kBK, s0);
+            __syncthreads();
+        }
+        const bool three = kt + 2 < KT;
+        if (three) load_step(m_begin + (kt + 2) * kBK, s0);
+        mma_step(0);
+        store_step(1, m_begin + (kt + 1) * kBK, s1);
+        __syncthreads();
+        mma_step(1);
+        if (three) {
+            store_step(0, m_begin + (kt + 2) * kBK, s0);
+            __syncthreads();
+            mma_step(0);
+        }
+    } else if (KT > 0) {
+        load_step(m_begin, s0);
+        store_step(0, m_begin, s0);
+        __syncthreads();
+        for (int kt = 0; kt < KT; ++kt) {
+            const int cur = kt & 1;
+            if (kt + 1 < KT) load_step(m_begin + (kt + 1) * kBK, s0);
+            mma_step(cur);
+            if (kt + 1 < KT) store_step(cur ^ 1, m_begin + (kt + 1) * kBK, s0);
+            __syncthreads();
+        }
+    }
+
+    float* dst = ws + ((((size_t)slice * tiles + tile) * 4 + wave) * (2 * NT * 16)) * 64 + lane;
+#pragma unroll
+    for (int mt = 0; mt < 2; ++mt)
+#pragma unroll
+        for (int nt = 0; nt < NT; ++nt)
+#pragma unroll
+            for (int e = 0; e < 16; ++e) dst[((mt * NT + nt) * 16 + e) * 64] = acc[mt][nt][e];
+}
+
+}
diff --git a/lightning-pose_amd/csrc/lp_common.h b/lightning-pose_amd/csrc/lp_common.h
--- a/lightning-pose_amd/csrc/lp_common.h
+++ b/lightning-pose_amd/csrc/lp_common.h
@@ -270,9 +270,12 @@
 }
 
 struct LpSwitches {
-    int conv_pipe, conv_halo, conv_res2d, infer_pipe, gemm_pipe, wgrad_pipe, wgrad_nb, stem_2d, stem_wgrad_nb, pool_v2, conv_max_wgs, bn_bwd_wgs_per_cu;
+    int conv_pipe, conv_halo, conv_res2d, infer_pipe, gemm_pipe, wgrad_pipe, wgrad_nb, stem_2d, stem_wgrad_nb, pool_v2, conv_max_wgs, bn_bwd_wgs_per_cu, bn_wgrad_fused;
 };
 const LpSwitches& lp_switches();
+
+void launch_bn_bwd_terms(const lp_fxsum* sums, float count0, float count1, int C, int nseg, float* terms, const lp_fxsum* sums_local,
+                         float* dbeta_acc, float* dgamma_acc, hipStream_t st);
 
 inline int launch_status() {
     hipError_t e = hipGetLastError();
diff --git a/lightning-pose_amd/engine.py b/lightning-pose_amd/engine.py
--- a/lightning-pose_amd/engine.py
+++ b/lightning-pose_amd/engine.py
@@ -209,6 +209,7 @@
         self._lib = _lib.lib()
         self.profile: list | None = None
         self._wgrad_ws: torch.Tensor | None = None
+        self._bn_wgrad_ws: torch.Tensor | None = None
         self._red_ws: torch.Tensor | None = None
         self._side = None
         self._side_busy = False
@@ -717,7 +718,8 @@
             h, w = g2.Ho, g2.Wo
         return self._head_forward(x, B, h, w, {})
 
-    def _bn_bwd(self, b: BNP, dy, y_out, z, mean, invstd, M: int, want_dres: bool, sums: torch.Tensor | None = None, seg: int = 0, ds=None):
+    def _bn_bwd(self, b: BNP, dy, y_out, z, mean, invstd, M: int, want_dres: bool, sums: torch.Tensor | None = None, seg: int = 0, ds=None,
+                wgrad=None):
         B = z.shape[0]
         rpi = M // B
         segs = self._segments(B, seg)
@@ -756,16 +758,38 @@
                                                        _p(terms), _p(zd), _p(md), _p(vd), _p(dsums), _p(self._ds_ws), self._ds_ws.numel(),
                                                        ops._stream()), "lp_bn_bwd_apply_seg_ds")
                 return dz, dres, dsums
+        if wgrad is not None:
+            fused = False
+            c, a, g = wgrad
+            need = int(self._lib.lp_bn_bwd_apply_wgrad_workspace_bytes(C.byref(g))) if (terms is not None and dres is None) else 0
+            if need > 0:
+                if self._bn_wgrad_ws is None or self._bn_wgrad_ws.numel() < need:
+                    self._bn_wgrad_ws = torch.empty(need, device=self.device, dtype=torch.uint8)
+                ws = self._bn_wgrad_ws
+
+                def run():
+                    rc = self._lib.lp_bn_bwd_apply_wgrad_seg(_p(dy), _p(y_out), _p(z), _p(mean), _p(invstd), gam, _p(total), counts[0], counts[-1],
+                                                             M, Cn, seg * rpi, _p(dz), None, _p(local), _p(self.G[b.b_off:]), _p(self.G[b.g_off:]),
+                                                             _p(terms), _p(a), C.byref(g), _p(self.G[c.w_off:]), _p(ws), ws.numel(), ops._stream())
+                    if rc != _lib.ERR_UNSUPPORTED:
+                        check(rc, "lp_bn_bwd_apply_wgrad_seg")
+                    return rc == 0
+                fused = self._timed("bn_wgrad_kernel<128>", self._flops(c, g), run, 2.0 * M * (3 * Cn + c.Ci) + 4.0 * c.Co * c.Ci, layer=c.name)
+            if fused:
+                return dz, dres, True
         check(self._lib.lp_bn_bwd_apply_seg(_p(dy), _p(y_out), _p(z), _p(mean), _p(invstd), gam, _p(total), counts[0], counts[-1], M, Cn,
                                             seg * rpi, _p(dz), _p(dres), _p(local), _p(self.G[b.b_off:]), _p(self.G[b.g_off:]), _p(terms),
                                             ops._stream()), "lp_bn_bwd_apply_seg")
+        if wgrad is not None:
+            return dz, dres, False
         return (dz, dres, None) if ds is not None else (dz, dres)
 
     def _conv_bwd(self, c: ConvP, x, dz, B, Hi, Wi, need_dx: bool, addend=None, relu_mask=None, accumulate_into=None, bn=None,
-                  relu_bits=None, seg: int = 0, mask_bits=None, addend_half: bool = False):
+                  relu_bits=None, seg: int = 0, mask_bits=None, addend_half: bool = False, wgrad_done: bool = False):
         g = self._geom(c, B, Hi, Wi)
-        self._timed(f"conv_wgrad_kernel<{128 if c.Co > 64 else 64}>", self._flops(c, g),
-                    lambda: self._wgrad(x, dz, g, self.G[c.w_off:]), self._bytes(c, g, wgrad=True), layer=c.name)
+        if not wgrad_done:
+            self._timed(f"conv_wgrad_kernel<{128 if c.Co > 64 else 64}>", self._flops(c, g),
+                        lambda: self._wgrad(x, dz, g, self.G[c.w_off:]), self._bytes(c, g, wgrad=True), layer=c.name)
         if not need_dx:
             return None
         st = ops._stream()
@@ -832,6 +856,7 @@
             Mo, Mi = B * ho * wo, B * hi * wi
             x = T[f"{key}.x"]
             last = i == len(plan.blocks) - 1
+            w3_done = False
             dbn_sums = None
             if last:
                 dz3, dres = self._bn_bwd(blk.bn3, d, T[f"{key}.out"], T[f"{key}.z3"], T[f"{key}.m3"], T[f"{key}.v3"], Mo, True, seg=seg)
@@ -840,11 +865,12 @@
                                                 ds=(T[f"{key}.zd"], T[f"{key}.md"], T[f"{key}.vd"]))
                 dres = d
             else:
-                dz3, _ = self._bn_bwd(blk.bn3, d, None, T[f"{key}.z3"], T[f"{key}.m3"], T[f"{key}.v3"], Mo, False, sums=d_sums, seg=seg)
+                dz3, _, w3_done = self._bn_bwd(blk.bn3, d, None, T[f"{key}.z3"], T[f"{key}.m3"], T[f"{key}.v3"], Mo, False, sums=d_sums, seg=seg,
+                                               wgrad=(blk.conv3, T[f"{key}.a2"], self._geom(blk.conv3, B, ho, wo)))
                 dres = d
             s2 = new_sums(blk.bn2)
             da2 = self._conv_bwd(blk.conv3, T[f"{key}.a2"], dz3, B, ho, wo, True,
-                                 bn=(blk.bn2, T[f"{key}.z2"], T[f"{key}.m2"], T[f"{key}.v2"], s2), seg=seg)
+                                 bn=(blk.bn2, T[f"{key}.z2"], T[f"{key}.m2"], T[f"{key}.v2"], s2), seg=seg, wgrad_done=w3_done)
             dz2, _ = self._bn_bwd(blk.bn2, da2, None, T[f"{key}.z2"], T[f"{key}.m2"], T[f"{key}.v2"], Mo, False, sums=s2, seg=seg)
             s1 = new_sums(blk.bn1)
             da1 = self._conv_bwd(blk.conv2, T[f"{key}.a1"], dz2, B, hi, wi, True,
diff --git a/profiles/kernel_resources.py b/profiles/kernel_resources.py
--- a/profiles/kernel_resources.py
+++ b/profiles/kernel_resources.py
@@ -8,6 +8,7 @@
 ROOT = os.path.dirname(os.path.dirname(os.path.abspath(__file__)))
 LLVM = os.path.join(os.environ.get("ROCM_PATH", "/opt/rocm"), "lib", "llvm", "bin")
 HOT = ("lp::conv_pipe_kernel", "lp::conv_spec_kernel", "lp::conv_wgrad_pipe_kernel", "lp::conv_res2d_kernel", "lp::conv_stem2d_kernel", "lp::conv_wgrad_kernel", "lp::stem_wgrad_nb_kernel", "lp::conv_wgrad_nb_kernel",
+       "lp::bn_wgrad_kernel",
        "lp::conv_igemm_kernel", "lp::bn_apply_kernel", "lp::bn_bwd_apply_kernel", "lp::bn_relu_maxpool_fwd_kernel", "lp::bn_pool_bwd_v2_kernel",
        "lp::colreduce_kernel", "lp::rows_reduce_kernel", "lp::decode_fwd_kernel", "lp::decode_bwd_kernel", "lp::heatmap_gen_kernel",
        "lp::hm_rowsq_kernel", "lp::hm_grad_kernel", "lp::softmax2d", "lp::adam_kernel", "lp::pca_kernel", "lp::temporal_kernel",
```

Result: no change. 4733 frames/s, median of 6 (+0.9%).
